# fixstars/cuda-bundle-adjustment

Measured on NVIDIA H100. Metric: LM edges/sec (10 iters), higher is better.
Workload: dtype f64

## Files before the change

### cuda-bundle-adjustment_b200/binding.py

```python
import ctypes as C
import os

import numpy as np

HERE = os.path.dirname(os.path.abspath(__file__))
ROBUST_NONE, ROBUST_HUBER, ROBUST_TUKEY = 0, 1, 2
EDGE_MONOCULAR, EDGE_STEREO = 0, 1
PROFILE_ITEMS = ("0: Initialize Optimizer", "1: Build Structure", "2: Compute Error", "3: Build System",
                 "4: Schur Complement", "5: Symbolic Decomposition", "6: Numerical Decomposition", "7: Update Solution")


PCG_INFO_LEN = 16
PCG_INFO_FIELDS = ("kernel", "two_level", "aggs_per_cta", "G", "gs", "A", "maxRows", "capBlocks", "zhInSmem", "coarse_kernel",
                   "cinfo", "status", "iters", "coarse_rebuilds", "bj_retries", "bad_rebuilds")
PCG_KERNELS = ("none", "k_pcg", "k_pcg2", "k_pcg3", "k_pcg4", "k_pcg5", "k_pcg5_big", "k_pcg5t")
COARSE_KERNELS = ("none", "k_coarse_invert", "cluster2<8>", "cluster2<16>", "k_coarse_dense", "k_coarse_chol_cluster")


class CubaError(RuntimeError):
    pass


def library_path():
    return os.path.join(HERE, "libcuba_b200.so")


class _Config(C.Structure):
    _fields_ = [("device", C.c_int), ("use_fp32", C.c_int), ("pcg_max_iters", C.c_int), ("pcg_tol", C.c_double),
                ("deterministic", C.c_int), ("reserved", C.c_int * 7)]


class _Problem(C.Structure):
    _fields_ = [("Pall", C.c_int32), ("numP", C.c_int32), ("Lall", C.c_int32), ("numL", C.c_int32),
                ("q", C.c_void_p), ("t", C.c_void_p), ("cam", C.c_void_p), ("Xw", C.c_void_p),
                ("E2", C.c_int32), ("idx2", C.c_void_p), ("meas2", C.c_void_p), ("omega2", C.c_void_p),
                ("E3", C.c_int32), ("idx3", C.c_void_p), ("meas3", C.c_void_p), ("omega3", C.c_void_p)]


class _IterStat(C.Structure):
    _fields_ = [("iteration", C.c_int32), ("trials", C.c_int32), ("chi2", C.c_double), ("lambda_", C.c_double),
                ("pcg_iters", C.c_int32), ("pcg_failed", C.c_int32)]


class _Sizes(C.Structure):
    _fields_ = [(n, C.c_int32) for n in ("Pall", "numP", "Lall", "numL", "E2", "E3", "nhpl", "nblk", "nmul", "nblk_full")]


_lib = None

_SYMBOLS = [
    "cuba_last_error", "cuba_version", "cuba_engine_create", "cuba_engine_destroy", "cuba_engine_set_robust_kernel",
    "cuba_comm_unique_id", "cuba_engine_set_comm", "cuba_engine_set_problem", "cuba_engine_set_structure_reuse", "cuba_engine_get_structure_reuses", "cuba_engine_set_state", "cuba_engine_get_sizes", "cuba_engine_reset_state", "cuba_engine_get_stream", "cuba_engine_flush_l2",
    "cuba_engine_optimize", "cuba_engine_get_state", "cuba_engine_get_chi2", "cuba_engine_get_profile",
    "cuba_engine_get_launch_count", "cuba_get_transfer_bytes", "cuba_stage_linearize", "cuba_stage_max_diagonal", "cuba_stage_solve", "cuba_stage_update",
    "cuba_stage_commit", "cuba_stage_chi2", "cuba_debug_get_hpl_structure", "cuba_debug_get_hsc_structure",
    "cuba_debug_get_system", "cuba_debug_get_schur", "cuba_debug_get_delta", "cuba_debug_get_pcg_info", "cuba_debug_get_coarse", "cuba_debug_build_structure_host", "cuba_debug_pcg_partition", "cuba_debug_pcg5_plan", "cuba_debug_pcg5_plan_apc", "cuba_debug_dropin_problem", "cuba_bench_stage",
]


def exported_symbols():
    return list(_SYMBOLS)


def load_library():
    global _lib
    if _lib is not None:
        return _lib
    path = library_path()
    if not os.path.exists(path):
        raise CubaError("%s not built: run `python -c 'import __graft_entry__ as g; g.build()'` (no CPU fallback exists)" % path)
    L = C.CDLL(path)
    L.cuba_last_error.restype = C.c_char_p
    vp, i, d = C.c_void_p, C.c_int, C.c_double
    sig = {
        "cuba_engine_create": [C.POINTER(_Config), C.POINTER(vp)],
        "cuba_engine_destroy": [vp],
        "cuba_engine_set_robust_kernel": [vp, i, i, d],
        "cuba_comm_unique_id": [vp],
        "cuba_engine_set_comm": [vp, i, i, vp],
        "cuba_engine_set_problem": [vp, C.POINTER(_Problem)],
        "cuba_engine_set_structure_reuse": [vp, i],
        "cuba_engine_get_structure_reuses": [vp, C.POINTER(C.c_longlong)],
        "cuba_engine_set_state": [vp, vp, vp, vp],
        "cuba_engine_get_sizes": [vp, C.POINTER(_Sizes)],
        "cuba_engine_reset_state": [vp],
        "cuba_engine_get_stream": [vp, C.POINTER(vp)],
        "cuba_engine_flush_l2": [vp],
        "cuba_engine_optimize": [vp, i, vp, C.POINTER(i)],
        "cuba_engine_get_state": [vp, vp, vp, vp],
        "cuba_engine_get_chi2": [vp, vp],
        "cuba_engine_get_profile": [vp, vp],
        "cuba_engine_get_launch_count": [vp, C.POINTER(C.c_longlong)],
        "cuba_get_transfer_bytes": [C.POINTER(C.c_longlong), C.POINTER(C.c_longlong)],
        "cuba_stage_linearize": [vp, C.POINTER(d)],
        "cuba_stage_max_diagonal": [vp, C.POINTER(d)],
        "cuba_stage_solve": [vp, d, C.POINTER(i), C.POINTER(i)],
        "cuba_stage_update": [vp, d, C.POINTER(d), C.POINTER(d)],
        "cuba_stage_commit": [vp, i],
        "cuba_stage_chi2": [vp, C.POINTER(d)],
        "cuba_debug_get_hpl_structure": [vp, vp, vp, vp],
        "cuba_debug_get_hsc_structure": [vp, vp, vp],
        "cuba_debug_get_system": [vp, vp, vp, vp, vp, vp],
        "cuba_debug_get_schur": [vp, vp, vp, vp],
        "cuba_debug_get_delta": [vp, vp, vp],
        "cuba_debug_get_pcg_info": [vp, vp, C.POINTER(d)],
        "cuba_debug_get_coarse": [vp, vp, vp, vp],
        "cuba_debug_build_structure_host": [C.POINTER(_Problem), i, i, C.POINTER(_Sizes), vp, vp, vp, vp, vp, vp, vp, vp],
        "cuba_debug_pcg_partition": [C.POINTER(_Problem), i, i, vp],
        "cuba_debug_pcg5_plan": [C.POINTER(_Problem), i, i, i, vp],
        "cuba_debug_pcg5_plan_apc": [C.POINTER(_Problem), i, i, i, i, vp, C.POINTER(C.c_uint64)],
        "cuba_debug_dropin_problem": [vp, C.POINTER(_Problem)],
        "cuba_bench_stage": [vp, i, i, i, d, C.POINTER(d)],
    }
    for name, args in sig.items():
        fn = getattr(L, name)
        fn.argtypes = args
        fn.restype = C.c_int
    _lib = L
    return L


def _check(rc):
    if rc != 0:
        raise CubaError("cuba error %d: %s" % (rc, load_library().cuba_last_error().decode()))


def _p(a):
    return None if a is None else a.ctypes.data_as(C.c_void_p)


def _problem_struct(prob):
    keep = [np.ascontiguousarray(prob.q, dtype=np.float64), np.ascontiguousarray(prob.t, dtype=np.float64),
            np.ascontiguousarray(prob.cam, dtype=np.float64), np.ascontiguousarray(prob.Xw, dtype=np.float64),
            np.ascontiguousarray(prob.idx2, dtype=np.int32), np.ascontiguousarray(prob.meas2, dtype=np.float64),
            np.ascontiguousarray(prob.omega2, dtype=np.float64), np.ascontiguousarray(prob.idx3, dtype=np.int32),
            np.ascontiguousarray(prob.meas3, dtype=np.float64), np.ascontiguousarray(prob.omega3, dtype=np.float64)]
    P = _Problem(prob.Pall, prob.numP, prob.Lall, prob.numL, _p(keep[0]), _p(keep[1]), _p(keep[2]), _p(keep[3]),
                 prob.E2, _p(keep[4]), _p(keep[5]), _p(keep[6]), prob.E3, _p(keep[7]), _p(keep[8]), _p(keep[9]))
    return P, keep


def transfer_bytes():
    a, b = C.c_longlong(0), C.c_longlong(0)
    _check(load_library().cuba_get_transfer_bytes(C.byref(a), C.byref(b)))
    return a.value, b.value


def build_structure_host(prob, rank=0, world=1):
    L = load_library()
    P, keep = _problem_struct(prob)
    sz = _Sizes()
    _check(L.cuba_debug_build_structure_host(C.byref(P), rank, world, C.byref(sz), None, None, None, None, None, None, None, None))
    out = {n: getattr(sz, n) for n, _ in _Sizes._fields_}
    arrs = {"hplColPtr": np.zeros(sz.numL + 1, np.int32), "hplRowInd": np.zeros(sz.nhpl, np.int32),
            "edge2Hpl": np.zeros(sz.E2 + sz.E3, np.int32), "hscRowPtr": np.zeros(sz.numP + 1, np.int32),
            "hscColInd": np.zeros(sz.nblk, np.int32), "fullRowPtr": np.zeros(sz.numP + 1, np.int32),
            "fullColInd": np.zeros(sz.nblk_full, np.int32), "shard": np.zeros(4, np.int32)}
    _check(L.cuba_debug_build_structure_host(C.byref(P), rank, world, C.byref(sz), *[_p(arrs[k]) for k in
           ("hplColPtr", "hplRowInd", "edge2Hpl", "hscRowPtr", "hscColInd", "fullRowPtr", "fullColInd", "shard")]))
    out.update(arrs)
    return out


def pcg_partition_host(prob, n_ctas=148, max_aggregates=74):
    L = load_library()
    P, keep = _problem_struct(prob)
    info = np.zeros(8, np.int32)
    _check(L.cuba_debug_pcg_partition(C.byref(P), int(n_ctas), int(max_aggregates), _p(info)))
    return dict(zip(("G", "gs", "A", "needMax", "maxRows", "blkMax", "maxNeedAgg", "coarse_list_size"), (int(v) for v in info)))


def pcg5_plan_host(prob, world=1, num_sms=148, max_aggregates=74):
    L = load_library()
    P, keep = _problem_struct(prob)
    info = np.zeros(8, np.int32)
    _check(L.cuba_debug_pcg5_plan(C.byref(P), int(world), int(num_sms), int(max_aggregates), _p(info)))
    return dict(zip(("ok", "G", "gs", "A", "needMax", "maxRows", "maxNeedAgg", "halo_rows"), (int(v) for v in info)))


def pcg5_plan_apc_host(prob, aggs_per_cta, world=1, num_sms=132, max_aggregates=148):
    L = load_library()
    P, keep = _problem_struct(prob)
    info = np.zeros(8, np.int32)
    h = C.c_uint64(0)
    _check(L.cuba_debug_pcg5_plan_apc(C.byref(P), int(world), int(num_sms), int(max_aggregates), int(aggs_per_cta), _p(info), C.byref(h)))
    out = dict(zip(("ok", "G", "gs", "A", "needMax", "maxRows", "maxNeedAgg", "halo_rows"), (int(v) for v in info)))
    out["hash"] = int(h.value)
    return out


class Engine:

    def __init__(self, device=-1, use_fp32=False, pcg_max_iters=0, pcg_tol=0.0, pcg_variant=0, structure_on_host=False, jh_variant=0, schur_variant=0,
                 coarse_refresh=0, two_level_switch=0, max_aggregates=0):
        self.L = load_library()
        res = (C.c_int * 7)()
        res[0] = int(pcg_variant)
        res[1] = int(bool(structure_on_host))
        res[2] = int(jh_variant)
        res[3] = int(schur_variant)
        res[4] = int(coarse_refresh)
        res[5] = int(two_level_switch)
        res[6] = int(max_aggregates)
        cfg = _Config(device, 2 if use_fp32 == "mixed" else int(use_fp32), int(pcg_max_iters), float(pcg_tol), 1, res)
        h = C.c_void_p()
        _check(self.L.cuba_engine_create(C.byref(cfg), C.byref(h)))
        self.h = h
        self.sizes = None
        self._stats = []

    def close(self):
        if getattr(self, "h", None):
            self.L.cuba_engine_destroy(self.h)
            self.h = None

    def __del__(self):
        try:
            self.close()
        except Exception:
            pass

    def set_robust_kernels(self, kernel_type, delta, edge_type):
        _check(self.L.cuba_engine_set_robust_kernel(self.h, int(edge_type), int(kernel_type), float(delta)))

    def set_comm(self, rank, world, unique_id=None):
        buf = None if unique_id is None else (C.c_char * 128).from_buffer_copy(bytes(unique_id))
        _check(self.L.cuba_engine_set_comm(self.h, rank, world, buf))

    @staticmethod
    def comm_unique_id():
        buf = (C.c_char * 128)()
        _check(load_library().cuba_comm_unique_id(buf))
        return bytes(buf)

    def initialize(self, prob):
        P, keep = _problem_struct(prob)
        _check(self.L.cuba_engine_set_problem(self.h, C.byref(P)))
        sz = _Sizes()
        _check(self.L.cuba_engine_get_sizes(self.h, C.byref(sz)))
        self.sizes = {n: getattr(sz, n) for n, _ in _Sizes._fields_}
        self._stats = []
        return self.sizes

    def set_structure_reuse(self, enable):
        _check(self.L.cuba_engine_set_structure_reuse(self.h, int(bool(enable))))

    def structure_reuses(self):
        n = C.c_longlong(0)
        _check(self.L.cuba_engine_get_structure_reuses(self.h, C.byref(n)))
        return n.value

    def set_state(self, q, t, Xw):
        q, t, Xw = (np.ascontiguousarray(a, dtype=np.float64) for a in (q, t, Xw))
        _check(self.L.cuba_engine_set_state(self.h, _p(q), _p(t), _p(Xw)))

    def reset_state(self):
        _check(self.L.cuba_engine_reset_state(self.h))

    def stream_ptr(self):
        s = C.c_void_p()
        _check(self.L.cuba_engine_get_stream(self.h, C.byref(s)))
        return s.value or 0

    def flush_l2(self):
        _check(self.L.cuba_engine_flush_l2(self.h))

    def optimize(self, niterations):
        stats = (_IterStat * max(niterations, 1))()
        n = C.c_int(0)
        _check(self.L.cuba_engine_optimize(self.h, niterations, stats, C.byref(n)))
        self._stats = [dict(iteration=s.iteration, trials=s.trials, chi2=s.chi2, lambda_=s.lambda_, pcg_iters=s.pcg_iters,
                            pcg_failed=s.pcg_failed) for s in stats[:n.value]]
        return self._stats

    def batch_statistics(self):
        return [(s["iteration"], s["chi2"]) for s in self._stats]

    def time_profile(self):
        sec = np.zeros(len(PROFILE_ITEMS))
        _check(self.L.cuba_engine_get_profile(self.h, _p(sec)))
        return dict(zip(PROFILE_ITEMS, sec.tolist()))

    def state(self):
        s = self.sizes
        q = np.zeros((s["Pall"], 4)); t = np.zeros((s["Pall"], 3)); Xw = np.zeros((s["Lall"], 3))
        _check(self.L.cuba_engine_get_state(self.h, _p(q), _p(t), _p(Xw)))
        return q, t, Xw

    def chi_squared(self):
        out = np.zeros(self.sizes["E2"] + self.sizes["E3"])
        _check(self.L.cuba_engine_get_chi2(self.h, _p(out)))
        return out

    def launch_count(self):
        n = C.c_longlong(0)
        _check(self.L.cuba_engine_get_launch_count(self.h, C.byref(n)))
        return n.value

    def linearize(self):
        v = C.c_double(0)
        _check(self.L.cuba_stage_linearize(self.h, C.byref(v)))
        return v.value

    def max_diagonal(self):
        v = C.c_double(0)
        _check(self.L.cuba_stage_max_diagonal(self.h, C.byref(v)))
        return v.value

    def solve(self, lam):
        it, ok = C.c_int(0), C.c_int(0)
        _check(self.L.cuba_stage_solve(self.h, float(lam), C.byref(it), C.byref(ok)))
        return it.value, bool(ok.value)

    def update(self, lam):
        chi, sc = C.c_double(0), C.c_double(0)
        _check(self.L.cuba_stage_update(self.h, float(lam), C.byref(chi), C.byref(sc)))
        return chi.value, sc.value

    def commit(self, accept):
        _check(self.L.cuba_stage_commit(self.h, int(bool(accept))))

    def chi2(self):
        v = C.c_double(0)
        _check(self.L.cuba_stage_chi2(self.h, C.byref(v)))
        return v.value

    def hpl_structure(self):
        s = self.sizes
        colPtr = np.zeros(s["numL"] + 1, np.int32); rowInd = np.zeros(s["nhpl"], np.int32); e2h = np.zeros(s["E2"] + s["E3"], np.int32)
        _check(self.L.cuba_debug_get_hpl_structure(self.h, _p(colPtr), _p(rowInd), _p(e2h)))
        return colPtr, rowInd, e2h

    def hsc_structure(self):
        s = self.sizes
        rowPtr = np.zeros(s["numP"] + 1, np.int32); colInd = np.zeros(s["nblk"], np.int32)
        _check(self.L.cuba_debug_get_hsc_structure(self.h, _p(rowPtr), _p(colInd)))
        return rowPtr, colInd

    def system(self):
        s = self.sizes
        Hpp = np.zeros((s["numP"], 36)); bp = np.zeros((s["numP"], 6)); Hll = np.zeros((s["numL"], 9)); bl = np.zeros((s["numL"], 3))
        Hpl = np.zeros((s["nhpl"], 18))
        _check(self.L.cuba_debug_get_system(self.h, _p(Hpp), _p(bp), _p(Hll), _p(bl), _p(Hpl)))
        return Hpp, bp, Hll, bl, Hpl

    def schur(self):
        s = self.sizes
        Hsc = np.zeros((s["nblk"], 36)); bsc = np.zeros((s["numP"], 6)); inv = np.zeros((s["numL"], 9))
        _check(self.L.cuba_debug_get_schur(self.h, _p(Hsc), _p(bsc), _p(inv)))
        return Hsc, bsc, inv

    def delta(self):
        s = self.sizes
        xp = np.zeros((s["numP"], 6)); xl = np.zeros((s["numL"], 3))
        _check(self.L.cuba_debug_get_delta(self.h, _p(xp), _p(xl)))
        return xp, xl

    def pcg_info(self):
        info = np.zeros(PCG_INFO_LEN, np.int32)
        lam = C.c_double(0)
        _check(self.L.cuba_debug_get_pcg_info(self.h, _p(info), C.byref(lam)))
        out = dict(zip(PCG_INFO_FIELDS, (int(v) for v in info)))
        out["kernel"] = PCG_KERNELS[out["kernel"]]
        out["coarse_kernel"] = COARSE_KERNELS[out["coarse_kernel"]]
        out["two_level"] = bool(out["two_level"])
        out["coarse_lambda"] = lam.value
        return out

    def coarse(self):
        A = self.pcg_info()["A"]
        agg = np.zeros(self.sizes["numP"], np.int32); AcP = np.zeros((A * (A + 1) // 2, 36)); AcInv = np.zeros((6 * A, 6 * A), np.float32)
        _check(self.L.cuba_debug_get_coarse(self.h, _p(agg), _p(AcP), _p(AcInv)))
        return agg, AcP, AcInv

    def bench_stage(self, stage, reps=10, flush_l2=True, lam=1.0):
        ms = C.c_double(0)
        _check(self.L.cuba_bench_stage(self.h, int(stage), int(reps), int(bool(flush_l2)), float(lam), C.byref(ms)))
        return ms.value
```

### cuda-bundle-adjustment_b200/csrc/cuba_coarse_dense.cuh

```cuda
#pragma once

#include "cuba_pcg4.cuh"

namespace cuba_b200 {
namespace cdense {

constexpr int NB = 16;
constexpr int WARPS = 8;
constexpr int TS = NB + 1;

struct Args {
	const double* AcP;
	int A;
	double* M;
	double* Lm;
	double* Dinv;
	double* W;
	float* AcInv;
	int* info;
	GridBar* bar;
};

__device__ __forceinline__ double ldcg(const double* p) { return __ldcg(p); }

__device__ __forceinline__ bool chol16(double* sD, double* sLi, int lane)
{
	bool ok = true;
	double rdiag = 0.0;
	for (int j = 0; j < NB; j++) {
		const double d = sD[j * TS + j];
		if (!(d > 0)) { ok = false; break; }
		const double sq = sqrt(d), rs = 1.0 / sq;
		__syncwarp();
		if (lane == j) { sD[j * TS + j] = sq; rdiag = rs; }
		else if (lane > j && lane < NB) sD[lane * TS + j] = sD[lane * TS + j] * rs;
		__syncwarp();
		if (lane > j && lane < NB) {
			const double lrj = sD[lane * TS + j];
			for (int c = j + 1; c <= lane; c++) sD[lane * TS + c] -= lrj * sD[c * TS + j];
		}
		__syncwarp();
	}
	if (!ok) return false;
	double col[NB];
#pragma unroll
	for (int i = 0; i < NB; i++) col[i] = 0.0;
	const int q = lane;
#pragma unroll
	for (int i = 0; i < NB; i++) {
		const double ri = __shfl_sync(0xffffffffu, rdiag, i);
		if (q < NB && i >= q) {
			if (i == q) col[i] = ri;
			else {
				double s = 0;
#pragma unroll
				for (int k = 0; k < NB; k++) if (k >= q && k < i) s += sD[i * TS + k] * col[k];
				col[i] = -s * ri;
			}
		}
	}
	if (q < NB) {
#pragma unroll
		for (int i = 0; i < NB; i++) sLi[i * TS + q] = i >= q ? col[i] : 0.0;
	}
	__syncwarp();
	return true;
}

__global__ void __launch_bounds__(WARPS * 32, 1) k_coarse_dense(const Args a)
{
	__shared__ double sD[NB * TS], sLi[NB * TS];
	__shared__ double sP[WARPS][2][NB * TS];
	__shared__ int s_fail;
	__shared__ unsigned int s_gen;
	const int tid = threadIdx.x, lane = tid & 31, wid = tid >> 5;
	const int G = gridDim.x, cta = blockIdx.x;
	const int n = 6 * a.A, nt = (n + NB - 1) / NB, np = nt * NB;
	const int nwarps = G * WARPS, gw = cta * WARPS + wid;
	if (tid == 0) { s_gen = ld_acquire_u32(&a.bar->gen); s_fail = 0; }
	__syncthreads();
	unsigned int gen = s_gen;
	const int r = lane >> 1, c0 = (lane & 1) * 8;

	{
		const int nblkP = a.A * (a.A + 1) / 2;
		for (long long e = (long long)cta * blockDim.x + tid; e < (long long)nblkP * 36; e += (long long)G * blockDim.x) {
			const int b = (int)(e / 36), rc = (int)(e - 36LL * b), c = rc / 6, rr = rc - 6 * c;
			int ib = (int)((sqrt(8.0 * b + 1.0) - 1.0) * 0.5);
			while ((ib + 1) * (ib + 2) / 2 <= b) ib++;
			while (ib * (ib + 1) / 2 > b) ib--;
			const int jb = b - ib * (ib + 1) / 2;
			const int row = 6 * ib + rr, col = 6 * jb + c;
			if (row >= col) __stcg(a.M + (size_t)col * np + row, a.AcP[e]);
		}
		for (int i = n + cta * blockDim.x + tid; i < np; i += G * blockDim.x) __stcg(a.M + (size_t)i * np + i, 1.0);
	}
	grid_barrier(a.bar, G, gen);

	for (int k = 0; k < nt; k++) {
		if (wid == 0) {
			for (int e = lane; e < NB * NB; e += 32) { const int rr = e % NB, cc = e / NB; sD[rr * TS + cc] = rr >= cc ? ldcg(a.M + (size_t)(k * NB + cc) * np + k * NB + rr) : 0.0; }
			__syncwarp();
			const bool ok = chol16(sD, sLi, lane);
			if (!ok && lane == 0) s_fail = 1;
			if (ok && cta == 0) {
				for (int e = lane; e < NB * NB; e += 32) {
					const int rr = e % NB, cc = e / NB;
					__stcg(a.Lm + (size_t)(k * NB + cc) * np + k * NB + rr, rr >= cc ? sD[rr * TS + cc] : 0.0);
					__stcg(a.Dinv + (size_t)k * NB * NB + rr * NB + cc, sLi[rr * TS + cc]);
				}
			}
		}
		__syncthreads();
		if (s_fail) break;
		const int m = nt - k - 1;
		const int ntile = m * (m + 1) / 2;
		double* Pi = sP[wid][0];
		double* Pj = sP[wid][1];
		for (int t = gw; t < ntile; t += nwarps) {
			int li = (int)((sqrt(8.0 * t + 1.0) - 1.0) * 0.5);
			while ((li + 1) * (li + 2) / 2 <= t) li++;
			while (li * (li + 1) / 2 > t) li--;
			const int lj = t - li * (li + 1) / 2;
			const int i = k + 1 + li, j = k + 1 + lj;
			{
				double arow[NB];
#pragma unroll
				for (int mm = 0; mm < NB; mm++) arow[mm] = ldcg(a.M + (size_t)(k * NB + mm) * np + i * NB + r);
#pragma unroll
				for (int c = 0; c < 8; c++) {
					const int cc = c0 + c;
					double s = 0;
#pragma unroll
					for (int mm = 0; mm < NB; mm++) if (mm <= cc) s += arow[mm] * sLi[cc * TS + mm];
					Pi[r * TS + cc] = s;
				}
				if (j != i) {
#pragma unroll
					for (int mm = 0; mm < NB; mm++) arow[mm] = ldcg(a.M + (size_t)(k * NB + mm) * np + j * NB + r);
#pragma unroll
					for (int c = 0; c < 8; c++) {
						const int cc = c0 + c;
						double s = 0;
#pragma unroll
						for (int mm = 0; mm < NB; mm++) if (mm <= cc) s += arow[mm] * sLi[cc * TS + mm];
						Pj[r * TS + cc] = s;
					}
				}
			}
			__syncwarp();
			const double* Q = j != i ? Pj : Pi;
#pragma unroll
			for (int c = 0; c < 8; c++) {
				const int cc = c0 + c;
				double s = 0;
#pragma unroll
				for (int mm = 0; mm < NB; mm++) s += Pi[r * TS + mm] * Q[cc * TS + mm];
				double* dst = a.M + (size_t)(j * NB + cc) * np + i * NB + r;
				__stcg(dst, ldcg(dst) - s);
				if (j == i) __stcg(a.Lm + (size_t)(k * NB + cc) * np + i * NB + r, Pi[r * TS + cc]);
			}
			__syncwarp();
		}
		grid_barrier(a.bar, G, gen);
	}
	if (s_fail) {
		for (long long e = (long long)cta * blockDim.x + tid; e < (long long)n * n; e += (long long)G * blockDim.x) a.AcInv[e] = 0.f;
		if (cta == 0 && tid == 0) *a.info = 1;
		return;
	}

	for (int jt = cta; jt < nt; jt += G) {
		for (int e = tid; e < NB * NB; e += blockDim.x) { const int rr = e / NB, cc = e % NB; __stcg(a.W + (size_t)(jt * NB + cc) * np + jt * NB + rr, ldcg(a.Dinv + (size_t)jt * NB * NB + e)); }
		__syncthreads();
		for (int i = jt + 1; i < nt; i++) {
			double acc[8];
#pragma unroll
			for (int c = 0; c < 8; c++) acc[c] = 0.0;
			for (int k = jt + wid; k < i; k += WARPS) {
				double lrow[NB];
#pragma unroll
				for (int mm = 0; mm < NB; mm++) lrow[mm] = ldcg(a.Lm + (size_t)(k * NB + mm) * np + i * NB + r);
#pragma unroll
				for (int c = 0; c < 8; c++) {
					const double* wc = a.W + (size_t)(jt * NB + c0 + c) * np + k * NB;
					double s = 0;
#pragma unroll
					for (int mm = 0; mm < NB; mm++) s += lrow[mm] * ldcg(wc + mm);
					acc[c] += s;
				}
			}
#pragma unroll
			for (int c = 0; c < 8; c++) sP[wid][1][r * NB + c0 + c] = acc[c];
			__syncthreads();
			if (wid == 0) {
				double* S = sP[0][0];
#pragma unroll
				for (int c = 0; c < 8; c++) {
					double s = 0;
#pragma unroll
					for (int w = 0; w < WARPS; w++) s += sP[w][1][r * NB + c0 + c];
					S[r * TS + c0 + c] = s;
				}
				__syncwarp();
				double lrow[NB];
#pragma unroll
				for (int mm = 0; mm < NB; mm++) lrow[mm] = ldcg(a.Dinv + (size_t)i * NB * NB + r * NB + mm);
#pragma unroll
				for (int c = 0; c < 8; c++) {
					double s = 0;
#pragma unroll
					for (int mm = 0; mm < NB; mm++) if (mm <= r) s += lrow[mm] * S[mm * TS + c0 + c];
					__stcg(a.W + (size_t)(jt * NB + c0 + c) * np + i * NB + r, -s);
				}
			}
			__syncthreads();
		}
	}
	grid_barrier(a.bar, G, gen);

	{
		const int ntile = nt * (nt + 1) / 2;
		double* Wi = sP[wid][0];
		double* Wj = sP[wid][1];
		for (int t = gw; t < ntile; t += nwarps) {
			int i = (int)((sqrt(8.0 * t + 1.0) - 1.0) * 0.5);
			while ((i + 1) * (i + 2) / 2 <= t) i++;
			while (i * (i + 1) / 2 > t) i--;
			const int j = t - i * (i + 1) / 2;
			double acc[8];
#pragma unroll
			for (int c = 0; c < 8; c++) acc[c] = 0.0;
			for (int k = i; k < nt; k++) {
#pragma unroll
				for (int c = 0; c < 8; c++) {
					Wi[r * TS + c0 + c] = ldcg(a.W + (size_t)(i * NB + c0 + c) * np + k * NB + r);
					Wj[r * TS + c0 + c] = ldcg(a.W + (size_t)(j * NB + c0 + c) * np + k * NB + r);
				}
				__syncwarp();
#pragma unroll
				for (int c = 0; c < 8; c++) {
					double s = 0;
#pragma unroll
					for (int mm = 0; mm < NB; mm++) s += Wi[mm * TS + r] * Wj[mm * TS + c0 + c];
					acc[c] += s;
				}
				__syncwarp();
			}
#pragma unroll
			for (int c = 0; c < 8; c++) {
				const int row = i * NB + r, col = j * NB + c0 + c;
				if (row < n && col < n) {
					const float v = (float)acc[c];
					a.AcInv[(size_t)row * n + col] = v;
					a.AcInv[(size_t)col * n + row] = v;
				}
			}
		}
	}
	if (cta == 0 && tid == 0) *a.info = 0;
}

}
}
```

### cuda-bundle-adjustment_b200/csrc/cuba_engine.cu

```cuda
#include <cuda_runtime.h>
#include <dlfcn.h>

#include <algorithm>
#include <chrono>
#include <cmath>
#include <cstdio>
#include <cstring>
#include <memory>
#include <string>
#include <vector>

#include "../../include/cuba_b200.h"
#include "cuba_kernels.cuh"
#include "cuba_pcg2.cuh"
#include "cuba_pcg3.cuh"
#include "cuba_pcg4.cuh"
#include "cuba_pcg5.cuh"
#include "cuba_pcg5t.cuh"
#include "cuba_coarse_dense.cuh"
#include "cuba_peer_reduce.cuh"
#include "cuba_schur2.cuh"
#include "cuba_jh4.cuh"
#include "cuba_schur3.cuh"
#include "cuba_schur5.cuh"
#include "cuba_structure.h"
#include "cuba_structure_gpu.cuh"

namespace cuba_b200 {

static thread_local std::string g_err;
static int fail(int code, const std::string& msg) { g_err = msg; return code; }

#define CUDA_TRY(expr)                                                                                      \
	do {                                                                                                    \
		cudaError_t _e = (expr);                                                                            \
		if (_e != cudaSuccess) {                                                                            \
			char _b[512];                                                                                   \
			snprintf(_b, sizeof(_b), "%s:%d: %s -> %s", __FILE__, __LINE__, #expr, cudaGetErrorString(_e)); \
			return fail(CUBA_ERR_CUDA, _b);                                                                 \
		}                                                                                                   \
	} while (0)

#define KLAUNCH(kernel, n, ...)                                                             \
	do {                                                                                     \
		if ((n) > 0) {                                                                       \
			kernel<<<sgpu::grid_for(n), sgpu::BLK, 0, stream>>>(__VA_ARGS__);                 \
			launches++;                                                                      \
			CUDA_TRY(cudaGetLastError());                                                    \
		}                                                                                    \
	} while (0)

static thread_local long long g_h2dBytes = 0, g_d2hBytes = 0;

struct PinnedArena {
	char* p = nullptr; size_t cap = 0, off = 0;
	~PinnedArena() { if (p) cudaFreeHost(p); }
	void reset() { off = 0; }
	void* put(const void* src, size_t bytes)
	{
		const size_t o = (off + 255) & ~(size_t)255;
		if (o + bytes > cap) {
			if (off != 0) return nullptr;
			if (p) cudaFreeHost(p);
			cap = std::max<size_t>(2 * (o + bytes), (size_t)1 << 20);
			if (cudaMallocHost((void**)&p, cap) != cudaSuccess) { p = nullptr; cap = 0; return nullptr; }
		}
		memcpy(p + o, src, bytes);
		off = o + bytes;
		return p + o;
	}
};

template <typename U>
struct DBuf {
	U* p = nullptr; size_t n = 0, cap = 0;
	bool view = false;
	DBuf() {}
	DBuf(const DBuf&) = delete;
	DBuf& operator=(const DBuf&) = delete;
	~DBuf() { release(); }
	void release() { if (p && !view) cudaFree(p); p = nullptr; n = 0; cap = 0; view = false; }
	void alias(U* q, size_t count) { release(); p = q; n = count; cap = count; view = true; }
	cudaError_t alloc(size_t count)
	{
		if (p && count <= cap && !view) { n = count; return cudaSuccess; }
		release();
		n = count; cap = count ? count : 1;
		return cudaMalloc((void**)&p, sizeof(U) * cap);
	}
	cudaError_t upload(const U* h, size_t count, cudaStream_t s)
	{
		cudaError_t e = alloc(count);
		if (e != cudaSuccess || !count) return e;
		g_h2dBytes += (long long)(sizeof(U) * count);
		return cudaMemcpyAsync(p, h, sizeof(U) * count, cudaMemcpyHostToDevice, s);
	}
	cudaError_t upload(const std::vector<U>& h, cudaStream_t s) { return upload(h.data(), h.size(), s); }
	cudaError_t upload(const std::vector<U>& h, cudaStream_t s, PinnedArena& arena)
	{
		const void* src = h.empty() ? nullptr : arena.put(h.data(), sizeof(U) * h.size());
		return upload(src ? (const U*)src : h.data(), h.size(), s);
	}
	operator U*() const { return p; }
};

struct Nccl {
	void* lib = nullptr;
	typedef struct { char internal[128]; } UniqueId;
	int (*GetUniqueId)(UniqueId*) = nullptr;
	int (*CommInitRank)(void**, int, UniqueId, int) = nullptr;
	int (*CommDestroy)(void*) = nullptr;
	int (*AllReduce)(const void*, void*, size_t, int, int, void*, cudaStream_t) = nullptr;
	int (*AllGather)(const void*, void*, size_t, int, void*, cudaStream_t) = nullptr;
	int (*Broadcast)(const void*, void*, size_t, int, int, void*, cudaStream_t) = nullptr;
	int (*GroupStart)() = nullptr;
	int (*GroupEnd)() = nullptr;
	const char* (*GetErrorString)(int) = nullptr;
	bool load(std::string& why)
	{
		if (lib) return true;
		const char* names[] = { "libnccl.so.2", "libnccl.so" };
		for (const char* nme : names) { lib = dlopen(nme, RTLD_NOW | RTLD_GLOBAL); if (lib) break; }
		if (!lib) { why = std::string("dlopen libnccl.so.2 failed: ") + dlerror(); return false; }
		GetUniqueId = (int (*)(UniqueId*))dlsym(lib, "ncclGetUniqueId");
		CommInitRank = (int (*)(void**, int, UniqueId, int))dlsym(lib, "ncclCommInitRank");
		CommDestroy = (int (*)(void*))dlsym(lib, "ncclCommDestroy");
		AllReduce = (int (*)(const void*, void*, size_t, int, int, void*, cudaStream_t))dlsym(lib, "ncclAllReduce");
		AllGather = (int (*)(const void*, void*, size_t, int, void*, cudaStream_t))dlsym(lib, "ncclAllGather");
		Broadcast = (int (*)(const void*, void*, size_t, int, int, void*, cudaStream_t))dlsym(lib, "ncclBroadcast");
		GroupStart = (int (*)())dlsym(lib, "ncclGroupStart");
		GroupEnd = (int (*)())dlsym(lib, "ncclGroupEnd");
		GetErrorString = (const char* (*)(int))dlsym(lib, "ncclGetErrorString");
		if (!GetUniqueId || !CommInitRank || !CommDestroy || !AllReduce || !AllGather || !Broadcast || !GroupStart || !GroupEnd) { why = "libnccl lacks expected symbols"; return false; }
		return true;
	}
};
static Nccl g_nccl;
enum { NCCL_INT8 = 0, NCCL_FLOAT32 = 7, NCCL_FLOAT64 = 8, NCCL_SUM = 0, NCCL_MAX = 2 };

struct Scalars { double v[8]; unsigned long long maxdiag; PcgStatus pcg; };

struct DevGuard {
	int prev = -1, dev;
	explicit DevGuard(int d) : dev(d) { if (cudaGetDevice(&prev) != cudaSuccess) prev = -1; if (prev != dev) cudaSetDevice(dev); }
	~DevGuard() { if (prev >= 0 && prev != dev) cudaSetDevice(prev); }
};

struct EngineBase {
	virtual ~EngineBase() {}
	cuba_config cfg{};
	int rk_type[2] = { 0, 0 };
	double rk_delta[2] = { 0, 0 };
	int rank = 0, world = 1;
	bool structureReuse = true;
	long long structureReuses = 0;
	int devOrdinal = 0;
	void* comm = nullptr;
	bool haveProblem = false;
	long long launches = 0;
	double prof[CUBA_PROF_NUM] = { 0 };

	virtual int set_problem(const cuba_problem* p) = 0;
	virtual int set_state(const double* q, const double* t, const double* Xw) = 0;
	virtual int get_sizes(cuba_sizes* out) const = 0;
	virtual int reset_state() = 0;
	virtual int get_stream(void** s) = 0;
	virtual int flush_l2() = 0;
	virtual int optimize(int niter, cuba_iter_stat* stats, int* nstats) = 0;
	virtual int get_state(double* q, double* t, double* Xw) = 0;
	virtual int get_chi2(double* out) = 0;
	virtual int get_profile(double* sec) = 0;
	virtual int stage_linearize(double* chi) = 0;
	virtual int stage_max_diagonal(double* md) = 0;
	virtual int stage_solve(double lambda, int* iters, int* ok) = 0;
	virtual int stage_update(double lambda, double* chi, double* scale) = 0;
	virtual int stage_commit(int accept) = 0;
	virtual int stage_chi2(double* chi) = 0;
	virtual int dbg_hpl_structure(int32_t* colPtr, int32_t* rowInd, int32_t* e2h) = 0;
	virtual int dbg_hsc_structure(int32_t* rowPtr, int32_t* colInd) = 0;
	virtual int dbg_system(double* Hpp, double* bp, double* Hll, double* bl, double* Hpl) = 0;
	virtual int dbg_schur(double* Hsc, double* bsc, double* invHll) = 0;
	virtual int dbg_delta(double* xp, double* xl) = 0;
	virtual int bench_stage(int stage, int reps, int flush, double lambda, double* ms) = 0;
	virtual int dbg_pcg_timing(long long* out, int maxCtas) = 0;
	virtual int dbg_pcg_info(int32_t* info, double* coarseLambda) = 0;
	virtual int dbg_coarse(int32_t* rowAgg, double* AcP, float* AcInv) = 0;
};

template <typename T>
struct Engine : EngineBase {
	Structure S;
	cudaStream_t stream = nullptr;
	int numSMs = 0;
	int ntiles = 0, nPoseBlocks = 0, nChiBlocks = 0;
	int tileSize = TILE;
	int jhMinBlocks = 2;
	bool jhV2 = true;
	bool jhV3 = true;
	int jh3Grid = 0, nChiLin = 0;
	bool jhV4 = true;
	int ntW = 0, jh4Grid = 0, jh4HasBig = 0, jh4MinB = 4, jh4Nst = 2;
	const void* jh4AttrSet = nullptr;
	int* jh4Host = nullptr;
	bool jh4Pending = false;
	DBuf<int> w_levels, w_start, w_pieces, w_base, w_tilePose, w_tilePieces, w_pieceCount, w_flag;
	DBuf<jh4::WTile> w_tile;
	DBuf<jh4::Rec> w_rec;
	DBuf<double> w_bigPartial;
	DBuf<TileInfo> tileInfo;
	bool useSchur2 = true;
	bool useSchur5 = false;
	int s5Ntiles = 0;
	DBuf<int> s5TileLm;
	DBuf<TileInfo> s5TileInfo;
	DBuf<int4> s5SegRec;
	DBuf<unsigned int> s5Off;
	int s2Nseg = 0, s2Nvalid = 0;
	DBuf<unsigned long long> s2_key, s2_keyS, s2_key3, s2_key3S;
	DBuf<int> s2_val, s2_valS, s2_head, s2_segId, s2_segStart, s2_segTile, s2_segDest, s2_val3, s2_val3S, s2_segRank, s2_rankDest, s2_tileSegPtr, s2_destSegPtr, s2_p2i, s2_p2j;
	DBuf<schur2::Counts> s2_counts;
	DBuf<T> s2_partial;
	DBuf<int> tilePose0, tilePoseN;
	int cur = 0;
	bool trialValid = false;
	DBuf<T> pose[2], Xw[2], cam, pose0, Xw0;
	DBuf<T> e_mx, e_my, e_mz, e_om, p_mx, p_my, p_mz, p_om;
	DBuf<int> tilePtr;
	DBuf<int> e_ip, e_il, e_hpl, e_user, lmPtr, tileLm, hplLm, posePtr, p_il;
	DBuf<T> Hpp, bp, Hll, bl, Hpl, invHll, fVal, bsc, xp, xl;
	DBuf<T> uVal;
	DBuf<float> HplF;
	bool mixed = false;
	bool upperReduce = false;
	DBuf<int> prodPtr, prodI, prodJ, prodL, blkRow, blkCol, u2f, u2fT, fRowPtr, fColInd;
	bool useSchur3 = true;
	DBuf<T> pr, pz, pq, pp0, pp1, Minv;
	DBuf<double> pcgPartial;
	int pcgGrid = 0;
	DBuf<T> fHat, Linv, vR0, vR1, vS0, vS1, vW0, vW1, vP, vY;
	DBuf<int> fLocal, ctaRow, needPtr, needCol;
	DBuf<double> pcg2Partial;
	DBuf<GridBar> gridBar;
	DBuf<long long> pcgTiming;
	DBuf<unsigned long long> llFlags;
	int pcg2Grid = 0, pcg2Cap = 0, pcg2NeedMax = 0, pcg2MaxRows = 0;
	DBuf<T> cZx, cZhat;
	DBuf<float> cAcInv;
	DBuf<double> cAcP, cPart, cU, cLp, cLd, cWp;
	DBuf<int> cAggRow, cNaPtr, cNaList, cNeedAgg, cInfo, cRowOf, cCbPtr, cCbList;
	int pcg4A = 0, pcg4Gs = 1, pcg4MaxNeedAgg = 0, pcg4Cap = 0, pcg4SliceInSmem = 0, pcg4ZhInSmem = 0;
	size_t pcg4Smem = 0, pcg4InvSmem = 0;
	bool pcg4Ok = false, tlActive = false, pcg4Cluster = false;
	PinnedArena arena;
	bool coarseValid = false;
	int coarseAge = 0;
	double coarseLambda = 0, curLambda = 0;
	bool pcg3Ok = false;
	size_t pcg2Smem = 0;
	DBuf<double> chiPartial, scalePartialL, scalePartialP, chiSq;
	DBuf<Scalars> dScal;
	Scalars* hScal = nullptr;
	DBuf<double> flushBuf;
	std::vector<std::pair<int, std::pair<cudaEvent_t, cudaEvent_t>>> profEvents;
	std::vector<cudaEvent_t> eventPool;

	~Engine() override
	{
		DevGuard guard(devOrdinal);
		if (stream) cudaStreamSynchronize(stream);
		p5CloseMappings(); uCloseMappings();
		for (auto& pe : profEvents) { cudaEventDestroy(pe.second.first); cudaEventDestroy(pe.second.second); }
		for (auto ev : eventPool) cudaEventDestroy(ev);
		if (hScal) cudaFreeHost(hScal);
		if (hMeta) cudaFreeHost(hMeta);
		if (jh4Host) cudaFreeHost(jh4Host);
		if (stream) cudaStreamDestroy(stream);
		if (comm && g_nccl.CommDestroy) g_nccl.CommDestroy(comm);
	}

	int init()
	{
		int ndev = 0;
		cudaError_t e = cudaGetDeviceCount(&ndev);
		if (e != cudaSuccess || ndev <= 0)
			return fail(CUBA_ERR_CUDA, std::string("no CUDA device available (") + cudaGetErrorString(e) + "); this library has no CPU fallback");
		if (cfg.device >= 0) CUDA_TRY(cudaSetDevice(cfg.device));
		int dev = 0;
		CUDA_TRY(cudaGetDevice(&dev));
		devOrdinal = dev;
		CUDA_TRY(cudaDeviceGetAttribute(&numSMs, cudaDevAttrMultiProcessorCount, dev));
		CUDA_TRY(cudaStreamCreateWithFlags(&stream, cudaStreamNonBlocking));
		CUDA_TRY(cudaMallocHost((void**)&hScal, sizeof(Scalars)));
		memset(hScal, 0, sizeof(Scalars));
		CUDA_TRY(dScal.alloc(1));
		CUDA_TRY(cudaMemsetAsync(dScal.p, 0, sizeof(Scalars), stream));
		return CUBA_OK;
	}

	cudaEvent_t newEvent()
	{
		cudaEvent_t ev;
		if (!eventPool.empty()) { ev = eventPool.back(); eventPool.pop_back(); return ev; }
		cudaEventCreate(&ev);
		return ev;
	}
	struct ProfScope {
		Engine* e; int item; cudaEvent_t a, b;
		ProfScope(Engine* e_, int item_) : e(e_), item(item_) { a = e->newEvent(); b = e->newEvent(); cudaEventRecord(a, e->stream); }
		~ProfScope() { cudaEventRecord(b, e->stream); e->profEvents.push_back({ item, { a, b } }); }
	};
	void resolveProfile()
	{
		cudaStreamSynchronize(stream);
		for (auto& pe : profEvents) {
			float ms = 0;
			if (cudaEventElapsedTime(&ms, pe.second.first, pe.second.second) == cudaSuccess) prof[pe.first] += 1e-3 * ms;
			eventPool.push_back(pe.second.first); eventPool.push_back(pe.second.second);
		}
		profEvents.clear();
	}

	RobustParams rkParams() const
	{
		RobustParams r;
		for (int i = 0; i < 2; i++) { r.type[i] = rk_type[i]; r.delta[i] = rk_delta[i]; }
		return r;
	}

	int allreduce(void* buf, size_t count, bool isT)
	{
		if (world <= 1 || !comm) return CUBA_OK;
		const int dt = isT ? (sizeof(T) == 8 ? NCCL_FLOAT64 : NCCL_FLOAT32) : NCCL_FLOAT64;
		const int rc = g_nccl.AllReduce(buf, buf, count, dt, NCCL_SUM, comm, stream);
		if (rc != 0) return fail(CUBA_ERR_COMM, std::string("ncclAllReduce failed: ") + (g_nccl.GetErrorString ? g_nccl.GetErrorString(rc) : "?"));
		return CUBA_OK;
	}

	DBuf<double> rawQ, rawT, rawC, rawX;
	int upload_state(const double* q, const double* t, const double* c, const double* X)
	{
		const int Pall = S.Pall, Lall = S.Lall;
		CUDA_TRY(rawQ.upload(q, 4 * (size_t)Pall, stream)); CUDA_TRY(rawT.upload(t, 3 * (size_t)Pall, stream));
		CUDA_TRY(rawX.upload(X, 3 * (size_t)Lall, stream));
		if (c) CUDA_TRY(rawC.upload(c, 5 * (size_t)Pall, stream));
		CUDA_TRY(pose0.alloc(8 * (size_t)Pall)); CUDA_TRY(Xw0.alloc(4 * (size_t)Lall));
		for (int b = 0; b < 2; b++) { CUDA_TRY(pose[b].alloc(8 * (size_t)Pall)); CUDA_TRY(Xw[b].alloc(4 * (size_t)Lall)); }
		if (c) CUDA_TRY(cam.alloc(8 * (size_t)Pall));
		const int n = std::max(Pall, Lall);
		if (n > 0) {
			k_pack_state<T><<<(n + 255) / 256, 256, 0, stream>>>(rawQ.p, rawT.p, c ? rawC.p : nullptr, rawX.p, Pall, Lall,
				pose0.p, pose[0].p, pose[1].p, c ? cam.p : nullptr, Xw0.p, Xw[0].p, Xw[1].p);
			launches++;
			CUDA_TRY(cudaGetLastError());
		}
		return CUBA_OK;
	}

	std::vector<std::pair<const char*, std::chrono::steady_clock::time_point>> marks;
	void tmark(const char* name) { if (markOn) marks.push_back({ name, std::chrono::steady_clock::now() }); }
	bool markOn = false;
	int set_problem(const cuba_problem* p) override
	{
		markOn = getenv("CUBA_SETUP_TIMING") != nullptr; marks.clear(); tmark("start");
		if (!p) return fail(CUBA_ERR_INVALID, "set_problem: null problem");
		if (p->Pall < 0 || p->Lall < 0 || p->numP < 0 || p->numL < 0 || p->numP > p->Pall || p->numL > p->Lall || p->E2 < 0 || p->E3 < 0)
			return fail(CUBA_ERR_INVALID, "set_problem: invalid sizes");
		if ((p->Pall > 0 && (!p->q || !p->t || !p->cam)) || (p->Lall > 0 && !p->Xw) || (p->E2 > 0 && (!p->idx2 || !p->meas2 || !p->omega2)) ||
			(p->E3 > 0 && (!p->idx3 || !p->meas3 || !p->omega3)))
			return fail(CUBA_ERR_INVALID, "set_problem: null array with a non-zero count");
		const auto t0 = std::chrono::steady_clock::now();
		lastPcgKernel = CUBA_PCG_KERNEL_NONE; p5Rebuilds = 0; bjRetries = 0;
		if (structureReuse && reusable && haveProblem && cfg.reserved[1] != 1 && same_topology(p)) {
			int rc = refresh_values(p); if (rc) return rc;
			structureReuses++;
			prof[CUBA_PROF_BUILD_STRUCTURE] += std::chrono::duration<double>(std::chrono::steady_clock::now() - t0).count();
			return CUBA_OK;
		}
		haveProblem = false;
		reusable = false;
		hostStructureValid = false;
		shardBoundValid = false;
		switch (cfg.reserved[2]) {
		case 2: tileSize = 256; jhMinBlocks = 3; break;
		case 3: tileSize = 128; jhMinBlocks = 4; break;
		case 4: tileSize = 128; jhMinBlocks = 6; break;
		case 1: tileSize = 256; jhMinBlocks = 2; break;
		default: tileSize = JH2_TL; jhMinBlocks = 4; break;
		}
		jhV4 = (cfg.reserved[2] == 0 || (cfg.reserved[2] >= 7 && cfg.reserved[2] <= 9)) && sizeof(T) == 8;
		jh4Nst = cfg.reserved[2] == 7 ? 3 : 2;
		jh4MinB = cfg.reserved[2] == 8 ? 5 : (cfg.reserved[2] == 9 ? 6 : 4);
		jhV3 = cfg.reserved[2] == 6 && sizeof(T) == 8;
		jhV2 = cfg.reserved[2] == 5 && sizeof(T) == 8;
		if (cfg.reserved[2] == 5) { tileSize = JH2_TL; jhMinBlocks = 4; }
		if (cfg.reserved[2] == 0 && sizeof(T) != 8) { tileSize = 128; jhMinBlocks = 6; }
		int rc = (cfg.reserved[1] == 1) ? build_on_host(p) : build_on_gpu(p);
		if (rc) return rc;
		tmark("structure built");
		rc = upload_state(p->q, p->t, p->cam, p->Xw); if (rc) return rc;
		tmark("state uploaded");
		rc = alloc_system(); if (rc) return rc;
		CUDA_TRY(cudaStreamSynchronize(stream));
		tmark("alloc_system done");
		if (markOn) {
			for (size_t i = 1; i < marks.size(); i++)
				fprintf(stderr, "setup %-28s %8.3f ms\n", marks[i].first, 1e3 * std::chrono::duration<double>(marks[i].second - marks[i - 1].second).count());
			fprintf(stderr, "setup total %8.3f ms\n", 1e3 * std::chrono::duration<double>(marks.back().second - marks.front().second).count());
		}
		cur = 0; trialValid = false;
		tlActive = false; coarseValid = false; coarseAge = 0; p5CoarseValid = false; p5CoarseAge = 0;
		resolveProfile();
		for (int i = 0; i < CUBA_PROF_NUM; i++) prof[i] = 0;
		const auto t1 = std::chrono::steady_clock::now();
		prof[CUBA_PROF_BUILD_STRUCTURE] += std::chrono::duration<double>(t1 - t0).count();
		haveProblem = true;
		if (cfg.reserved[1] != 1 && structureReuse) {
			lastIdx2.assign(p->idx2, p->idx2 + 2 * (size_t)p->E2); lastIdx3.assign(p->idx3, p->idx3 + 2 * (size_t)p->E3);
			const int sz[6] = { p->Pall, p->numP, p->Lall, p->numL, p->E2, p->E3 };
			memcpy(lastSizes, sz, sizeof(sz));
			reusable = true;
		}
		return CUBA_OK;
	}

	bool same_topology(const cuba_problem* p) const
	{
		const int sz[6] = { p->Pall, p->numP, p->Lall, p->numL, p->E2, p->E3 };
		if (memcmp(sz, lastSizes, sizeof(sz)) != 0) return false;
		if (p->E2 > 0 && memcmp(p->idx2, lastIdx2.data(), sizeof(int32_t) * 2 * (size_t)p->E2) != 0) return false;
		if (p->E3 > 0 && memcmp(p->idx3, lastIdx3.data(), sizeof(int32_t) * 2 * (size_t)p->E3) != 0) return false;
		return true;
	}

	int refresh_values(const cuba_problem* p)
	{
		using namespace sgpu;
		const int E2 = p->E2, E3 = p->E3, eL = S.eLocal;
		CUDA_TRY(g_meas2.upload(p->meas2, 2 * (size_t)E2, stream)); CUDA_TRY(g_meas3.upload(p->meas3, 3 * (size_t)E3, stream));
		CUDA_TRY(g_om2.upload(p->omega2, (size_t)E2, stream)); CUDA_TRY(g_om3.upload(p->omega3, (size_t)E3, stream));
		int rc = upload_state(p->q, p->t, p->cam, p->Xw); if (rc) return rc;
		KLAUNCH(k_edge_stream<T>, eL, g_keyS.p, g_valS.p, g_ff.p, g_hplG.p, savedKBeg, eL, S.hplBase, E2, g_meas2.p, g_om2.p, g_meas3.p, g_om3.p,
			e_user.p, e_ip.p, e_il.p, e_hpl.p, e_mx.p, e_my.p, e_mz.p, e_om.p);
		KLAUNCH(k_pose_stream<T>, eL, g_psrc.p, posePtr.p, S.numP, eL, e_ip.p, e_il.p, e_mx.p, e_my.p, e_mz.p, e_om.p, p_il.p, p_mx.p, p_my.p, p_mz.p, p_om.p);
		if constexpr (sizeof(T) == 8) {
			if (jhV4 && ntW > 0) {
				const int lb = S.lmBeg, N = S.lmEnd - S.lmBeg;
				KLAUNCH(jh4::k_emit, (long long)N * 32, w_start.p, w_pieces.p, w_base.p, N, lmPtr.p, lb, w_levels.p,
					e_mx.p, e_my.p, e_mz.p, e_om.p, e_ip.p, e_il.p, e_hpl.p, w_tile.p, w_rec.p, w_tilePose.p, w_tilePieces.p);
			}
		}
		CUDA_TRY(cudaStreamSynchronize(stream));
		cur = 0; trialValid = false;
		tlActive = false; coarseValid = false; coarseAge = 0; p5CoarseValid = false; p5CoarseAge = 0;
		resolveProfile();
		for (int i = 0; i < CUBA_PROF_NUM; i++) prof[i] = 0;
		return CUBA_OK;
	}

	int build_on_host(const cuba_problem* p)
	{
		const char* err = "";
		if (!build_structure(p->Pall, p->numP, p->Lall, p->numL, p->E2, p->idx2, p->E3, p->idx3, rank, world, tileSize, S, &err))
			return fail(CUBA_ERR_INVALID, err);
		hostStructureValid = true;
		const int eL = S.eLocal;
		std::vector<T> mx(eL), my(eL), mz(eL), om(eL);
		for (int e = 0; e < eL; e++) {
			const int u = S.order[e];
			if (u < S.E2) { mx[e] = (T)p->meas2[2 * (size_t)u]; my[e] = (T)p->meas2[2 * (size_t)u + 1]; mz[e] = T(0); om[e] = (T)p->omega2[u]; }
			else { const size_t k = (size_t)(u - S.E2); mx[e] = (T)p->meas3[3 * k]; my[e] = (T)p->meas3[3 * k + 1]; mz[e] = (T)p->meas3[3 * k + 2]; om[e] = (T)p->omega3[k]; }
		}
		CUDA_TRY(e_mx.upload(mx, stream)); CUDA_TRY(e_my.upload(my, stream)); CUDA_TRY(e_mz.upload(mz, stream)); CUDA_TRY(e_om.upload(om, stream));
		CUDA_TRY(e_ip.upload(S.e_ip, stream)); CUDA_TRY(e_il.upload(S.e_il, stream)); CUDA_TRY(e_hpl.upload(S.e_hpl, stream));
		CUDA_TRY(e_user.upload(S.order, stream));
		CUDA_TRY(lmPtr.upload(S.lmPtr, stream)); CUDA_TRY(tilePtr.upload(S.lmPtr, stream));
		CUDA_TRY(tileLm.upload(S.tileLm, stream)); CUDA_TRY(hplLm.upload(S.hplLm, stream));
		const size_t nPe = S.p_src.size();
		std::vector<T> qx(nPe), qy(nPe), qz(nPe), qo(nPe);
		for (size_t k = 0; k < nPe; k++) { const int e = S.p_src[k]; qx[k] = mx[e]; qy[k] = my[e]; qz[k] = mz[e]; qo[k] = om[e]; }
		CUDA_TRY(p_mx.upload(qx, stream)); CUDA_TRY(p_my.upload(qy, stream)); CUDA_TRY(p_mz.upload(qz, stream)); CUDA_TRY(p_om.upload(qo, stream));
		CUDA_TRY(p_il.upload(S.p_il, stream)); CUDA_TRY(posePtr.upload(S.posePtr, stream));
		CUDA_TRY(prodPtr.upload(S.prodPtr, stream)); CUDA_TRY(prodI.upload(S.prodI, stream)); CUDA_TRY(prodJ.upload(S.prodJ, stream));
		CUDA_TRY(blkRow.upload(S.blkRow, stream)); CUDA_TRY(blkCol.upload(S.blkCol, stream));
		CUDA_TRY(u2f.upload(S.u2f, stream)); CUDA_TRY(u2fT.upload(S.u2fT, stream));
		CUDA_TRY(fRowPtr.upload(S.fRowPtr, stream)); CUDA_TRY(fColInd.upload(S.fColInd, stream));
		CUDA_TRY(cudaStreamSynchronize(stream));
		ntiles = (int)S.tileLm.size() - 1;
		return CUBA_OK;
	}
// ... 570 lines not shown
					schur3::k_schur3<double, float><<<(S.nblk + schur3::WARPS - 1) / schur3::WARPS, schur3::WARPS * 32, 0, stream>>>(m);
				}
			}
			else if (cfg.reserved[3] != 4) schur3::k_schur3<T><<<(S.nblk + schur3::WARPS - 1) / schur3::WARPS, schur3::WARPS * 32, 0, stream>>>(a);
			else schur3::k_schur4<T><<<(S.nblk + schur3::WARPS - 1) / schur3::WARPS, schur3::WARPS * 32, 0, stream>>>(a);
			launches++;
			CUDA_TRY(cudaGetLastError());
			if (upperReduce) {
				static const bool timing = getenv("CUBA_SCHUR_TIMING") != nullptr;
				cudaEvent_t ev[3];
				if (timing) { for (auto& e : ev) cudaEventCreate(&e); cudaEventRecord(ev[0], stream); }
				int rc = uPeerOk ? launch_peer_allreduce() : allreduce(uVal.p, 36 * (size_t)S.nblk + 6 * (size_t)S.numP, true); if (rc) return rc;
				if (timing) cudaEventRecord(ev[1], stream);
				KLAUNCH(schur3::k_expand_upper<T>, 36LL * S.nblk, uVal.p, u2f.p, u2fT.p, blkRow.p, blkCol.p, S.nblk, fVal.p);
				if (timing) {
					cudaEventRecord(ev[2], stream); cudaEventSynchronize(ev[2]);
					float a1 = 0, a2 = 0; cudaEventElapsedTime(&a1, ev[0], ev[1]); cudaEventElapsedTime(&a2, ev[1], ev[2]);
					static int count = 0;
					if (rank == 0 && (count++ % 16) == 8) fprintf(stderr, "schur split: all-reduce (%s) %.3f ms, expand %.3f ms, %zu elements\n", uPeerOk ? "peer" : "nccl", a1, a2, uCount);
					for (auto& e : ev) cudaEventDestroy(e);
				}
			}
			else if (world > 1) {
				int rc = allreduce(fVal.p, 36 * (size_t)S.nfull + 6 * (size_t)S.numP, true); if (rc) return rc;
			}
		}
		else if (S.numP > 0 && S.numL > 0) {
			SchurArgs<T> a;
			a.Hpl = Hpl; a.invHll = invHll; a.bl = bl; a.Hpp = Hpp; a.bp = bp;
			a.prodPtr = prodPtr; a.prodI = prodI; a.prodJ = prodJ; a.hplLm = hplLm;
			a.blkRow = blkRow; a.blkCol = blkCol; a.u2f = u2f; a.u2fT = u2fT; a.nblk = S.nblk;
			a.lambda = lambda; a.addDiag = rank == 0 ? 1 : 0; a.fVal = fVal; a.bsc = bsc;
			const int wpb = SCHUR_BLOCK / 32;
			k_schur<T><<<(S.nblk + wpb - 1) / wpb, SCHUR_BLOCK, 0, stream>>>(a);
			launches++;
			CUDA_TRY(cudaGetLastError());
			if (world > 1) {
				int rc = allreduce(fVal.p, 36 * (size_t)S.nfull + 6 * (size_t)S.numP, true); if (rc) return rc;
			}
		}
		return CUBA_OK;
	}

	int setup_jh4()
	{
		ntW = 0; jh4Grid = 0; jh4HasBig = 0;
		if constexpr (sizeof(T) == 8) {
			using namespace jh4;
			const int lb = S.lmBeg, N = S.lmEnd - S.lmBeg;
			if (N <= 0 || S.eLocal <= 0) return CUBA_OK;
			int K = 1;
			while ((1LL << K) <= (long long)N) K++;
			CUDA_TRY(w_levels.alloc((size_t)K * ((size_t)N + 1)));
			CUDA_TRY(w_start.alloc((size_t)N + 1)); CUDA_TRY(w_pieces.alloc((size_t)N + 1)); CUDA_TRY(w_base.alloc((size_t)N + 1));
			CUDA_TRY(w_flag.alloc(1));
			CUDA_TRY(cudaMemsetAsync(w_flag.p, 0, sizeof(int), stream));
			KLAUNCH(jh4::k_next, N + 1, lmPtr.p, lb, N, w_levels.p);
			for (int k = 1; k < K; k++)
				KLAUNCH(jh4::k_lift, N + 1, w_levels.p + (size_t)(k - 1) * ((size_t)N + 1), N, w_levels.p + (size_t)k * ((size_t)N + 1));
			KLAUNCH(jh4::k_starts, N + 1, w_levels.p, K, N, lmPtr.p, lb, w_start.p, w_pieces.p, w_flag.p);
			int rc = exclusiveSum(w_pieces.p, w_base.p, N + 1); if (rc) return rc;
			if (!jh4Host) CUDA_TRY(cudaMallocHost((void**)&jh4Host, 2 * sizeof(int)));
			CUDA_TRY(cudaMemcpyAsync(&jh4Host[0], w_base.p + N, sizeof(int), cudaMemcpyDeviceToHost, stream));
			CUDA_TRY(cudaMemcpyAsync(&jh4Host[1], w_flag.p, sizeof(int), cudaMemcpyDeviceToHost, stream));
			jh4Pending = true;
		}
		return CUBA_OK;
	}
	int setup_jh4_finish()
	{
		if (!jh4Pending) return CUBA_OK;
		jh4Pending = false;
		if constexpr (sizeof(T) == 8) {
			using namespace jh4;
			const int lb = S.lmBeg, N = S.lmEnd - S.lmBeg;
			CUDA_TRY(cudaStreamSynchronize(stream));
			const int big = jh4Host[1];
			ntW = jh4Host[0]; jh4HasBig = big;
			if (ntW <= 0) return CUBA_OK;
			CUDA_TRY(w_tile.alloc(ntW)); CUDA_TRY(w_rec.alloc(ntW)); CUDA_TRY(w_tilePose.alloc(32 * (size_t)ntW)); CUDA_TRY(w_tilePieces.alloc(ntW)); CUDA_TRY(w_pieceCount.alloc(ntW));
			CUDA_TRY(cudaMemsetAsync(w_pieceCount.p, 0, sizeof(int) * (size_t)ntW, stream));
			CUDA_TRY(w_bigPartial.alloc(std::max<size_t>(big ? 12 * (size_t)ntW : 12, 11 * (size_t)numSMs * 6 * jh4::WARPS)));
			KLAUNCH(jh4::k_emit, (long long)N * 32, w_start.p, w_pieces.p, w_base.p, N, lmPtr.p, lb, w_levels.p,
				e_mx.p, e_my.p, e_mz.p, e_om.p, e_ip.p, e_il.p, e_hpl.p, w_tile.p, w_rec.p, w_tilePose.p, w_tilePieces.p);
			jh4Grid = std::max(1, std::min((ntW + WARPS - 1) / WARPS, numSMs * jh4MinB));
		}
		return CUBA_OK;
	}

	int setup_schur2(const TileInfo* tinfo, int nt)
	{
		using namespace schur2;
		const int N = (int)S.nmulLocal, nblk = S.nblk;
		if (N <= 0) { useSchur2 = false; useSchur5 = false; return CUBA_OK; }
		CUDA_TRY(s2_key.alloc(N)); CUDA_TRY(s2_keyS.alloc(N)); CUDA_TRY(s2_val.alloc(N)); CUDA_TRY(s2_valS.alloc(N));
		CUDA_TRY(s2_head.alloc(N)); CUDA_TRY(s2_segId.alloc(N)); CUDA_TRY(s2_counts.alloc(1));
		KLAUNCH(schur2::k_keys, N, prodPtr.p, nblk, prodI.p, N, tinfo, nt, s2_key.p, s2_val.p);
		int rc = sortPairs(s2_key.p, s2_keyS.p, s2_val.p, s2_valS.p, N, 64); if (rc) return rc;
		KLAUNCH(schur2::k_heads, N, s2_keyS.p, N, s2_head.p);
		rc = exclusiveSum(s2_head.p, s2_segId.p, N); if (rc) return rc;
		schur2::k_counts<<<1, 32, 0, stream>>>(s2_keyS.p, s2_head.p, s2_segId.p, N, s2_counts.p);
		launches++;
		schur2::Counts hc;
		CUDA_TRY(cudaMemcpyAsync(&hc, s2_counts.p, sizeof(hc), cudaMemcpyDeviceToHost, stream));
		CUDA_TRY(cudaStreamSynchronize(stream));
		const int nseg = hc.nseg;
		s2Nseg = nseg; s2Nvalid = hc.nvalid;
		CUDA_TRY(s2_segStart.alloc((size_t)nseg + 1)); CUDA_TRY(s2_segTile.alloc(nseg)); CUDA_TRY(s2_segDest.alloc(nseg));
		CUDA_TRY(s2_key3.alloc(nseg)); CUDA_TRY(s2_key3S.alloc(nseg)); CUDA_TRY(s2_val3.alloc(nseg)); CUDA_TRY(s2_val3S.alloc(nseg));
		CUDA_TRY(s2_segRank.alloc(nseg)); CUDA_TRY(s2_rankDest.alloc(nseg));
		CUDA_TRY(s2_tileSegPtr.alloc((size_t)nt + 1)); CUDA_TRY(s2_destSegPtr.alloc((size_t)nblk + 1));
		CUDA_TRY(s2_p2i.alloc(N)); CUDA_TRY(s2_p2j.alloc(N));
		KLAUNCH(schur2::k_segments, N + 1, s2_keyS.p, s2_valS.p, s2_head.p, s2_segId.p, prodI.p, prodJ.p, N, nseg, hc.nvalid,
			s2_segStart.p, s2_segTile.p, s2_segDest.p, s2_p2i.p, s2_p2j.p, s2_key3.p, s2_val3.p);
		KLAUNCH(schur2::k_ptr_from_field, nt + 1, s2_segTile.p, nseg, nt, s2_tileSegPtr.p);
		rc = sortPairs(s2_key3.p, s2_key3S.p, s2_val3.p, s2_val3S.p, nseg, 32 + sgpu::bits_for((unsigned long long)std::max(nblk, 1))); if (rc) return rc;
		KLAUNCH(schur2::k_rank, nseg, s2_key3S.p, s2_val3S.p, nseg, s2_segRank.p, s2_rankDest.p);
		KLAUNCH(schur2::k_ptr_from_field, nblk + 1, s2_rankDest.p, nseg, nblk, s2_destSegPtr.p);
		CUDA_TRY(s2_partial.alloc((size_t)schur2::PW * std::max(nseg, 1)));
		return CUBA_OK;
	}

	int setup_pcg2()
	{
		const int numP = S.numP;
		int smemMax = 0;
		CUDA_TRY(cudaDeviceGetAttribute(&smemMax, cudaDevAttrMaxSharedMemoryPerBlockOptin, devOrdinal));
		const size_t budget = (size_t)smemMax > 8192 ? (size_t)smemMax - 6144 : 0;
		const size_t matBytes = (size_t)S.nfull * (36 * sizeof(T) + 4);
		int G = std::max((numP + 7) / 8, (int)((matBytes + budget - 1) / std::max<size_t>(budget, 1)));
		G = std::max(1, std::min(G, std::min(numSMs, numP)));
		PcgPartition& PP = hostPP;
		build_pcg_partition(numP, S.nfull, S.fRowPtr, S.fColInd, G, PP);
		const std::vector<int>& rows = PP.rows; const std::vector<int>& nptr = PP.nptr; const std::vector<int>& ncol = PP.ncol; const std::vector<int>& local = PP.local;
		const int needMax = PP.needMax, blkMax = PP.blkMax, maxRows = PP.maxRows;
		const size_t needBytes = (size_t)needMax * (12 * sizeof(T) + 8) + (size_t)maxRows * (12 * sizeof(T) + 4) + ((size_t)maxRows + 1) * 4
			+ (size_t)PCG3_CHUNK * 6 * sizeof(T);
		pcg3Ok = maxRows * 6 <= PCG3_BLOCK && 2 * G <= 2 * PCG3_BLOCK;
		size_t cap = budget > needBytes ? (budget - needBytes) / (36 * sizeof(T) + 4) : 0;
		cap = std::min<size_t>(cap, (size_t)blkMax);
		pcg2Grid = G; pcg2Cap = (int)cap; pcg2NeedMax = needMax; pcg2MaxRows = maxRows;
		pcg2Smem = (size_t)cap * 36 * sizeof(T) + needBytes + (size_t)cap * 4 + 16;
		CUDA_TRY(cudaFuncSetAttribute(k_pcg2<T>, cudaFuncAttributeMaxDynamicSharedMemorySize, (int)pcg2Smem));
		CUDA_TRY(cudaFuncSetAttribute(k_pcg3<T>, cudaFuncAttributeMaxDynamicSharedMemorySize, (int)pcg2Smem));
		CUDA_TRY(llFlags.alloc(2 * (2 * 6 * (size_t)numP) + 2 * (2 * PCG3_REPL * 2 * (size_t)G) + 2));
		int perSM = 0;
		CUDA_TRY(cudaOccupancyMaxActiveBlocksPerMultiprocessor(&perSM, k_pcg2<T>, PCG2_BLOCK, pcg2Smem));
		if (perSM < 1) return fail(CUBA_ERR_CUDA, "k_pcg2 cannot be resident with the requested shared memory");
		arena.reset();
		CUDA_TRY(ctaRow.upload(rows, stream, arena)); CUDA_TRY(needPtr.upload(nptr, stream, arena)); CUDA_TRY(needCol.upload(ncol, stream, arena));
		CUDA_TRY(fLocal.upload(local, stream, arena));
		const size_t n6 = 6 * (size_t)numP;
		CUDA_TRY(fHat.alloc(36 * (size_t)S.nfull)); CUDA_TRY(Linv.alloc(36 * (size_t)numP));
		CUDA_TRY(vR0.alloc(n6)); CUDA_TRY(vR1.alloc(n6)); CUDA_TRY(vS0.alloc(n6)); CUDA_TRY(vS1.alloc(n6));
		CUDA_TRY(vW0.alloc(n6)); CUDA_TRY(vW1.alloc(n6)); CUDA_TRY(vP.alloc(n6)); CUDA_TRY(vY.alloc(n6));
		CUDA_TRY(pcg2Partial.alloc(4 * (size_t)G));
		CUDA_TRY(gridBar.alloc(1));
		CUDA_TRY(cudaMemsetAsync(gridBar.p, 0, sizeof(GridBar), stream));
		tmark("  pcg2 partition + uploads");
		pcg4Ok = false;
		if (cfg.reserved[0] == 3 || sizeof(T) != 8 || numP > 80 * numSMs * (world > 1 && numP >= 2048 ? world : 1)) {
			const int maxAgg = (cfg.reserved[6] > 0 && cfg.reserved[6] < PCG4_MAXAGG) ? cfg.reserved[6] : PCG4_MAXAGG;
			CoarsePartition CP;
			build_coarse_partition(numP, PP, maxAgg, CP);
			const int gs = CP.gs, A = CP.A, nc = 6 * A;
			pcg4Cluster = A > PCG4_MAXAGG1;
			pcg4A = A; pcg4Gs = gs; pcg4MaxNeedAgg = CP.maxNeedAgg;
			size_t fixed4 = (size_t)needMax * (12 * sizeof(T) + 8) + (size_t)maxRows * (6 * sizeof(T) + 8) + 8 + 2 * (size_t)nc * sizeof(T)
				+ (size_t)pcg4MaxNeedAgg * (6 * sizeof(T) + 4) + 64;
			const size_t matAll = (size_t)blkMax * (36 * sizeof(T) + 4);
			const size_t zhBytes = (size_t)needMax * 36 * sizeof(T);
			const size_t sliceBytes = (((size_t)pcg4MaxNeedAgg * 6 * nc + 1) & ~(size_t)1) * sizeof(float);
			pcg4ZhInSmem = budget >= fixed4 + matAll + zhBytes ? 1 : 0;
			if (pcg4ZhInSmem) fixed4 += zhBytes;
			pcg4SliceInSmem = budget >= fixed4 + matAll + sliceBytes ? 1 : 0;
			if (pcg4SliceInSmem) fixed4 += sliceBytes;
			size_t cap4 = budget > fixed4 ? (budget - fixed4) / (36 * sizeof(T) + 4) : 0;
			cap4 = std::min<size_t>(cap4, (size_t)blkMax);
			pcg4Cap = (int)cap4;
			pcg4Smem = (size_t)cap4 * (36 * sizeof(T) + 4) + fixed4;
			if (getenv("CUBA_PCG_VERBOSE")) fprintf(stderr, "pcg4: G %d A %d gs %d needMax %d maxRows %d blkMax %d maxNeedAgg %d zhInSmem %d sliceInSmem %d cap %d smem %zu\n",
				G, A, gs, needMax, maxRows, blkMax, pcg4MaxNeedAgg, pcg4ZhInSmem, pcg4SliceInSmem, pcg4Cap, pcg4Smem);
			const size_t nblkPz = (size_t)A * (A + 1) / 2;
			pcg4InvSmem = pcg4Cluster ? (((nblkPz + PCG4_CL - 1) / PCG4_CL + 2 * (size_t)A) * 36 * sizeof(double) + 2 * nblkPz + 16)
			                          : ((nblkPz + 2 * (size_t)A) * 36 * sizeof(double));
			pcg4Ok = budget > fixed4 && nc + 64 <= PCG4_BLOCK && pcg4InvSmem + 1024 <= (size_t)smemMax && numP >= 2 * A;
			if (pcg4Ok) {
				CUDA_TRY(cudaFuncSetAttribute(k_pcg4<T>, cudaFuncAttributeMaxDynamicSharedMemorySize, (int)pcg4Smem));
				if (pcg4Cluster) CUDA_TRY(cudaFuncSetAttribute(k_coarse_chol_cluster, cudaFuncAttributeMaxDynamicSharedMemorySize, (int)pcg4InvSmem));
				else CUDA_TRY(cudaFuncSetAttribute(k_coarse_invert<T>, cudaFuncAttributeMaxDynamicSharedMemorySize, (int)pcg4InvSmem));
				int perSM4 = 0;
				CUDA_TRY(cudaOccupancyMaxActiveBlocksPerMultiprocessor(&perSM4, k_pcg4<T>, PCG4_BLOCK, pcg4Smem));
				if (perSM4 < 1) pcg4Ok = false;
			}
			if (pcg4Ok) {
				CUDA_TRY(cAggRow.upload(CP.aggRow, stream, arena)); CUDA_TRY(cNaPtr.upload(CP.naPtr, stream, arena)); CUDA_TRY(cNaList.upload(CP.naList, stream, arena));
				CUDA_TRY(cNeedAgg.upload(CP.needAgg, stream, arena));
				build_coarse_lists(numP, S.nfull, S.fRowPtr, S.fColInd, CP);
				CUDA_TRY(cRowOf.upload(CP.rowOf, stream, arena)); CUDA_TRY(cCbPtr.upload(CP.cbPtr, stream, arena)); CUDA_TRY(cCbList.upload(CP.cbList, stream, arena));
				CUDA_TRY(cZx.alloc(36 * (size_t)numP)); CUDA_TRY(cZhat.alloc(36 * (size_t)numP)); CUDA_TRY(cU.alloc(36 * (size_t)S.nfull));
				CUDA_TRY(cAcP.alloc((size_t)A * (A + 1) / 2 * 36)); CUDA_TRY(cAcInv.alloc((size_t)nc * nc));
				CUDA_TRY(cLp.alloc((size_t)A * (A + 1) / 2 * 36)); CUDA_TRY(cWp.alloc((size_t)A * (A + 1) / 2 * 36)); CUDA_TRY(cLd.alloc((size_t)A * 36));
				CUDA_TRY(cPart.alloc(2 * (size_t)G * PCG4_PSTRIDE)); CUDA_TRY(cInfo.alloc(1));
				CUDA_TRY(cudaMemsetAsync(cPart.p, 0, sizeof(double) * cPart.n, stream));
			}
			tlActive = false; coarseValid = false; coarseAge = 0;
		}
		return CUBA_OK;
	}

	int launch_pcg4()
	{
		ProfScope ps(this, CUBA_PROF_DECOMP_NUMERICAL);
		const int numP = S.numP, A = pcg4A, nblkP = A * (A + 1) / 2;
		KLAUNCH(k_coarse_basis<T>, numP, pose[cur].p, numP, cZx.p);
		const int refreshEvery = cfg.reserved[4] > 0 ? cfg.reserved[4] : 8;
		const double lamRatio = (coarseValid && coarseLambda > 0 && curLambda > 0) ? std::max(curLambda / coarseLambda, coarseLambda / curLambda) : 1.0;
		if (!coarseValid || coarseAge >= refreshEvery || lamRatio > 300.0) {
			KLAUNCH(k_coarse_project<T>, 36LL * S.nfull, fVal.p, cRowOf.p, fColInd.p, S.nfull, cZx.p, cU.p);
			KLAUNCH(k_coarse_assemble, (long long)nblkP * 36, cCbPtr.p, cCbList.p, cU.p, nblkP, cAcP.p);
			if (pcg4Cluster) {
				k_coarse_chol_cluster<<<PCG4_CL, 1024, pcg4InvSmem, stream>>>(cAcP.p, A, cLp.p, cLd.p, cAcInv.p, cInfo.p);
				k_coarse_trinv<<<A, 256, (size_t)A * 36 * sizeof(double), stream>>>(cLp.p, cLd.p, A, cWp.p, cInfo.p);
				k_coarse_wtw<<<(nblkP * 36 + 255) / 256, 256, 0, stream>>>(cWp.p, A, cAcInv.p, cInfo.p);
				launches += 2;
			}
			else k_coarse_invert<T><<<1, 1024, pcg4InvSmem, stream>>>(cAcP.p, A, cAcInv.p, cInfo.p);
			launches++;
			CUDA_TRY(cudaGetLastError());
			coarseValid = true; coarseAge = 0; coarseLambda = curLambda;
		}
		coarseAge++;
		Pcg4Args<T> b;
		Pcg2Args<T>& a = b.base;
		a.fRowPtr = fRowPtr; a.fColInd = fColInd; a.fLocal = fLocal; a.fVal = fVal; a.fHat = fHat;
		a.ctaRow = ctaRow; a.needPtr = needPtr; a.needCol = needCol; a.b = bsc; a.numP = S.numP; a.Linv = Linv;
		a.R0 = vR0; a.R1 = vR1; a.S0 = vS0; a.S1 = vS1; a.W0 = vW0; a.W1 = vW1; a.P = vP; a.Y = vY; a.x = xp;
		a.partial = pcg2Partial; a.bar = gridBar; a.capBlocks = pcg4Cap; a.needMax = pcg2NeedMax; a.maxRows = pcg2MaxRows;
		a.maxIters = cfg.pcg_max_iters > 0 ? cfg.pcg_max_iters : std::max(200, 40 * S.numP);
		const double tol = cfg.pcg_tol > 0 ? cfg.pcg_tol : (sizeof(T) == 8 ? 1e-11 : 1e-6);
		a.tol2 = tol * tol;
		a.status = &dScal.p->pcg;
		b.Zx = cZx; b.Zhat = cZhat; b.AcInv = cAcInv; b.aggRow = cAggRow; b.naPtr = cNaPtr; b.naList = cNaList; b.needAgg = cNeedAgg;
		b.A = A; b.gs = pcg4Gs; b.maxNeedAgg = pcg4MaxNeedAgg; b.sliceInSmem = pcg4SliceInSmem; b.zhInSmem = pcg4ZhInSmem; b.cpart = cPart;
		b.timing = nullptr;
#ifdef CUBA_PCG_TIMING
		CUDA_TRY(pcgTiming.alloc(8 * (size_t)pcg2Grid));
		b.timing = pcgTiming.p;
#endif
		void* args[] = { (void*)&b };
		CUDA_TRY(cudaLaunchCooperativeKernel((void*)k_pcg4<T>, dim3(pcg2Grid), dim3(PCG4_BLOCK), args, pcg4Smem, stream));
		launches++;
		lastPcgTwoLevel = true;
		lastPcgKernel = CUBA_PCG_KERNEL_PCG4;
		return CUBA_OK;
	}
	bool lastPcgTwoLevel = false;
	bool forceBlockJacobi = false;
	void note_pcg_iters(int iters) { if (!lastPcgTwoLevel && iters > (cfg.reserved[5] > 0 ? cfg.reserved[5] : 100)) tlActive = true; }

	int launch_pcg2(bool flagged)
	{
		ProfScope ps(this, CUBA_PROF_DECOMP_NUMERICAL);
		Pcg2Args<T> a;
		a.fRowPtr = fRowPtr; a.fColInd = fColInd; a.fLocal = fLocal; a.fVal = fVal; a.fHat = fHat;
		a.ctaRow = ctaRow; a.needPtr = needPtr; a.needCol = needCol; a.b = bsc; a.numP = S.numP; a.Linv = Linv;
		a.R0 = vR0; a.R1 = vR1; a.S0 = vS0; a.S1 = vS1; a.W0 = vW0; a.W1 = vW1; a.P = vP; a.Y = vY; a.x = xp;
		a.partial = pcg2Partial; a.bar = gridBar; a.capBlocks = pcg2Cap; a.needMax = pcg2NeedMax; a.maxRows = pcg2MaxRows;
		a.maxIters = cfg.pcg_max_iters > 0 ? cfg.pcg_max_iters : std::max(200, 40 * S.numP);
		const double tol = cfg.pcg_tol > 0 ? cfg.pcg_tol : (sizeof(T) == 8 ? 1e-11 : 1e-6);
		a.tol2 = tol * tol;
		a.status = &dScal.p->pcg;
		if (flagged) {
			Pcg3Args<T> b;
			b.base = a;
			b.wFlag = llFlags.p;
			b.pFlag = llFlags.p + 2 * (2 * 6 * (size_t)S.numP);
			b.abortFlag = (int*)(b.pFlag + 2 * (2 * PCG3_REPL * 2 * (size_t)pcg2Grid));
			b.timing = nullptr;
#ifdef CUBA_PCG_TIMING
			CUDA_TRY(pcgTiming.alloc(8 * (size_t)pcg2Grid));
			b.timing = pcgTiming.p;
#endif
			CUDA_TRY(cudaMemsetAsync(llFlags.p, 0, sizeof(unsigned long long) * llFlags.n, stream));
			void* args3[] = { (void*)&b };
			CUDA_TRY(cudaLaunchCooperativeKernel((void*)k_pcg3<T>, dim3(pcg2Grid), dim3(PCG3_BLOCK), args3, pcg2Smem, stream));
			launches++;
			lastPcgKernel = CUBA_PCG_KERNEL_PCG3;
			return CUBA_OK;
		}
		void* args[] = { (void*)&a };
		CUDA_TRY(cudaLaunchCooperativeKernel((void*)k_pcg2<T>, dim3(pcg2Grid), dim3(PCG2_BLOCK), args, pcg2Smem, stream));
		launches++;
		lastPcgKernel = CUBA_PCG_KERNEL_PCG2;
		return CUBA_OK;
	}


	DBuf<int> p5CtaRow, p5NeedPtr, p5NeedCol, p5Local, p5AggRow, p5NaPtr, p5NaList, p5NeedAgg, p5CbPtr, p5CbList;
	DBuf<unsigned char> p5RowPeers;
	DBuf<T> p5Linv, p5R0, p5Zhat, p5RcRow, p5Rc0;
	DBuf<float> p5AcInv;
	DBuf<double> p5AcP, p5Lp, p5Wp, p5Ld;
	DBuf<double> cdM, cdL, cdW, cdDinv;
	bool p5Dense = false;
	DBuf<unsigned long long> p5Boards;
	void* p5PeerBase[PCG5_MAXWORLD] = { nullptr };
	void* p5MappedFor = nullptr;
	size_t p5WWords = 0, p5PWords = 0, p5RWords = 0, p5CWords = 0;
	PcgPartition hostPP;
	Pcg5Dims p5Dims{}, p5DimsBJ{};
	size_t p5Smem = 0;
	int p5G = 0, p5W = 1, p5A = 0, p5Gs = 1;
	bool p5Ok = false, p5Dist = false, p5Big = false, p5Tuned = false;
	p5t::Pcg5Dims p5tDims{}, p5tDimsBJ{};
	const void* p5Fn = nullptr;
	int p5Block = PCG5_BLOCK;
	int p5Cluster = 0;
	bool p5CoarseValid = false; int p5CoarseAge = 0; double p5CoarseLambda = 0;
	size_t p5InvSmem = 0;
	int p5Apc = 1;
	static constexpr int P5_INFO_LOG = 256;
	int lastPcgKernel = CUBA_PCG_KERNEL_NONE;
	long long p5Rebuilds = 0, bjRetries = 0;
	int* p5InfoSlot() const { return cInfo.p + 1 + (int)(p5Rebuilds % P5_INFO_LOG); }
	long long p5TagBound = 0;

	Pcg5Ctl* p5Ctl(void* base) const { return (Pcg5Ctl*)((unsigned long long*)base + 2 * (p5WWords + p5PWords + p5RWords + p5CWords)); }

	void p5CloseMappings()
	{
		for (int r = 0; r < PCG5_MAXWORLD; r++) {
			if (p5PeerBase[r] && r != rank) cudaIpcCloseMemHandle(p5PeerBase[r]);
			p5PeerBase[r] = nullptr;
		}
		p5MappedFor = nullptr;
	}

	int ipcExchange(void* localBase, void** peerBase, void*& mappedFor, bool& ok)
	{
		ok = false;
		if (mappedFor == localBase) { ok = true; return CUBA_OK; }
		for (int r = 0; r < PCG5_MAXWORLD; r++) { if (peerBase[r] && r != rank) cudaIpcCloseMemHandle(peerBase[r]); peerBase[r] = nullptr; }
		mappedFor = nullptr;
		cudaIpcMemHandle_t mine;
		int good = cudaIpcGetMemHandle(&mine, localBase) == cudaSuccess ? 1 : 0;
		if (!good) cudaGetLastError();
		DBuf<char> dh;
		CUDA_TRY(dh.alloc(sizeof(cudaIpcMemHandle_t) * (size_t)world));
		CUDA_TRY(cudaMemcpyAsync(dh.p + sizeof(cudaIpcMemHandle_t) * (size_t)rank, &mine, sizeof(mine), cudaMemcpyHostToDevice, stream));
		int rc = g_nccl.AllGather(dh.p + sizeof(cudaIpcMemHandle_t) * (size_t)rank, dh.p, sizeof(cudaIpcMemHandle_t), NCCL_INT8, comm, stream);
		if (rc != 0) return fail(CUBA_ERR_COMM, "ncclAllGather (memory handles) failed");
		std::vector<cudaIpcMemHandle_t> all(world);
		CUDA_TRY(cudaMemcpyAsync(all.data(), dh.p, sizeof(cudaIpcMemHandle_t) * (size_t)world, cudaMemcpyDeviceToHost, stream));
		CUDA_TRY(cudaStreamSynchronize(stream));
		for (int r = 0; r < world && good; r++) {
			if (r == rank) { peerBase[r] = localBase; continue; }
			if (cudaIpcOpenMemHandle(&peerBase[r], all[r], cudaIpcMemLazyEnablePeerAccess) != cudaSuccess) { cudaGetLastError(); peerBase[r] = nullptr; good = 0; }
		}
		DBuf<double> flag;
		CUDA_TRY(flag.alloc(1));
		const double mineOk = good;
		CUDA_TRY(cudaMemcpyAsync(flag.p, &mineOk, sizeof(double), cudaMemcpyHostToDevice, stream));
		rc = allreduce(flag.p, 1, false); if (rc) return rc;
		double tot = 0;
		CUDA_TRY(cudaMemcpyAsync(&tot, flag.p, sizeof(double), cudaMemcpyDeviceToHost, stream));
		CUDA_TRY(cudaStreamSynchronize(stream));
		if ((int)(tot + 0.5) != world) {
			for (int r = 0; r < PCG5_MAXWORLD; r++) { if (peerBase[r] && r != rank) cudaIpcCloseMemHandle(peerBase[r]); peerBase[r] = nullptr; }
			return CUBA_OK;
		}
		mappedFor = localBase;
		ok = true;
		return CUBA_OK;
	}
	int p5Exchange(bool& ok) { return ipcExchange((void*)p5Boards.p, p5PeerBase, p5MappedFor, ok); }

	void* uPeerBase[PCG5_MAXWORLD] = { nullptr };
	void* uMappedFor = nullptr;
	bool uPeerOk = false;
	unsigned int uEpoch = 0;
	size_t uCount = 0;
	void uCloseMappings()
	{
		for (int r = 0; r < PCG5_MAXWORLD; r++) { if (uPeerBase[r] && r != rank) cudaIpcCloseMemHandle(uPeerBase[r]); uPeerBase[r] = nullptr; }
		uMappedFor = nullptr; uPeerOk = false;
	}
	int launch_peer_allreduce()
	{
		peer::Args<T> pa;
		pa.local = uVal.p; pa.n = uCount; pa.rank = rank; pa.world = world; pa.epoch = ++uEpoch; pa.bar = gridBar;
		const size_t sigOff = (uCount + 1) & ~(size_t)1;
		for (int r = 0; r < peer::MAXW; r++) { pa.peers[r] = nullptr; pa.sigPeer[r] = nullptr; }
		for (int r = 0; r < world; r++) { pa.peers[r] = (T*)uPeerBase[r]; pa.sigPeer[r] = (unsigned int*)((T*)uPeerBase[r] + sigOff); }
		pa.sigLocal = (unsigned int*)(uVal.p + sigOff);
		void* args[] = { (void*)&pa };
		CUDA_TRY(cudaLaunchCooperativeKernel((void*)peer::k_peer_allreduce<T>, dim3(numSMs), dim3(peer::BLOCK), args, 0, stream));
		launches++;
		return CUBA_OK;
	}

	int setup_pcg5()
	{
		p5Ok = false; p5Dist = false; p5CoarseValid = false; p5CoarseAge = 0;
		const int numP = S.numP;
		if (numP < 1) return CUBA_OK;
		const int mode = cfg.reserved[0];
		if (mode == 1 || mode == 2 || mode == 3 || mode == 4) return CUBA_OK;
		const bool wantDist = world > 1 && comm && mode != 7 && (mode == 8 || numP >= 2048);
		const int W = wantDist ? world : 1;
		int smemMax = 0;
		CUDA_TRY(cudaDeviceGetAttribute(&smemMax, cudaDevAttrMaxSharedMemoryPerBlockOptin, devOrdinal));
		const size_t budget = (size_t)smemMax > 4096 ? (size_t)smemMax - 2048 : 0;
		const int maxAgg = (cfg.reserved[6] > 0 && cfg.reserved[6] < PCG5_MAXAGG) ? cfg.reserved[6] : PCG5_MAXAGG;
		const bool tryTuned = W == 1 && !getenv("CUBA_PCG5_LEGACY");
		int apcTop = p5t::DEFAULT_APC;
		if (const char* e = getenv("CUBA_PCG5_AGGS_PER_CTA")) apcTop = std::min(3, std::max(1, atoi(e)));
		p5Tuned = false;
		Pcg5Plan plan;
		Pcg5Dims d{};
		int NR = 0;
		const size_t per = 36 * sizeof(T) + 4;
		size_t wantCache = 0;
		for (int apc = tryTuned ? apcTop : 1; apc >= 1 && !p5Tuned; apc--) {
			build_pcg5_plan(numP, S.nfull, S.fRowPtr, S.fColInd, W, numSMs, maxAgg, 2 * PCG5_BLOCK / 6, plan, &hostPP, apc);
			if (!plan.ok) continue;
			const int G = plan.G, nc = 6 * plan.A;
			const PcgPartition& PP = plan.P; const CoarsePartition& CP = plan.C;
			NR = 3 + 6 * (G / plan.gs);
			d = Pcg5Dims{};
			d.needMax = PP.needMax; d.maxRows = PP.maxRows; d.nc = nc; d.maxNeedAgg = CP.maxNeedAgg;
			d.npv = std::max(std::max(G * p5t::pcg5t_np(apc), W * NR), 6 * CP.maxNeedAgg); d.nls = NR;
			d.sliceRows = (nc + G - 1) / G;
			wantCache = PP.blkMax > PCG5_REGBLK ? (size_t)(PP.blkMax - PCG5_REGBLK) : 0;
			if (!tryTuned) break;
			using TS = p5t::Pcg5Shape;
			p5t::Pcg5Dims t{};
			t.needMax = PP.needMax; t.maxRows = PP.maxRows; t.nc = nc; t.maxNeedAgg = CP.maxNeedAgg;
			t.npv = d.npv; t.nls = NR; t.sliceRows = d.sliceRows;
			t.ccCap = PP.blkMax >= TS::CHUNK ? TS::CHUNK : std::max((std::max(PP.blkMax, PP.needMax) + 31) / 32 * 32, 32);
			t.sqWords = p5t::pcg5t_np(apc) * (TS::BLOCK / 32);
			t.capBlocks = 0; t.zhInSmem = 0;
			const size_t base = p5t::Pcg5Layout<T>(t).total + 64;
			const size_t zhBytes = (size_t)t.needMax * 36 * sizeof(T);
			size_t used = base + wantCache * per, cap = wantCache;
			if (used + zhBytes <= budget) { t.zhInSmem = 1; used += zhBytes; }
			if (apc > 1 && used > budget && base <= budget) { cap = std::min(wantCache, (budget - base) / per); used = base + cap * per; }
			if (PP.maxRows * 6 <= TS::BLOCK && used <= budget) {
				t.capBlocks = (int)cap;
				p5tDims = t;
				p5tDimsBJ = t; p5tDimsBJ.nc = 0; p5tDimsBJ.maxNeedAgg = 0; p5tDimsBJ.zhInSmem = 0; p5tDimsBJ.sliceRows = 0; p5tDimsBJ.nls = 3; p5tDimsBJ.npv = std::max(G * 3, W * 3);
				const size_t smemT = std::max(p5t::Pcg5Layout<T>(p5tDims).total, p5t::Pcg5Layout<T>(p5tDimsBJ).total);
				const void* fn = apc == 3 ? (const void*)p5t::k_pcg5t<T, 3> : apc == 2 ? (const void*)p5t::k_pcg5t<T, 2> : (const void*)p5t::k_pcg5t<T, 1>;
				int perSM = 0;
				if (smemT <= (size_t)smemMax - 1024 && cudaFuncSetAttribute(fn, cudaFuncAttributeMaxDynamicSharedMemorySize, (int)smemT) == cudaSuccess &&
					cudaOccupancyMaxActiveBlocksPerMultiprocessor(&perSM, fn, TS::BLOCK, smemT) == cudaSuccess && perSM >= 1) {
					p5Tuned = true; p5Big = false; p5Fn = fn; p5Block = TS::BLOCK; p5Smem = smemT;
					p5Dims = Pcg5Dims{}; p5Dims.capBlocks = t.capBlocks;
					d.capBlocks = t.capBlocks; d.zhInSmem = t.zhInSmem;
				} else cudaGetLastError();
			}
			if (!p5Tuned && apc == 1) break;
		}
		if (!plan.ok) return CUBA_OK;
		const int G = plan.G, gs = plan.gs, A = plan.A;
		const PcgPartition& PP = plan.P; const CoarsePartition& CP = plan.C;
		const std::vector<unsigned char>& peers = plan.rowPeers;
		const int nc = 6 * A;
		if (!p5Tuned) {
		bool big = PP.maxRows * 6 > PCG5_BLOCK;
		{
			d.capBlocks = 0; d.zhInSmem = 0;
			const size_t base = Pcg5Layout<T>(d).total + 64;
			if (base > budget) return CUBA_OK;
			const size_t zhBytes = (size_t)d.needMax * 36 * sizeof(T);
			size_t used = base + wantCache * per;
			if (used + zhBytes <= budget) { d.zhInSmem = 1; used += zhBytes; }
			const size_t fixed = used - wantCache * per;
			d.capBlocks = (int)std::min(wantCache, (budget - fixed) / per);
			if ((size_t)d.capBlocks < wantCache) big = true;
			if (big) d.capBlocks = (int)std::min((size_t)PP.blkMax, (budget - fixed) / per);
		}
		p5Dims = d;
		p5DimsBJ = d; p5DimsBJ.nc = 0; p5DimsBJ.maxNeedAgg = 0; p5DimsBJ.zhInSmem = 0; p5DimsBJ.sliceRows = 0; p5DimsBJ.nls = 3; p5DimsBJ.npv = std::max(G * 3, W * 3);
		p5Smem = std::max(Pcg5Layout<T>(p5Dims).total, Pcg5Layout<T>(p5DimsBJ).total);
		if (p5Smem > (size_t)smemMax - 1024) return CUBA_OK;
		p5Big = big;
		p5Fn = p5Big ? (const void*)k_pcg5<T, true> : (const void*)k_pcg5<T, false>;
		p5Block = PCG5_BLOCK;
		CUDA_TRY(cudaFuncSetAttribute(p5Fn, cudaFuncAttributeMaxDynamicSharedMemorySize, (int)p5Smem));
		int perSM = 0;
		if (p5Big) CUDA_TRY(cudaOccupancyMaxActiveBlocksPerMultiprocessor(&perSM, k_pcg5<T, true>, PCG5_BLOCK, p5Smem));
		else CUDA_TRY(cudaOccupancyMaxActiveBlocksPerMultiprocessor(&perSM, k_pcg5<T, false>, PCG5_BLOCK, p5Smem));
		if (perSM < 1) return CUBA_OK;
		}
		if (getenv("CUBA_PCG_VERBOSE")) fprintf(stderr, "pcg5: world %d G %d gs %d A %d aggsPerCta %d needMax %d maxRows %d blkMax %d maxNeedAgg %d zhInSmem %d sliceRows %d cap %d smem %zu\n",
			W, G, gs, A, plan.apc, d.needMax, d.maxRows, PP.blkMax, d.maxNeedAgg, d.zhInSmem, d.sliceRows, d.capBlocks, p5Smem);
		if (getenv("CUBA_PCG_VERBOSE")) fprintf(stderr, "pcg5: shape %s, %d threads\n", p5Big ? "big" : p5Tuned ? "tuned" : "legacy", p5Block);
		p5Dense = A > PCG4_MAXAGG1 && (A > PCG5_MAXAGG || !getenv("CUBA_COARSE_CLUSTER"));
		p5Cluster = A > PCG5_MAXAGG ? 0 : A > PCG4_MAXAGG1 ? (A > PCG4_MAXAGG ? 16 : 8) : 0;
		const size_t nblkPz = (size_t)A * (A + 1) / 2;
		if (A > PCG5_MAXAGG) p5InvSmem = 0;
		else if (p5Cluster) {
			const size_t nloc = (nblkPz + p5Cluster - 1) / p5Cluster;
			p5InvSmem = nloc * 36 * sizeof(double) + 2 * nloc + 16;
		} else p5InvSmem = (nblkPz + 2 * (size_t)A) * 36 * sizeof(double);
		if (p5InvSmem + 1024 > (size_t)smemMax) return CUBA_OK;
		if (p5Cluster == 16) {
			CUDA_TRY(cudaFuncSetAttribute(k_coarse_chol_cluster2<16>, cudaFuncAttributeMaxDynamicSharedMemorySize, (int)p5InvSmem));
			CUDA_TRY(cudaFuncSetAttribute(k_coarse_chol_cluster2<16>, cudaFuncAttributeNonPortableClusterSizeAllowed, 1));
		} else if (p5Cluster == 8) CUDA_TRY(cudaFuncSetAttribute(k_coarse_chol_cluster2<8>, cudaFuncAttributeMaxDynamicSharedMemorySize, (int)p5InvSmem));
		else if (!p5Dense) CUDA_TRY(cudaFuncSetAttribute(k_coarse_invert<T>, cudaFuncAttributeMaxDynamicSharedMemorySize, (int)std::max(p5InvSmem, (!pcg4Cluster && pcg4Ok) ? pcg4InvSmem : 0)));
		if (p5Cluster && (size_t)A * 36 * sizeof(double) > 48 * 1024) CUDA_TRY(cudaFuncSetAttribute(k_coarse_trinv, cudaFuncAttributeMaxDynamicSharedMemorySize, (int)((size_t)A * 36 * sizeof(double))));
		CUDA_TRY(p5CtaRow.upload(PP.rows, stream, arena)); CUDA_TRY(p5NeedPtr.upload(PP.nptr, stream, arena)); CUDA_TRY(p5NeedCol.upload(PP.ncol, stream, arena));
		CUDA_TRY(p5Local.upload(PP.local, stream, arena)); CUDA_TRY(p5RowPeers.upload(peers, stream, arena));
		CUDA_TRY(p5AggRow.upload(CP.aggRow, stream, arena)); CUDA_TRY(p5NaPtr.upload(CP.naPtr, stream, arena)); CUDA_TRY(p5NaList.upload(CP.naList, stream, arena));
		CUDA_TRY(p5NeedAgg.upload(CP.needAgg, stream, arena)); CUDA_TRY(p5CbPtr.upload(CP.cbPtr, stream, arena)); CUDA_TRY(p5CbList.upload(CP.cbList, stream, arena));
		CUDA_TRY(cRowOf.upload(CP.rowOf, stream, arena));
		const size_t nP = (size_t)numP;
		CUDA_TRY(p5Linv.alloc(36 * nP)); CUDA_TRY(p5R0.alloc(6 * nP)); CUDA_TRY(p5Zhat.alloc(36 * nP)); CUDA_TRY(p5RcRow.alloc(6 * nP)); CUDA_TRY(p5Rc0.alloc(std::max(nc, 1)));
		CUDA_TRY(cZx.alloc(36 * nP)); CUDA_TRY(cU.alloc(36 * (size_t)S.nfull)); CUDA_TRY(cInfo.alloc(1 + P5_INFO_LOG));
		CUDA_TRY(cudaMemsetAsync(cInfo.p, 0, sizeof(int) * cInfo.n, stream));
		CUDA_TRY(fHat.alloc(36 * (size_t)S.nfull));
		CUDA_TRY(p5AcP.alloc(nblkPz * 36)); CUDA_TRY(p5AcInv.alloc((size_t)nc * nc)); CUDA_TRY(p5Lp.alloc(nblkPz * 36)); CUDA_TRY(p5Wp.alloc(nblkPz * 36)); CUDA_TRY(p5Ld.alloc((size_t)A * 36));
		if (p5Dense) {
			const size_t ntd = ((size_t)nc + cdense::NB - 1) / cdense::NB, npd = ntd * cdense::NB;
			CUDA_TRY(cdM.alloc(npd * npd)); CUDA_TRY(cdL.alloc(npd * npd)); CUDA_TRY(cdW.alloc(npd * npd)); CUDA_TRY(cdDinv.alloc(ntd * cdense::NB * cdense::NB));
			CUDA_TRY(gridBar.alloc(1));
		}
		const size_t wW = 4 * 6 * nP, pW = 4 * (size_t)PCG5_REPL * G * p5t::pcg5t_np(plan.apc), rW = 4 * (size_t)PCG5_REPL * W * NR, cW = 4 * (size_t)PCG5_REPL * nc;
		const size_t words2 = 2 * (wW + pW + rW + cW) + (sizeof(Pcg5Ctl) + 7) / 8 + 2;
		const bool fresh = !p5Boards.p || words2 > p5Boards.cap || wW != p5WWords || pW != p5PWords || rW != p5RWords || cW != p5CWords;
		if (fresh) {
			if (p5MappedFor) { CUDA_TRY(cudaStreamSynchronize(stream)); p5CloseMappings(); }
			CUDA_TRY(p5Boards.alloc(std::max(words2, (size_t)(1u << 18))));
			CUDA_TRY(cudaMemsetAsync(p5Boards.p, 0, sizeof(unsigned long long) * p5Boards.cap, stream));
			p5WWords = wW; p5PWords = pW; p5RWords = rW; p5CWords = cW;
			p5TagBound = 0;
		}
		p5G = G; p5W = W; p5A = A; p5Gs = gs; p5Apc = plan.apc;
		if (W > 1) {
			bool ok = false;
			int rc = p5Exchange(ok); if (rc) return rc;
			if (!ok) {
				if (rank == 0) fprintf(stderr, "cuba_b200: cudaIpc mapping of the peers' PCG boards failed; keeping the replicated PCG\n");
				return CUBA_OK;
			}
			p5Dist = true;
		} else p5PeerBase[rank] = (void*)p5Boards.p;
		p5Ok = true;
		return CUBA_OK;
	}

	int launch_coarse_setup(int A, int cluster, size_t invSmem, const int* cbPtr, const int* cbList, double* AcP, float* AcInv, double* Lp, double* Ld, double* Wp, bool dense = false)
	{
		const int nblkP = A * (A + 1) / 2;
		int* infoP = p5InfoSlot();
		KLAUNCH(k_coarse_project<T>, 36LL * S.nfull, fVal.p, cRowOf.p, fColInd.p, S.nfull, cZx.p, cU.p);
		KLAUNCH(k_coarse_assemble, (long long)nblkP * 36, cbPtr, cbList, cU.p, nblkP, AcP);
		if (dense) {
			CUDA_TRY(cudaMemsetAsync(cdM.p, 0, sizeof(double) * cdM.n, stream));
			cdense::Args da;
			da.AcP = AcP; da.A = A; da.M = cdM; da.Lm = cdL; da.Dinv = cdDinv; da.W = cdW; da.AcInv = AcInv; da.info = infoP; da.bar = gridBar;
			void* dargs[] = { (void*)&da };
			CUDA_TRY(cudaLaunchCooperativeKernel((void*)cdense::k_coarse_dense, dim3(numSMs), dim3(cdense::WARPS * 32), dargs, 0, stream));
			launches++;
			return CUBA_OK;
		}
		if (cluster) {
			cudaLaunchConfig_t lc = {};
			lc.gridDim = dim3(cluster); lc.blockDim = dim3(1024); lc.dynamicSmemBytes = invSmem; lc.stream = stream;
			cudaLaunchAttribute at[1];
			at[0].id = cudaLaunchAttributeClusterDimension; at[0].val.clusterDim.x = cluster; at[0].val.clusterDim.y = 1; at[0].val.clusterDim.z = 1;
			lc.attrs = at; lc.numAttrs = 1;
			if (cluster == 16) CUDA_TRY(cudaLaunchKernelEx(&lc, k_coarse_chol_cluster2<16>, (const double*)AcP, A, Lp, Ld, AcInv, infoP));
			else CUDA_TRY(cudaLaunchKernelEx(&lc, k_coarse_chol_cluster2<8>, (const double*)AcP, A, Lp, Ld, AcInv, infoP));
			k_coarse_trinv<<<A, 256, (size_t)A * 36 * sizeof(double), stream>>>(Lp, Ld, A, Wp, infoP);
			k_coarse_wtw<<<(nblkP * 36 + 255) / 256, 256, 0, stream>>>(Wp, A, AcInv, infoP);
			launches += 2;
		}
		else k_coarse_invert<T><<<1, 1024, invSmem, stream>>>(AcP, A, AcInv, infoP);
		launches++;
		CUDA_TRY(cudaGetLastError());
		return CUBA_OK;
	}

	int launch_pcg5(bool twoLevel)
	{
		ProfScope ps(this, CUBA_PROF_DECOMP_NUMERICAL);
		const int numP = S.numP, A = twoLevel ? p5A : 0;
		const int maxIters = cfg.pcg_max_iters > 0 ? cfg.pcg_max_iters : std::max(200, 40 * numP);
		p5TagBound += (long long)maxIters + 8;
		if (p5TagBound > (1LL << 31)) {
			if (p5Dist) { int rc0 = allreduce(&dScal.p->v[7], 1, false); if (rc0) return rc0; }
			CUDA_TRY(cudaMemsetAsync(p5Boards.p, 0, sizeof(unsigned long long) * p5Boards.cap, stream));
			if (p5Dist) { int rc0 = allreduce(&dScal.p->v[7], 1, false); if (rc0) return rc0; }
			p5TagBound = (long long)maxIters + 8;
		}
		if (twoLevel) KLAUNCH(k_coarse_basis<T>, numP, pose[cur].p, numP, cZx.p);
		Pcg5PrepArgs<T> pa;
		pa.fRowPtr = fRowPtr; pa.fColInd = fColInd; pa.fVal = fVal; pa.b = bsc; pa.Zx = cZx; pa.numP = numP; pa.A = A; pa.aggRow = p5AggRow;
		pa.Linv = p5Linv; pa.R0 = p5R0; pa.Zhat = p5Zhat; pa.rcRow = p5RcRow; pa.rc0 = p5Rc0; pa.ctl = p5Ctl(p5Boards.p);
		k_pcg5_prep_rows<T><<<(numP + 127) / 128, 128, 0, stream>>>(pa);
		launches++;
		if (twoLevel) {
			k_pcg5_prep_rc<T><<<(6 * A + 127) / 128, 128, 0, stream>>>(pa);
			launches++;
			const int refreshEvery = cfg.reserved[4] > 0 ? cfg.reserved[4] : 8;
			const double lamRatio = (p5CoarseValid && p5CoarseLambda > 0 && curLambda > 0) ? std::max(curLambda / p5CoarseLambda, p5CoarseLambda / curLambda) : 1.0;
			if (!p5CoarseValid || p5CoarseAge >= refreshEvery || lamRatio > 300.0) {
				int rc = launch_coarse_setup(A, p5Cluster, p5InvSmem, p5CbPtr, p5CbList, p5AcP, p5AcInv, p5Lp, p5Ld, p5Wp, p5Dense); if (rc) return rc;
				p5CoarseValid = true; p5CoarseAge = 0; p5CoarseLambda = curLambda; p5Rebuilds++;
			}
			p5CoarseAge++;
		}
		CUDA_TRY(cudaGetLastError());
		auto fill = [&](auto& a) {
			using CtlPtr = decltype(a.ctl);
			a.fRowPtr = fRowPtr; a.fColInd = fColInd; a.fLocal = p5Local; a.fVal = fVal; a.fHat = fHat;
			a.ctaRow = p5CtaRow; a.needPtr = p5NeedPtr; a.needCol = p5NeedCol;
			a.numP = numP; a.G = p5G; a.rank = p5Dist ? rank : 0; a.world = p5W;
			a.Linv = p5Linv; a.R0 = p5R0; a.Zhat = p5Zhat; a.rc0 = p5Rc0; a.x = xp;
			a.maxIters = maxIters;
			const double tol = cfg.pcg_tol > 0 ? cfg.pcg_tol : (sizeof(T) == 8 ? 1e-11 : 1e-6);
			a.tol2 = tol * tol;
			a.status = &dScal.p->pcg;
			a.AcInv = p5AcInv; a.naPtr = p5NaPtr; a.naList = p5NaList; a.needAgg = p5NeedAgg; a.A = A; a.gs = p5Gs;
			for (int r = 0; r < PCG5_MAXWORLD; r++) { a.peerW[r] = nullptr; a.peerR[r] = nullptr; a.peerCtl[r] = nullptr; }
			for (int r = 0; r < p5W; r++) {
				unsigned long long* base = (unsigned long long*)p5PeerBase[p5Dist ? r : rank];
				a.peerW[r] = base; a.peerR[r] = base + 2 * (p5WWords + p5PWords); a.peerCtl[r] = reinterpret_cast<CtlPtr>(p5Ctl(base));
			}
			a.wBoard = p5Boards.p; a.pBoard = p5Boards.p + 2 * p5WWords; a.rBoard = p5Boards.p + 2 * (p5WWords + p5PWords);
			a.cBoard = p5Boards.p + 2 * (p5WWords + p5PWords + p5RWords);
			a.rowPeers = p5RowPeers; a.ctl = reinterpret_cast<CtlPtr>(p5Ctl(p5Boards.p));
			a.timing = nullptr;
		};
#ifdef CUBA_PCG_TIMING
		CUDA_TRY(pcgTiming.alloc(8 * (size_t)p5G));
#endif
		if (p5Dist) CUDA_TRY(cudaMemsetAsync(xp.p, 0, sizeof(T) * 6 * (size_t)numP, stream));
		Pcg5Args<T> a;
		p5t::Pcg5Args<T> at;
		void* args[1];
		if (p5Tuned) {
			fill(at);
			at.aggRow = p5AggRow;
			at.dims = twoLevel ? p5tDims : p5tDimsBJ;
			at.dims.capBlocks = p5tDims.capBlocks;
#ifdef CUBA_PCG_TIMING
			at.timing = pcgTiming.p;
#endif
			args[0] = (void*)&at;
		} else {
			fill(a);
			a.dims = twoLevel ? p5Dims : p5DimsBJ;
			a.dims.capBlocks = p5Dims.capBlocks;
#ifdef CUBA_PCG_TIMING
			a.timing = pcgTiming.p;
#endif
			args[0] = (void*)&a;
		}
		CUDA_TRY(cudaLaunchCooperativeKernel(p5Fn, dim3(p5G), dim3(p5Block), args, p5Smem, stream));
		k_pcg5_commit<<<1, 1, 0, stream>>>(p5Ctl(p5Boards.p));
		launches += 2;
		CUDA_TRY(cudaGetLastError());
		if (p5Dist) { int rc = allreduce(xp.p, 6 * (size_t)numP, true); if (rc) return rc; }
		lastPcgTwoLevel = twoLevel;
		lastPcgKernel = p5Tuned ? CUBA_PCG_KERNEL_PCG5T : p5Big ? CUBA_PCG_KERNEL_PCG5_BIG : CUBA_PCG_KERNEL_PCG5;
		return CUBA_OK;
	}

	int launch_pcg()
	{
		lastPcgTwoLevel = false;
		{
			const int m = cfg.reserved[0];
			const bool two = tlActive && !forceBlockJacobi;
			if (p5Ok && (m == 5 || m == 6)) return launch_pcg5(m == 5 && !forceBlockJacobi);
			if (p5Ok && (m == 0 || m == 7 || m == 8) && (p5Dist || two)) return launch_pcg5(two);
			if ((m == 0 || m == 7 || m == 8) && !(pcg4Ok && two)) return launch_pcg2(pcg3Ok);
			if ((m == 0 || m == 7 || m == 8) && pcg4Ok && two) return launch_pcg4();
		}
		if (pcg4Ok && cfg.reserved[0] == 3 && !forceBlockJacobi) return launch_pcg4();
		if (cfg.reserved[0] == 0 || cfg.reserved[0] == 3 || cfg.reserved[0] == 4) return launch_pcg2(pcg3Ok);
		if (cfg.reserved[0] == 2) return launch_pcg2(false);
		ProfScope ps(this, CUBA_PROF_DECOMP_NUMERICAL);
		PcgArgs<T> a;
		a.fRowPtr = fRowPtr; a.fColInd = fColInd; a.fVal = fVal; a.b = bsc; a.numP = S.numP;
		a.x = xp; a.r = pr; a.z = pz; a.q = pq; a.p0 = pp0; a.p1 = pp1; a.Minv = Minv; a.partial = pcgPartial;
		a.maxIters = cfg.pcg_max_iters > 0 ? cfg.pcg_max_iters : std::max(200, 40 * S.numP);
		const double tol = cfg.pcg_tol > 0 ? cfg.pcg_tol : (sizeof(T) == 8 ? 1e-11 : 1e-6);
		a.tol2 = tol * tol;
		a.status = &dScal.p->pcg;
		void* args[] = { (void*)&a };
		CUDA_TRY(cudaLaunchCooperativeKernel((void*)k_pcg<T>, dim3(pcgGrid), dim3(PCG_BLOCK), args, 0, stream));
		launches++;
		lastPcgKernel = CUBA_PCG_KERNEL_PCG;
		return CUBA_OK;
	}

	int launch_backsub(T lambda)
	{
		ProfScope ps(this, CUBA_PROF_SCHUR_COMPLEMENT);
		if (ntiles > 0 && S.numL > 0) {
			BacksubArgs<T> a;
			a.Hpl = Hpl; a.invHll = invHll; a.bl = bl; a.xp = xp; a.ip = e_ip; a.hpl = e_hpl; a.lmPtr = tilePtr; a.tileLm = tileLm;
			a.numL = S.numL; a.lambda = lambda; a.XwCur = Xw[cur]; a.XwTrial = Xw[cur ^ 1]; a.xl = xl; a.scalePartial = scalePartialL;
			if (mixed) {
				if constexpr (sizeof(T) == 8) {
					BacksubArgs<double, float> m;
					m.Hpl = HplF; m.invHll = invHll; m.bl = bl; m.xp = xp; m.ip = e_ip; m.hpl = e_hpl; m.lmPtr = tilePtr; m.tileLm = tileLm;
					m.numL = S.numL; m.lambda = lambda; m.XwCur = Xw[cur]; m.XwTrial = Xw[cur ^ 1]; m.xl = xl; m.scalePartial = scalePartialL;
					if (tileSize == 128) k_backsub<double, 128, float><<<ntiles, 128, 0, stream>>>(m);
					else k_backsub<double, 256, float><<<ntiles, 256, 0, stream>>>(m);
				}
			}
			else if (tileSize == 128) k_backsub<T, 128><<<ntiles, 128, 0, stream>>>(a);
			else k_backsub<T, 256><<<ntiles, 256, 0, stream>>>(a);
			launches++;
			CUDA_TRY(cudaGetLastError());
		}
		return CUBA_OK;
	}

	int stage_solve(double lambda, int* iters, int* ok) override
	{
		if (!haveProblem) return fail(CUBA_ERR_STATE, "solve before set_problem");
		const T lam = (T)lambda;
		curLambda = lambda;
		int rc = launch_schur(lam); if (rc) return rc;
		int nScaleL = 0;
		if (S.numP > 0 && S.numL > 0) {
			rc = launch_pcg(); if (rc) return rc;
			rc = launch_backsub(lam); if (rc) return rc;
			nScaleL = ntiles;
		} else if (S.numP > 0) {
			k_solve_poses_only<T><<<(S.numP + 127) / 128, 128, 0, stream>>>(Hpp, bp, S.numP, lam, xp);
			launches++;
			CUDA_TRY(cudaGetLastError());
			hScal->pcg.iters = 0; hScal->pcg.status = 0;
			lastPcgKernel = CUBA_PCG_KERNEL_NONE;
		} else if (S.numL > 0) {
			nScaleL = (S.numL + RED_BLOCK - 1) / RED_BLOCK;
			k_solve_landmarks_only<T><<<nScaleL, RED_BLOCK, 0, stream>>>(invHll, bl, S.numL, lam, Xw[cur], Xw[cur ^ 1], xl, scalePartialL);
			launches++;
			CUDA_TRY(cudaGetLastError());
		}
		nScaleLandmark = nScaleL;
		solvedLambda = lambda;
		if (iters || ok) {
			rc = fetchScalars(); if (rc) return rc;
			const bool usedPcg = S.numP > 0 && S.numL > 0;
			if (usedPcg) note_pcg_iters(hScal->pcg.iters);
			if (iters) *iters = usedPcg ? hScal->pcg.iters : 0;
			if (ok) *ok = usedPcg ? (hScal->pcg.status == 0) : 1;
		}
		return CUBA_OK;
	}
	int nScaleLandmark = 0;
	double solvedLambda = 0;

	int stage_update(double lambda, double* chi, double* scale) override
	{
		if (!haveProblem) return fail(CUBA_ERR_STATE, "update before set_problem");
		const T lam = (T)lambda;
		{
			ProfScope ps(this, CUBA_PROF_UPDATE);
			if (S.numP > 0) {
				k_update_poses<T><<<nPoseBlocks, RED_BLOCK, 0, stream>>>(xp, bp, S.numP, lam, pose[cur], pose[cur ^ 1], scalePartialP);
				launches++;
				CUDA_TRY(cudaGetLastError());
			}
		}
		int rc = launch_chi2(cur ^ 1, 1, false); if (rc) return rc;
		rc = launch_sum(scalePartialL, nScaleLandmark, scalePartialP, S.numP > 0 ? nPoseBlocks : 0, nullptr, 0, 2); if (rc) return rc;
		if (world > 1) { rc = allreduce(&dScal.p->v[1], 2, false); if (rc) return rc; }
		rc = fetchScalars(); if (rc) return rc;
		trialValid = true;
		if (chi) *chi = hScal->v[1];
		if (scale) *scale = hScal->v[2] + hScal->v[3];
		return CUBA_OK;
	}

	int stage_commit(int accept) override
	{
		if (!trialValid) return fail(CUBA_ERR_STATE, "commit without a trial state");
		if (accept) cur ^= 1;
		trialValid = false;
		return CUBA_OK;
	}

	int optimize(int niter, cuba_iter_stat* stats, int* nstats) override
	{
		if (!haveProblem) return fail(CUBA_ERR_STATE, "optimize before set_problem");
		const int maxq = 10;
		const double tau = 1e-5;
		double nu = 2, lambda = 0, F = 0;
		int n = 0;
		tlActive = false; coarseValid = false; coarseAge = 0;
		p5CoarseValid = false; p5CoarseAge = 0; forceBlockJacobi = false;
		bool haveF = false;
		for (int it = 0; it < niter; it++) {
			double chi0 = 0;
			int rc = stage_linearize(&chi0); if (rc) return rc;
			if (!haveF) F = chi0;
			F = chi0; haveF = true;
			if (it == 0) {
				double md = 0;
				rc = stage_max_diagonal(&md); if (rc) return rc;
				lambda = tau * md;
			}
			int q = 0, trials = 0, pcgIters = 0, pcgFailed = 0;
			double rho = -1;
			for (; q < maxq && rho < 0; q++) {
				trials++;
				int iters = 0, ok = 1;
				double Fhat = 0, scale = 0;
				for (int attempt = 0; attempt < 2; attempt++) {
					rc = stage_solve(lambda, nullptr, nullptr); if (rc) return rc;
					rc = stage_update(lambda, &Fhat, &scale); if (rc) return rc;
					if (!(S.numP > 0 && S.numL > 0)) break;
					const PcgStatus& ps = hScal->pcg;
					iters += ps.iters;
					if (ps.status == 3) return fail(CUBA_ERR_COMM, "PCG: a CTA or a peer GPU stopped answering (flag exchange timed out)");
					const double loose = sizeof(T) == 8 ? 1e-6 : 1e-3;
					ok = ps.status == 0 || (ps.status == 1 && ps.rz0 > 0 && ps.rz <= loose * loose * ps.rz0);
					if (ps.status == 2 && lastPcgTwoLevel && attempt == 0) {
						forceBlockJacobi = true; coarseValid = false; p5CoarseValid = false; bjRetries++;
						rc = stage_commit(0); if (rc) return rc;
						continue;
					}
					break;
				}
				forceBlockJacobi = false;
				if (S.numP > 0 && S.numL > 0) note_pcg_iters(hScal->pcg.iters);
				pcgIters += iters; if (!ok) pcgFailed++;
				scale += 1e-3;
				rho = ok ? (F - Fhat) / scale : -1;
				if (!(rho == rho)) rho = -1;
				if (rho > 0) {
					const double a = 2 * rho - 1;
					lambda *= std::max(1. / 3, std::min(1 - a * a * a, 2. / 3));
					nu = 2; F = Fhat;
					rc = stage_commit(1); if (rc) return rc;
					break;
				} else {
					lambda *= nu; nu *= 2;
					rc = stage_commit(0); if (rc) return rc;
				}
			}
			if (stats) {
				stats[n].iteration = it; stats[n].trials = trials; stats[n].chi2 = F; stats[n].lambda = lambda;
				stats[n].pcg_iters = pcgIters; stats[n].pcg_failed = pcgFailed;
			}
			n++;
			if (q == maxq || rho <= 0 || !std::isfinite(lambda)) break;
		}
		if (nstats) *nstats = n;
		resolveProfile();
		return CUBA_OK;
	}

	int get_state(double* q, double* t, double* X) override
	{
		if (!haveProblem) return fail(CUBA_ERR_STATE, "get_state before set_problem");
		std::vector<T> hp((size_t)S.Pall * 8), hx((size_t)S.Lall * 4);
		g_d2hBytes += (long long)(sizeof(T) * (hp.size() + hx.size()));
		CUDA_TRY(cudaMemcpyAsync(hp.data(), pose[cur].p, sizeof(T) * hp.size(), cudaMemcpyDeviceToHost, stream));
		if (world > 1 && comm && S.numL > 0) {
			T* tmp = Xw[cur ^ 1].p;
			trialValid = false;
			CUDA_TRY(cudaMemcpyAsync(tmp, Xw[cur].p, sizeof(T) * 4 * (size_t)S.Lall, cudaMemcpyDeviceToDevice, stream));
			if (shardBoundValid) {
				const int dt = sizeof(T) == 8 ? NCCL_FLOAT64 : NCCL_FLOAT32;
				g_nccl.GroupStart();
				int rcn = 0;
				for (int r = 0; r < world; r++) {
					const int b0 = std::min(shardBound[r], S.numL), b1 = std::min(shardBound[r + 1], S.numL);
					if (b1 > b0) rcn |= g_nccl.Broadcast(tmp + 4 * (size_t)b0, tmp + 4 * (size_t)b0, 4 * (size_t)(b1 - b0), dt, r, comm, stream);
				}
				rcn |= g_nccl.GroupEnd();
				if (rcn != 0) return fail(CUBA_ERR_COMM, "ncclBroadcast (landmark gather) failed");
			} else {
				CUDA_TRY(cudaMemsetAsync(tmp, 0, sizeof(T) * 4 * (size_t)S.Lall, stream));
				if (S.lmEnd > S.lmBeg)
					CUDA_TRY(cudaMemcpyAsync(tmp + 4 * (size_t)S.lmBeg, Xw[cur].p + 4 * (size_t)S.lmBeg, sizeof(T) * 4 * (size_t)(S.lmEnd - S.lmBeg), cudaMemcpyDeviceToDevice, stream));
				int rc = allreduce(tmp, 4 * (size_t)S.Lall, true); if (rc) return rc;
			}
			CUDA_TRY(cudaMemcpyAsync(hx.data(), tmp, sizeof(T) * hx.size(), cudaMemcpyDeviceToHost, stream));
			CUDA_TRY(cudaStreamSynchronize(stream));
		} else {
			CUDA_TRY(cudaMemcpyAsync(hx.data(), Xw[cur].p, sizeof(T) * hx.size(), cudaMemcpyDeviceToHost, stream));
			CUDA_TRY(cudaStreamSynchronize(stream));
		}
		for (int i = 0; i < S.Pall; i++) {
			if (q) for (int k = 0; k < 4; k++) q[4 * (size_t)i + k] = (double)hp[8 * (size_t)i + k];
			if (t) for (int k = 0; k < 3; k++) t[3 * (size_t)i + k] = (double)hp[8 * (size_t)i + 4 + k];
		}
		if (X) for (int i = 0; i < S.Lall; i++) for (int k = 0; k < 3; k++) X[3 * (size_t)i + k] = (double)hx[4 * (size_t)i + k];
		return CUBA_OK;
	}

	int get_chi2(double* out) override
	{
		if (!haveProblem) return fail(CUBA_ERR_STATE, "get_chi2 before set_problem");
		CUDA_TRY(cudaMemsetAsync(chiSq.p, 0, sizeof(double) * (size_t)std::max(S.E, 1), stream));
		if (S.eLocal > 0) {
			k_chi_sqs<T><<<(S.eLocal + 255) / 256, 256, 0, stream>>>(chiArgs(cur), e_user, chiSq);
			launches++;
			CUDA_TRY(cudaGetLastError());
		}
		if (world > 1) { int rc = allreduce(chiSq.p, (size_t)S.E, false); if (rc) return rc; }
		g_d2hBytes += (long long)(sizeof(double) * (size_t)S.E);
		CUDA_TRY(cudaMemcpyAsync(out, chiSq.p, sizeof(double) * (size_t)S.E, cudaMemcpyDeviceToHost, stream));
		CUDA_TRY(cudaStreamSynchronize(stream));
		return CUBA_OK;
	}

	int get_profile(double* sec) override
	{
		resolveProfile();
		for (int i = 0; i < CUBA_PROF_NUM; i++) sec[i] = prof[i];
		return CUBA_OK;
	}

	int dbg_hpl_structure(int32_t* colPtr, int32_t* rowInd, int32_t* e2h) override
	{
		if (!haveProblem) return fail(CUBA_ERR_STATE, "no problem");
		{ const int rc0 = ensureHostStructure(); if (rc0) return rc0; }
		if (colPtr) memcpy(colPtr, S.hplColPtr.data(), sizeof(int) * S.hplColPtr.size());
		if (rowInd) memcpy(rowInd, S.hplRowInd.data(), sizeof(int) * S.hplRowInd.size());
		if (e2h) memcpy(e2h, S.edge2Hpl.data(), sizeof(int) * S.edge2Hpl.size());
		return CUBA_OK;
	}
	int dbg_hsc_structure(int32_t* rowPtr, int32_t* colInd) override
	{
		if (!haveProblem) return fail(CUBA_ERR_STATE, "no problem");
		{ const int rc0 = ensureHostStructure(); if (rc0) return rc0; }
		if (rowPtr) memcpy(rowPtr, S.hscRowPtr.data(), sizeof(int) * S.hscRowPtr.size());
		if (colInd) memcpy(colInd, S.hscColInd.data(), sizeof(int) * S.hscColInd.size());
		return CUBA_OK;
	}
	int download(const T* d, size_t n, double* out)
	{
		std::vector<T> h(n);
		CUDA_TRY(cudaMemcpyAsync(h.data(), d, sizeof(T) * n, cudaMemcpyDeviceToHost, stream));
		CUDA_TRY(cudaStreamSynchronize(stream));
		for (size_t i = 0; i < n; i++) out[i] = (double)h[i];
		return CUBA_OK;
	}
	int dbg_system(double* oHpp, double* obp, double* oHll, double* obl, double* oHpl) override
	{
		if (!haveProblem) return fail(CUBA_ERR_STATE, "no problem");
		int rc;
		if (oHpp && (rc = download(Hpp, 36 * (size_t)S.numP, oHpp))) return rc;
		if (obp && (rc = download(bp, 6 * (size_t)S.numP, obp))) return rc;
		if (oHll && (rc = download(Hll, 9 * (size_t)S.numL, oHll))) return rc;
		if (obl && (rc = download(bl, 3 * (size_t)S.numL, obl))) return rc;
		if (oHpl) {
			memset(oHpl, 0, sizeof(double) * 18 * (size_t)S.nhpl);
			if (mixed) {
				std::vector<float> hf(20 * (size_t)S.nhplLocal);
				CUDA_TRY(cudaMemcpyAsync(hf.data(), HplF.p, sizeof(float) * hf.size(), cudaMemcpyDeviceToHost, stream));
				CUDA_TRY(cudaStreamSynchronize(stream));
				for (size_t b = 0; b < (size_t)S.nhplLocal; b++) for (int e = 0; e < 18; e++) oHpl[18 * ((size_t)S.hplBase + b) + e] = (double)hf[20 * b + e];
			}
			else if ((rc = download(Hpl, 18 * (size_t)S.nhplLocal, oHpl + 18 * (size_t)S.hplBase))) return rc;
		}
		return CUBA_OK;
	}
	int dbg_schur(double* oHsc, double* obsc, double* oinv) override
	{
		if (!haveProblem) return fail(CUBA_ERR_STATE, "no problem");
		int rc;
		if ((rc = ensureHostStructure())) return rc;
		if (oHsc) {
			std::vector<double> full(36 * (size_t)S.nfull);
			if ((rc = download(fVal, full.size(), full.data()))) return rc;
			for (int k = 0; k < S.nblk; k++) memcpy(oHsc + 36 * (size_t)k, full.data() + 36 * (size_t)S.u2f[k], sizeof(double) * 36);
		}
		if (obsc && (rc = download(bsc, 6 * (size_t)S.numP, obsc))) return rc;
		if (oinv && (rc = download(invHll, 9 * (size_t)S.numL, oinv))) return rc;
		return CUBA_OK;
	}
	int dbg_delta(double* oxp, double* oxl) override
	{
		if (!haveProblem) return fail(CUBA_ERR_STATE, "no problem");
		int rc;
		if (oxp && (rc = download(xp, 6 * (size_t)S.numP, oxp))) return rc;
		if (oxl && (rc = download(xl, 3 * (size_t)S.numL, oxl))) return rc;
		return CUBA_OK;
	}

	int dbg_pcg_timing(long long* out, int maxCtas) override
	{
		const int n = std::min(maxCtas, pcg2Grid);
		if (!pcgTiming.p || n <= 0) return 0;
		cudaMemcpyAsync(out, pcgTiming.p, sizeof(long long) * 8 * (size_t)n, cudaMemcpyDeviceToHost, stream);
		cudaStreamSynchronize(stream);
		return n;
	}

	int dbg_pcg_info(int32_t* info, double* coarseLambda) override
	{
		if (!haveProblem) return fail(CUBA_ERR_STATE, "no problem");
		CUDA_TRY(cudaStreamSynchronize(stream));
		PcgStatus ps{};
		CUDA_TRY(cudaMemcpy(&ps, &dScal.p->pcg, sizeof(ps), cudaMemcpyDeviceToHost));
		int last = -1, bad = 0;
		if (p5Ok && p5A > 0 && p5Rebuilds > 0) {
			const int nlog = (int)std::min<long long>(p5Rebuilds, P5_INFO_LOG);
			std::vector<int> log(nlog);
			CUDA_TRY(cudaMemcpy(log.data(), cInfo.p + 1, sizeof(int) * nlog, cudaMemcpyDeviceToHost));
			for (int v : log) if (v != 0) bad++;
			last = log[(int)((p5Rebuilds - 1) % P5_INFO_LOG)];
		}
		int coarseKernel = CUBA_COARSE_KERNEL_NONE;
		if (lastPcgTwoLevel && lastPcgKernel == CUBA_PCG_KERNEL_PCG4) coarseKernel = pcg4Cluster ? CUBA_COARSE_KERNEL_PCG4_CLUSTER : CUBA_COARSE_KERNEL_INVERT;
		else if (lastPcgTwoLevel && p5Ok)
			coarseKernel = p5Dense ? CUBA_COARSE_KERNEL_DENSE : p5Cluster == 16 ? CUBA_COARSE_KERNEL_CLUSTER16 : p5Cluster == 8 ? CUBA_COARSE_KERNEL_CLUSTER8 : CUBA_COARSE_KERNEL_INVERT;
		const bool tuned = p5Ok && p5Tuned;
		const int32_t v[CUBA_PCG_INFO_LEN] = {
			lastPcgKernel, lastPcgKernel != CUBA_PCG_KERNEL_NONE && lastPcgTwoLevel ? 1 : 0,
			p5Ok ? p5Apc : 0, p5Ok ? p5G : 0, p5Ok ? p5Gs : 0, p5Ok ? p5A : 0,
			p5Ok ? (tuned ? p5tDims.maxRows : p5Dims.maxRows) : 0, p5Ok ? (tuned ? p5tDims.capBlocks : p5Dims.capBlocks) : 0,
			p5Ok ? (tuned ? p5tDims.zhInSmem : p5Dims.zhInSmem) : 0,
			coarseKernel, last, ps.status, ps.iters, (int32_t)p5Rebuilds, (int32_t)bjRetries, bad };
		if (info) memcpy(info, v, sizeof(v));
		if (coarseLambda) *coarseLambda = p5CoarseValid ? p5CoarseLambda : 0.0;
		return CUBA_OK;
	}
	int dbg_coarse(int32_t* rowAgg, double* oAcP, float* oAcInv) override
	{
		if (!haveProblem) return fail(CUBA_ERR_STATE, "no problem");
		if (!p5Ok || p5A < 1 || !p5CoarseValid) return fail(CUBA_ERR_STATE, "debug_get_coarse: no coarse level of k_pcg5 has been built");
		const int A = p5A, nc = 6 * A;
		CUDA_TRY(cudaStreamSynchronize(stream));
		if (rowAgg) {
			std::vector<int> ptr(A + 1);
			CUDA_TRY(cudaMemcpy(ptr.data(), p5AggRow.p, sizeof(int) * (A + 1), cudaMemcpyDeviceToHost));
			for (int i = 0; i < S.numP; i++) rowAgg[i] = -1;
			for (int ag = 0; ag < A; ag++) for (int i = ptr[ag]; i < ptr[ag + 1] && i < S.numP; i++) rowAgg[i] = ag;
		}
		if (oAcP) CUDA_TRY(cudaMemcpy(oAcP, p5AcP.p, sizeof(double) * 36 * ((size_t)A * (A + 1) / 2), cudaMemcpyDeviceToHost));
		if (oAcInv) CUDA_TRY(cudaMemcpy(oAcInv, p5AcInv.p, sizeof(float) * (size_t)nc * nc, cudaMemcpyDeviceToHost));
		return CUBA_OK;
	}

	int bench_stage(int stage, int reps, int flush, double lambda, double* ms) override
	{
		if (!haveProblem) return fail(CUBA_ERR_STATE, "bench before set_problem");
		if (reps < 1) reps = 1;
		const size_t flushN = (size_t)40 << 20;
		if (flush) CUDA_TRY(flushBuf.alloc(flushN));
		cudaEvent_t a, b;
		CUDA_TRY(cudaEventCreate(&a)); CUDA_TRY(cudaEventCreate(&b));
		double total = 0;
		const T lam = (T)lambda;
		for (int r = 0; r < reps; r++) {
			if (flush) { k_fill<<<numSMs * 8, 256, 0, stream>>>(flushBuf.p, flushN, (double)r); launches++; }
			CUDA_TRY(cudaEventRecord(a, stream));
			int rc = CUBA_OK;
			switch (stage) {
			case 0: rc = launch_linearize_landmark(); if (!rc) rc = launch_linearize_pose(); break;
			case 1: rc = launch_linearize_landmark(); break;
			case 2: rc = launch_linearize_pose(); break;
			case 3: rc = launch_schur(lam); break;
			case 4: curLambda = lambda; rc = launch_pcg(); break;
			case 5: rc = launch_backsub(lam); if (!rc) rc = stage_update_nofetch(lam); break;
			case 6: rc = launch_chi2(cur, 0); break;
			case 7:
				if (!p5Ok || p5A < 1) rc = fail(CUBA_ERR_STATE, "bench_stage: no two-level k_pcg5 plan");
				else rc = launch_coarse_setup(p5A, p5Cluster, p5InvSmem, p5CbPtr, p5CbList, p5AcP, p5AcInv, p5Lp, p5Ld, p5Wp, p5Dense);
				break;
			default: rc = fail(CUBA_ERR_INVALID, "bench_stage: unknown stage");
			}
			if (rc) return rc;
			CUDA_TRY(cudaEventRecord(b, stream));
			CUDA_TRY(cudaEventSynchronize(b));
			float t = 0;
			CUDA_TRY(cudaEventElapsedTime(&t, a, b));
			total += t;
		}
		cudaEventDestroy(a); cudaEventDestroy(b);
		resolveProfile();
		if (ms) *ms = total / reps;
		return CUBA_OK;
	}
	int stage_update_nofetch(T lam)
	{
		if (S.numP > 0) {
			k_update_poses<T><<<nPoseBlocks, RED_BLOCK, 0, stream>>>(xp, bp, S.numP, lam, pose[cur], pose[cur ^ 1], scalePartialP);
			launches++;
			CUDA_TRY(cudaGetLastError());
		}
		return launch_chi2(cur ^ 1, 1);
	}
};

}

using namespace cuba_b200;

struct cuba_engine { std::unique_ptr<EngineBase> impl; };

extern "C" {

const char* cuba_last_error(void) { return g_err.c_str(); }
int cuba_version(void) { return 100; }

int cuba_engine_create(const cuba_config* cfg, cuba_engine** out)
{
	if (!out) return fail(CUBA_ERR_INVALID, "create: null out");
	cuba_config c;
	memset(&c, 0, sizeof(c));
	c.device = -1; c.deterministic = 1;
	if (cfg) c = *cfg;
	std::unique_ptr<EngineBase> impl;
	int rc;
	if (c.use_fp32 == 1) { auto* e = new Engine<float>(); e->cfg = c; impl.reset(e); rc = e->init(); }
	else { auto* e = new Engine<double>(); e->cfg = c; impl.reset(e); rc = e->init(); }
	if (rc) return rc;
	if (getenv("CUBA_NO_STRUCTURE_REUSE")) impl->structureReuse = false;
	*out = new cuba_engine{ std::move(impl) };
	return CUBA_OK;
}

int cuba_engine_destroy(cuba_engine* e) { delete e; return CUBA_OK; }

#define ENGINE_OR_FAIL(e) if (!(e) || !(e)->impl) return fail(CUBA_ERR_INVALID, "null engine"); DevGuard _devGuard((e)->impl->devOrdinal)

int cuba_engine_set_robust_kernel(cuba_engine* e, int edge_type, int kernel_type, double delta)
{
	ENGINE_OR_FAIL(e);
	if (edge_type < 0 || edge_type > 1 || kernel_type < 0 || kernel_type > 2) return fail(CUBA_ERR_INVALID, "set_robust_kernel: bad type");
	e->impl->rk_type[edge_type] = kernel_type; e->impl->rk_delta[edge_type] = delta;
	return CUBA_OK;
}

int cuba_comm_unique_id(void* out128)
{
	std::string why;
	if (!g_nccl.load(why)) return fail(CUBA_ERR_COMM, why);
	Nccl::UniqueId id;
	const int rc = g_nccl.GetUniqueId(&id);
	if (rc) return fail(CUBA_ERR_COMM, "ncclGetUniqueId failed");
	memcpy(out128, &id, 128);
	return CUBA_OK;
}

int cuba_engine_set_comm(cuba_engine* e, int rank, int world, const void* uid)
{
	ENGINE_OR_FAIL(e);
	if (world < 1 || rank < 0 || rank >= world || world > PCG5_MAXWORLD) return fail(CUBA_ERR_INVALID, "set_comm: bad rank/world (at most 8 ranks)");
	if (e->impl->haveProblem) return fail(CUBA_ERR_STATE, "set_comm must precede set_problem");
	e->impl->rank = rank; e->impl->world = world;
	if (world == 1) return CUBA_OK;
	if (getenv("CUBA_DRY_SHARD")) return CUBA_OK;
	if (!uid) return fail(CUBA_ERR_INVALID, "set_comm: null unique id");
	std::string why;
	if (!g_nccl.load(why)) return fail(CUBA_ERR_COMM, why);
	Nccl::UniqueId id;
	memcpy(&id, uid, 128);
	const int rc = g_nccl.CommInitRank(&e->impl->comm, world, id, rank);
	if (rc) return fail(CUBA_ERR_COMM, std::string("ncclCommInitRank failed: ") + (g_nccl.GetErrorString ? g_nccl.GetErrorString(rc) : "?"));
	return CUBA_OK;
}

int cuba_engine_set_problem(cuba_engine* e, const cuba_problem* p) { ENGINE_OR_FAIL(e); return e->impl->set_problem(p); }
int cuba_engine_set_structure_reuse(cuba_engine* e, int enable) { ENGINE_OR_FAIL(e); e->impl->structureReuse = enable != 0; return CUBA_OK; }
int cuba_engine_get_structure_reuses(cuba_engine* e, long long* count) { ENGINE_OR_FAIL(e); if (count) *count = e->impl->structureReuses; return CUBA_OK; }
int cuba_engine_set_state(cuba_engine* e, const double* q, const double* t, const double* Xw)
{
	ENGINE_OR_FAIL(e);
	if (!q || !t || !Xw) return fail(CUBA_ERR_INVALID, "set_state: null array");
	return e->impl->set_state(q, t, Xw);
}
int cuba_engine_reset_state(cuba_engine* e) { ENGINE_OR_FAIL(e); return e->impl->reset_state(); }
int cuba_engine_get_stream(cuba_engine* e, void** s) { ENGINE_OR_FAIL(e); if (!s) return fail(CUBA_ERR_INVALID, "null out"); return e->impl->get_stream(s); }
int cuba_engine_flush_l2(cuba_engine* e) { ENGINE_OR_FAIL(e); return e->impl->flush_l2(); }
int cuba_engine_get_sizes(const cuba_engine* e, cuba_sizes* out) { ENGINE_OR_FAIL(e); if (!out) return fail(CUBA_ERR_INVALID, "null out"); return e->impl->get_sizes(out); }
int cuba_engine_optimize(cuba_engine* e, int niter, cuba_iter_stat* stats, int* nstats) { ENGINE_OR_FAIL(e); return e->impl->optimize(niter, stats, nstats); }
int cuba_engine_get_state(cuba_engine* e, double* q, double* t, double* Xw) { ENGINE_OR_FAIL(e); return e->impl->get_state(q, t, Xw); }
int cuba_engine_get_chi2(cuba_engine* e, double* per_edge) { ENGINE_OR_FAIL(e); if (!per_edge) return fail(CUBA_ERR_INVALID, "null out"); return e->impl->get_chi2(per_edge); }
int cuba_engine_get_profile(cuba_engine* e, double* sec) { ENGINE_OR_FAIL(e); if (!sec) return fail(CUBA_ERR_INVALID, "null out"); return e->impl->get_profile(sec); }
int cuba_debug_get_pcg_timing(cuba_engine* e, long long* out, int maxCtas)
{
	if (!e || !e->impl) return -1;
	DevGuard guard(e->impl->devOrdinal);
	return e->impl->dbg_pcg_timing(out, maxCtas);
}
int cuba_get_transfer_bytes(long long* h2d, long long* d2h) { if (h2d) *h2d = g_h2dBytes; if (d2h) *d2h = g_d2hBytes; return CUBA_OK; }
int cuba_engine_get_launch_count(cuba_engine* e, long long* count) { ENGINE_OR_FAIL(e); if (count) *count = e->impl->launches; return CUBA_OK; }

int cuba_stage_linearize(cuba_engine* e, double* chi2) { ENGINE_OR_FAIL(e); return e->impl->stage_linearize(chi2); }
int cuba_stage_max_diagonal(cuba_engine* e, double* md) { ENGINE_OR_FAIL(e); return e->impl->stage_max_diagonal(md); }
int cuba_stage_solve(cuba_engine* e, double lambda, int* iters, int* ok)
{
	ENGINE_OR_FAIL(e);
	int it = 0, k = 1;
	const int rc = e->impl->stage_solve(lambda, &it, &k);
	if (iters) *iters = it;
	if (ok) *ok = k;
	return rc;
}
int cuba_stage_update(cuba_engine* e, double lambda, double* chi, double* scale) { ENGINE_OR_FAIL(e); return e->impl->stage_update(lambda, chi, scale); }
int cuba_stage_commit(cuba_engine* e, int accept) { ENGINE_OR_FAIL(e); return e->impl->stage_commit(accept); }
int cuba_stage_chi2(cuba_engine* e, double* chi) { ENGINE_OR_FAIL(e); return e->impl->stage_chi2(chi); }

int cuba_debug_get_hpl_structure(cuba_engine* e, int32_t* colPtr, int32_t* rowInd, int32_t* e2h) { ENGINE_OR_FAIL(e); return e->impl->dbg_hpl_structure(colPtr, rowInd, e2h); }
int cuba_debug_get_hsc_structure(cuba_engine* e, int32_t* rowPtr, int32_t* colInd) { ENGINE_OR_FAIL(e); return e->impl->dbg_hsc_structure(rowPtr, colInd); }
int cuba_debug_get_system(cuba_engine* e, double* Hpp, double* bp, double* Hll, double* bl, double* Hpl) { ENGINE_OR_FAIL(e); return e->impl->dbg_system(Hpp, bp, Hll, bl, Hpl); }
int cuba_debug_get_schur(cuba_engine* e, double* Hsc, double* bsc, double* invHll) { ENGINE_OR_FAIL(e); return e->impl->dbg_schur(Hsc, bsc, invHll); }
int cuba_debug_get_delta(cuba_engine* e, double* xp, double* xl) { ENGINE_OR_FAIL(e); return e->impl->dbg_delta(xp, xl); }
int cuba_debug_get_pcg_info(cuba_engine* e, int32_t* info, double* coarse_lambda) { ENGINE_OR_FAIL(e); return e->impl->dbg_pcg_info(info, coarse_lambda); }
int cuba_debug_get_coarse(cuba_engine* e, int32_t* aggRow, double* AcP, float* AcInv) { ENGINE_OR_FAIL(e); return e->impl->dbg_coarse(aggRow, AcP, AcInv); }
int cuba_debug_build_structure_host(const cuba_problem* p, int rank, int world, cuba_sizes* sizes,
	int32_t* hplColPtr, int32_t* hplRowInd, int32_t* edge2Hpl, int32_t* hscRowPtr, int32_t* hscColInd,
	int32_t* fullRowPtr, int32_t* fullColInd, int32_t* shard)
{
	if (!p) return fail(CUBA_ERR_INVALID, "null problem");
	Structure S;
	const char* err = "";
	if (!build_structure(p->Pall, p->numP, p->Lall, p->numL, p->E2, p->idx2, p->E3, p->idx3, rank, world, TILE, S, &err))
		return fail(CUBA_ERR_INVALID, err);
	if (sizes) {
		sizes->Pall = S.Pall; sizes->numP = S.numP; sizes->Lall = S.Lall; sizes->numL = S.numL; sizes->E2 = S.E2; sizes->E3 = S.E3;
		sizes->nhpl = S.nhpl; sizes->nblk = S.nblk; sizes->nmul = (int32_t)S.nmul; sizes->nblk_full = S.nfull;
	}
	auto cp = [](int32_t* dst, const std::vector<int>& v) { if (dst && !v.empty()) memcpy(dst, v.data(), sizeof(int) * v.size()); };
	cp(hplColPtr, S.hplColPtr); cp(hplRowInd, S.hplRowInd); cp(edge2Hpl, S.edge2Hpl);
	cp(hscRowPtr, S.hscRowPtr); cp(hscColInd, S.hscColInd); cp(fullRowPtr, S.fRowPtr); cp(fullColInd, S.fColInd);
	if (shard) { shard[0] = S.lmBeg; shard[1] = S.lmEnd; shard[2] = S.eLocal; shard[3] = (int32_t)S.nmulLocal; }
	if ((int)S.tileLm.size() < 1 || S.tileLm.front() != S.lmBeg || S.tileLm.back() != S.lmEnd) return fail(CUBA_ERR_INVALID, "structure self-check: tiles");
	for (size_t t = 0; t + 1 < S.tileLm.size(); t++) {
		const int nl = S.tileLm[t + 1] - S.tileLm[t];
		const int ne = S.lmPtr[S.tileLm[t + 1]] - S.lmPtr[S.tileLm[t]];
		if (nl < 1 || nl > TILE || (ne > TILE && nl != 1)) return fail(CUBA_ERR_INVALID, "structure self-check: tile size");
	}
	for (int k = 0; k < S.nblk; k++)
		for (int n = S.prodPtr[k]; n < S.prodPtr[k + 1]; n++) {
			const int i = S.prodI[n] + S.hplBase, j = S.prodJ[n] + S.hplBase;
			if (S.hplRowInd[i] != S.blkRow[k] || S.hplRowInd[j] != S.blkCol[k] || S.hplLm[S.prodI[n]] != S.hplLm[S.prodJ[n]] || i > j)
				return fail(CUBA_ERR_INVALID, "structure self-check: product list");
		}
	return CUBA_OK;
}

int cuba_debug_pcg_partition(const cuba_problem* p, int nCtas, int maxAgg, int32_t* info)
{
	if (!p || nCtas < 1 || maxAgg < 1) return fail(CUBA_ERR_INVALID, "pcg_partition: bad arguments");
	Structure S;
	const char* err = "";
	if (!build_structure(p->Pall, p->numP, p->Lall, p->numL, p->E2, p->idx2, p->E3, p->idx3, 0, 1, TILE, S, &err)) return fail(CUBA_ERR_INVALID, err);
	if (S.numP < 1) return fail(CUBA_ERR_INVALID, "pcg_partition: no free pose");
	const int G = std::max(1, std::min(nCtas, S.numP));
	PcgPartition P; CoarsePartition C;
	build_pcg_partition(S.numP, S.nfull, S.fRowPtr, S.fColInd, G, P);
	build_coarse_partition(S.numP, P, maxAgg, C);
	build_coarse_lists(S.numP, S.nfull, S.fRowPtr, S.fColInd, C);
	const char* bad = check_pcg_partition(S.numP, S.nfull, S.fRowPtr, S.fColInd, P, C);
	if (bad) return fail(CUBA_ERR_INVALID, std::string("pcg_partition self-check: ") + bad);
	if (info) { info[0] = P.G; info[1] = C.gs; info[2] = C.A; info[3] = P.needMax; info[4] = P.maxRows; info[5] = P.blkMax; info[6] = C.maxNeedAgg; info[7] = (int32_t)C.cbList.size(); }
	return CUBA_OK;
}

int cuba_debug_pcg5_plan(const cuba_problem* p, int world, int numSMs, int maxAgg, int32_t* info)
{
	return cuba_debug_pcg5_plan_apc(p, world, numSMs, maxAgg, 1, info, nullptr);
}

int cuba_debug_pcg5_plan_apc(const cuba_problem* p, int world, int numSMs, int maxAgg, int aggsPerCta, int32_t* info, uint64_t* hash)
{
	if (!p || world < 1 || world > 8 || numSMs < 1 || maxAgg < 1 || aggsPerCta < 1 || aggsPerCta > 3) return fail(CUBA_ERR_INVALID, "pcg5_plan: bad arguments");
	Structure S;
	const char* err = "";
	if (!build_structure(p->Pall, p->numP, p->Lall, p->numL, p->E2, p->idx2, p->E3, p->idx3, 0, 1, TILE, S, &err)) return fail(CUBA_ERR_INVALID, err);
	Pcg5Plan plan;
	build_pcg5_plan(S.numP, S.nfull, S.fRowPtr, S.fColInd, world, numSMs, maxAgg, 2 * PCG5_BLOCK / 6, plan, nullptr, aggsPerCta);
	if (info) for (int i = 0; i < 8; i++) info[i] = 0;
	if (hash) *hash = 0;
	if (!plan.ok) return CUBA_OK;
	const char* bad = check_pcg5_plan(S.numP, S.nfull, S.fRowPtr, S.fColInd, plan);
	if (bad) return fail(CUBA_ERR_INVALID, std::string("pcg5_plan self-check: ") + bad);
	if (info) {
		int halo = 0;
		for (unsigned char m : plan.rowPeers) if (m) halo++;
		info[0] = 1; info[1] = plan.G; info[2] = plan.gs; info[3] = plan.A; info[4] = plan.P.needMax; info[5] = plan.P.maxRows; info[6] = plan.C.maxNeedAgg; info[7] = halo;
	}
	if (hash) {
		uint64_t h = 1469598103934665603ull;
		auto mix = [&h](const void* data, size_t bytes) {
			const unsigned char* b = (const unsigned char*)data;
			for (size_t i = 0; i < bytes; i++) { h ^= b[i]; h *= 1099511628211ull; }
		};
		auto vec = [&mix](const std::vector<int>& v) { const uint64_t n = v.size(); mix(&n, sizeof n); mix(v.data(), v.size() * sizeof(int)); };
		const int scal[] = { plan.G, plan.gs, plan.A, plan.P.needMax, plan.P.blkMax, plan.P.maxRows, plan.C.maxNeedAgg };
		mix(scal, sizeof scal);
		for (const std::vector<int>* v : { &plan.P.rows, &plan.P.nptr, &plan.P.ncol, &plan.P.local, &plan.C.aggRow, &plan.C.rowAgg, &plan.C.naPtr,
			&plan.C.naList, &plan.C.needAgg, &plan.C.rowOf, &plan.C.cbPtr, &plan.C.cbList }) vec(*v);
		mix(plan.rowPeers.data(), plan.rowPeers.size());
		*hash = h;
	}
	return CUBA_OK;
}

int cuba_bench_stage(cuba_engine* e, int stage, int reps, int flush, double lambda, double* ms) { ENGINE_OR_FAIL(e); return e->impl->bench_stage(stage, reps, flush, lambda, ms); }

}
```

### cuda-bundle-adjustment_b200/csrc/cuba_math.cuh

```cuda
#pragma once

#include <math.h>

#if defined(__CUDACC__)
#define CUBA_HD __host__ __device__ __forceinline__
#else
#define CUBA_HD inline
#endif

namespace cuba_b200 {

enum { RK_NONE = 0, RK_HUBER = 1, RK_TUKEY = 2 };

template <typename T> CUBA_HD T t_sqrt(T x);
template <> CUBA_HD double t_sqrt<double>(double x) { return sqrt(x); }
template <> CUBA_HD float t_sqrt<float>(float x) { return sqrtf(x); }
template <typename T> CUBA_HD T t_sin(T x);
template <> CUBA_HD double t_sin<double>(double x) { return sin(x); }
template <> CUBA_HD float t_sin<float>(float x) { return sinf(x); }
template <typename T> CUBA_HD T t_cos(T x);
template <> CUBA_HD double t_cos<double>(double x) { return cos(x); }
template <> CUBA_HD float t_cos<float>(float x) { return cosf(x); }

template <typename T>
CUBA_HD void rotate(const T q[4], const T X[3], T Xc[3])
{
	T a0 = q[1] * X[2] - q[2] * X[1];
	T a1 = q[2] * X[0] - q[0] * X[2];
	T a2 = q[0] * X[1] - q[1] * X[0];
	a0 += a0; a1 += a1; a2 += a2;
	const T b0 = q[1] * a2 - q[2] * a1;
	const T b1 = q[2] * a0 - q[0] * a2;
	const T b2 = q[0] * a1 - q[1] * a0;
	Xc[0] = X[0] + q[3] * a0 + b0;
	Xc[1] = X[1] + q[3] * a1 + b1;
	Xc[2] = X[2] + q[3] * a2 + b2;
}

template <typename T>
CUBA_HD void robust(int type, T delta, T e, T& rho, T& drho)
{
	const T d2 = delta * delta;
	if (type == RK_HUBER) {
		if (e <= d2) { rho = e; drho = T(1); }
		else { const T s = t_sqrt(e); rho = 2 * s * delta - d2; drho = delta / s; }
	} else if (type == RK_TUKEY) {
		const T maxv = (T(1) / 3) * d2;
		if (e <= d2) { const T u = 1 - e / d2; rho = maxv * (1 - u * u * u); drho = u * u; }
		else { rho = maxv; drho = T(0); }
	} else { rho = e; drho = T(1); }
}

template <typename T>
CUBA_HD void edge_residual(const T q[4], const T t[3], const T cam[5], const T Xw[3], const T m[3], bool stereo,
	T Xc[3], T r[3])
{
	rotate(q, Xw, Xc);
	Xc[0] += t[0]; Xc[1] += t[1]; Xc[2] += t[2];
	const T invZ = 1 / Xc[2];
	const T u = cam[0] * invZ * Xc[0] + cam[2];
	const T v = cam[1] * invZ * Xc[1] + cam[3];
	r[0] = u - m[0];
	r[1] = v - m[1];
	r[2] = stereo ? ((u - cam[4] * invZ) - m[2]) : T(0);
}

template <typename T>
CUBA_HD void edge_jacobians(const T q[4], const T cam[5], const T Xc[3], bool stereo, T JP[3][6], T JL[3][3])
{
	const T x = q[0], y = q[1], z = q[2], w = q[3];
	const T tx = 2 * x, ty = 2 * y, tz = 2 * z;
	const T twx = tx * w, twy = ty * w, twz = tz * w;
	const T txx = tx * x, txy = ty * x, txz = tz * x;
	const T tyy = ty * y, tyz = tz * y, tzz = tz * z;
	const T R00 = 1 - (tyy + tzz), R01 = txy - twz, R02 = txz + twy;
	const T R10 = txy + twz, R11 = 1 - (txx + tzz), R12 = tyz - twx;
	const T R20 = txz - twy, R21 = tyz + twx, R22 = 1 - (txx + tyy);

	const T invZ = 1 / Xc[2];
	const T xn = invZ * Xc[0], yn = invZ * Xc[1];
	const T fu = cam[0], fv = cam[1];
	const T fuZ = fu * invZ, fvZ = fv * invZ;

	JL[0][0] = -fuZ * (R00 - xn * R20); JL[0][1] = -fuZ * (R01 - xn * R21); JL[0][2] = -fuZ * (R02 - xn * R22);
	JL[1][0] = -fvZ * (R10 - yn * R20); JL[1][1] = -fvZ * (R11 - yn * R21); JL[1][2] = -fvZ * (R12 - yn * R22);

	JP[0][0] = fu * xn * yn;       JP[0][1] = -fu * (1 + xn * xn); JP[0][2] = fu * yn;
	JP[0][3] = -fuZ;               JP[0][4] = T(0);                JP[0][5] = fuZ * xn;
	JP[1][0] = fv * (1 + yn * yn); JP[1][1] = -fv * xn * yn;       JP[1][2] = -fv * xn;
	JP[1][3] = T(0);               JP[1][4] = -fvZ;                JP[1][5] = fvZ * yn;

	if (stereo) {
		const T bZZ = cam[4] * invZ * invZ;
		JL[2][0] = JL[0][0] - bZZ * R20; JL[2][1] = JL[0][1] - bZZ * R21; JL[2][2] = JL[0][2] - bZZ * R22;
		JP[2][0] = JP[0][0] - bZZ * Xc[1]; JP[2][1] = JP[0][1] + bZZ * Xc[0]; JP[2][2] = JP[0][2];
		JP[2][3] = JP[0][3];               JP[2][4] = T(0);                   JP[2][5] = JP[0][5] - bZZ;
	} else {
#pragma unroll
		for (int i = 0; i < 3; i++) JL[2][i] = T(0);
#pragma unroll
		for (int i = 0; i < 6; i++) JP[2][i] = T(0);
	}
}

template <typename T>
CUBA_HD void sym3_inverse(T A00, T A01, T A02, T A11, T A12, T A22, T B[6] )
{
	const T det = A00 * A11 * A22 + A01 * A12 * A02 + A02 * A01 * A12 - A00 * A12 * A12 - A02 * A11 * A02 - A01 * A01 * A22;
	const T id = 1 / det;
	B[0] = id * (A11 * A22 - A12 * A12);
	B[1] = id * (A02 * A12 - A01 * A22);
	B[2] = id * (A01 * A12 - A02 * A11);
	B[3] = id * (A00 * A22 - A02 * A02);
	B[4] = id * (A02 * A01 - A00 * A12);
	B[5] = id * (A00 * A11 - A01 * A01);
}

template <typename T>
CUBA_HD bool spd6_inverse(T A[36])
{
	T L[36];
#pragma unroll
	for (int i = 0; i < 36; i++) L[i] = T(0);
	for (int j = 0; j < 6; j++) {
		T d = A[j * 6 + j];
		for (int k = 0; k < j; k++) d -= L[k * 6 + j] * L[k * 6 + j];
		if (!(d > T(0))) return false;
		d = t_sqrt(d);
		L[j * 6 + j] = d;
		const T id = 1 / d;
		for (int i = j + 1; i < 6; i++) {
			T s = A[j * 6 + i];
			for (int k = 0; k < j; k++) s -= L[k * 6 + i] * L[k * 6 + j];
			L[j * 6 + i] = s * id;
		}
	}
	T Li[36];
#pragma unroll
	for (int i = 0; i < 36; i++) Li[i] = T(0);
	for (int j = 0; j < 6; j++) {
		Li[j * 6 + j] = 1 / L[j * 6 + j];
		for (int i = j + 1; i < 6; i++) {
			T s = T(0);
			for (int k = j; k < i; k++) s -= L[k * 6 + i] * Li[j * 6 + k];
			Li[j * 6 + i] = s / L[i * 6 + i];
		}
	}
	for (int j = 0; j < 6; j++)
		for (int i = 0; i <= j; i++) {
			T s = T(0);
			for (int k = j; k < 6; k++) s += Li[i * 6 + k] * Li[j * 6 + k];
			A[j * 6 + i] = s; A[i * 6 + j] = s;
		}
	return true;
}

template <typename T>
CUBA_HD void se3_update(const T upd[6], T q[4], T t[3])
{
	const T wx = upd[0], wy = upd[1], wz = upd[2];
	const T theta = t_sqrt(wx * wx + wy * wy + wz * wz);
	T a1, a2, a3;
	if (theta < T(0.00001)) { a1 = T(1); a2 = T(0.5); a3 = T(1) / 6; }
	else {
		a1 = t_sin(theta) / theta;
		a2 = (1 - t_cos(theta)) / (theta * theta);
		a3 = (theta - t_sin(theta)) / (theta * theta * theta);
	}
	const T O1[3][3] = { { T(0), -wz, wy }, { wz, T(0), -wx }, { -wy, wx, T(0) } };
	const T xx = wx * wx, yy = wy * wy, zz = wz * wz, xy = wx * wy, yz = wy * wz, zx = wz * wx;
	const T O2[3][3] = { { -yy - zz, xy, zx }, { xy, -zz - xx, yz }, { zx, yz, -xx - yy } };
	T R[3][3], V[3][3];
#pragma unroll
	for (int i = 0; i < 3; i++)
#pragma unroll
		for (int j = 0; j < 3; j++) {
			const T I = (i == j) ? T(1) : T(0);
			R[i][j] = I + a1 * O1[i][j] + a2 * O2[i][j];
			V[i][j] = I + a2 * O1[i][j] + a3 * O2[i][j];
		}
	T eq[4];
	T tr = R[0][0] + R[1][1] + R[2][2];
	if (tr > T(0)) {
		tr = t_sqrt(tr + 1);
		eq[3] = T(0.5) * tr; tr = T(0.5) / tr;
		eq[0] = (R[2][1] - R[1][2]) * tr; eq[1] = (R[0][2] - R[2][0]) * tr; eq[2] = (R[1][0] - R[0][1]) * tr;
	} else {
		int i = 0;
		if (R[1][1] > R[0][0]) i = 1;
		if (R[2][2] > R[i][i]) i = 2;
		const int j = (i + 1) % 3, k = (j + 1) % 3;
		tr = t_sqrt(R[i][i] - R[j][j] - R[k][k] + 1);
		eq[i] = T(0.5) * tr; tr = T(0.5) / tr;
		eq[3] = (R[k][j] - R[j][k]) * tr; eq[j] = (R[j][i] + R[i][j]) * tr; eq[k] = (R[k][i] + R[i][k]) * tr;
	}
	T et[3];
#pragma unroll
	for (int i = 0; i < 3; i++) et[i] = V[i][0] * upd[3] + V[i][1] * upd[4] + V[i][2] * upd[5];
	T u[3];
	rotate(eq, t, u);
#pragma unroll
	for (int i = 0; i < 3; i++) t[i] = et[i] + u[i];
	T r[4];
	r[3] = eq[3] * q[3] - eq[0] * q[0] - eq[1] * q[1] - eq[2] * q[2];
	r[0] = eq[3] * q[0] + eq[0] * q[3] + eq[1] * q[2] - eq[2] * q[1];
	r[1] = eq[3] * q[1] + eq[1] * q[3] + eq[2] * q[0] - eq[0] * q[2];
	r[2] = eq[3] * q[2] + eq[2] * q[3] + eq[0] * q[1] - eq[1] * q[0];
	T invn = 1 / t_sqrt(r[0] * r[0] + r[1] * r[1] + r[2] * r[2] + r[3] * r[3]);
	if (r[3] < T(0)) invn = -invn;
#pragma unroll
	for (int i = 0; i < 4; i++) q[i] = invn * r[i];
}

}
```

### cuda-bundle-adjustment_b200/csrc/cuba_schur5.cuh

```cuda
#pragma once

#include "cuba_schur2.cuh"

namespace cuba_b200 {
namespace schur5 {

constexpr int TL = 512;
constexpr int BS = 21;
constexpr int WINDOW = 448;
constexpr int WARPS = 8;

struct Smem {
	double V[TL * BS];
	double zero[2];
	double L[TL * 6];
	int lm[TL];
};

__device__ __forceinline__ void dmma884(double& c0, double& c1, double a, double b)
{
	asm volatile("mma.sync.aligned.m8n8k4.row.col.f64.f64.f64.f64 {%0, %1}, {%2}, {%3}, {%0, %1};" : "+d"(c0), "+d"(c1) : "d"(a), "d"(b));
}

__device__ __forceinline__ void chol3(const double B[6], double L[6])
{
	L[0] = sqrt(B[0]);
	const double i0 = 1.0 / L[0];
	L[1] = B[1] * i0; L[2] = B[2] * i0;
	L[3] = sqrt(B[3] - L[1] * L[1]);
	L[4] = (B[4] - L[2] * L[1]) / L[3];
	L[5] = sqrt(B[5] - L[2] * L[2] - L[4] * L[4]);
}

__global__ void k_seg_records(const int* __restrict__ segStart, const int* __restrict__ segDest, const int* __restrict__ segRank, const int* __restrict__ segTile,
	const int* __restrict__ blkRow, const int* __restrict__ blkCol, const TileInfo* __restrict__ info, const int* __restrict__ p2i, const int* __restrict__ p2j,
	int nseg, int4* rec)
{
	const int s = blockIdx.x * blockDim.x + threadIdx.x;
	if (s >= nseg) return;
	const int k = segDest[s], h0 = info[segTile[s]].h0;
	int flags = blkRow[k] == blkCol[k] ? 1 : 0;
	for (int n = segStart[s]; n < segStart[s + 1]; n++) if (p2i[n] - h0 >= TL || p2j[n] - h0 >= TL) { flags |= 2; break; }
	rec[s] = make_int4(segStart[s], segStart[s + 1] - segStart[s], segRank[s], flags);
}
__global__ void k_prod_offsets(const int* __restrict__ segStart, const int* __restrict__ segTile, const TileInfo* __restrict__ info,
	const int* __restrict__ p2i, const int* __restrict__ p2j, int nseg, int nprod, unsigned int* off)
{
	const int n = blockIdx.x * blockDim.x + threadIdx.x;
	if (n >= nprod) return;
	int lo = 0, hi = nseg - 1;
	while (lo < hi) { const int mid = (lo + hi + 1) >> 1; if (segStart[mid] <= n) lo = mid; else hi = mid - 1; }
	const int h0 = info[segTile[lo]].h0;
	const int bi = p2i[n] - h0, bj = p2j[n] - h0;
	const unsigned int oi = bi < TL ? (unsigned)(bi * BS) : 0u, oj = bj < TL ? (unsigned)(bj * BS) : 0u;
	off[n] = oi | (oj << 16);
}

struct Args {
	const double* Hpl; const double* Hll; const double* bl;
	const TileInfo* info; const int* hplLm;
	const int* tileSegPtr; const int4* segRec; const unsigned int* off; const int* p2i; const int* p2j;
	int numL; double lambda;
	double* invHll; double* partial;
};

__global__ void __launch_bounds__(WARPS * 32, 2) k_schur_tiles_mma(const Args a)
{
	extern __shared__ __align__(16) unsigned char smem_raw[];
	Smem& sm = *reinterpret_cast<Smem*>(smem_raw);
	const int tid = threadIdx.x, lane = tid & 31, wid = tid >> 5, t = blockIdx.x;
	const TileInfo ti = a.info[t];
	const int nb = ti.h1 - ti.h0;
	int nl = ti.l1 - ti.l0;
	if (ti.l0 + nl > a.numL) nl = a.numL - ti.l0;
	const int nbs = nb < TL ? nb : TL;
	for (int i = tid; i < nbs * 9; i += WARPS * 32) {
		double x, y;
		ld2(a.Hpl + 18 * (size_t)ti.h0 + 2 * i, x, y);
		const int b = i / 9, e = 2 * (i - 9 * b);
		sm.V[BS * b + e] = x; sm.V[BS * b + e + 1] = y;
	}
	for (int i = tid; i < nbs; i += WARPS * 32) sm.lm[i] = a.hplLm[ti.h0 + i] - ti.l0;
	if (tid < 2) sm.zero[tid] = 0.0;
	for (int j = tid; j < nl; j += WARPS * 32) {
		const double* H = a.Hll + 9 * (size_t)(ti.l0 + j);
		double B[6];
		sym3_inverse<double>(H[0] + a.lambda, H[3], H[6], H[4] + a.lambda, H[7], H[8] + a.lambda, B);
		double* o = a.invHll + 9 * (size_t)(ti.l0 + j);
		o[0] = B[0]; o[1] = B[1]; o[2] = B[2]; o[3] = B[1]; o[4] = B[3]; o[5] = B[4]; o[6] = B[2]; o[7] = B[4]; o[8] = B[5];
		if (j < TL) {
			double L[6];
			chol3(B, L);
#pragma unroll
			for (int k = 0; k < 6; k++) sm.L[6 * j + k] = L[k];
		}
	}
	if (nb <= 0) return;
	__syncthreads();
	for (int w = tid; w < nbs * 6; w += WARPS * 32) {
		const int b = w / 6, r = w - 6 * b;
		const int lml = sm.lm[b];
		double L[6];
		if (lml < TL) {
#pragma unroll
			for (int k = 0; k < 6; k++) L[k] = sm.L[6 * lml + k];
		} else {
			const double* iv = a.invHll + 9 * (size_t)(ti.l0 + lml);
			const double B[6] = { iv[0], iv[3], iv[6], iv[4], iv[7], iv[8] };
			chol3(B, L);
		}
		double* Vb = sm.V + BS * b;
		const double a0 = Vb[r], a1 = Vb[6 + r], a2 = Vb[12 + r];
		Vb[r] = a0 * L[0] + a1 * L[1] + a2 * L[2];
		Vb[6 + r] = a1 * L[3] + a2 * L[4];
		Vb[12 + r] = a2 * L[5];
		if (r == 0) {
			const double* bb = a.bl + 3 * (size_t)(ti.l0 + lml);
			const double b0 = bb[0], b1 = bb[1], b2 = bb[2];
			Vb[18] = L[0] * b0 + L[1] * b1 + L[2] * b2;
			Vb[19] = L[3] * b1 + L[4] * b2;
			Vb[20] = L[5] * b2;
		}
	}
	__syncthreads();
	const int g = lane >> 2, q = lane & 3;
	const bool inAB = g < 6 && q < 3;
	const int fo = q * 6 + g;
	const int s0 = a.tileSegPtr[t], s1 = a.tileSegPtr[t + 1];
	const int4 none = make_int4(0, 0, 0, 0);
	int4 rec = s0 + wid < s1 ? __ldg(a.segRec + s0 + wid) : none;
	int4 recN = s0 + wid + WARPS < s1 ? __ldg(a.segRec + s0 + wid + WARPS) : none;
	unsigned int cur = 0;
	if (s0 + wid < s1 && lane < rec.y) cur = __ldg(a.off + rec.x + lane);
	const double* aBase = inAB ? sm.V + fo : sm.zero;
	const int aMul = inAB ? 1 : 0;
	for (int s = s0 + wid; s < s1; s += WARPS) {
		const int4 recNN = s + 2 * WARPS < s1 ? __ldg(a.segRec + s + 2 * WARPS) : none;
		unsigned int nxt = 0;
		if (s + WARPS < s1 && lane < recN.y) nxt = __ldg(a.off + recN.x + lane);
		const bool diag = (rec.w & 1) != 0;
		const bool useU = diag && g == 6 && q < 3;
		const double* bBase = inAB ? sm.V + fo : (useU ? sm.V + 18 + q : sm.zero);
		const int bMul = (inAB || useU) ? 1 : 0;
		double c0 = 0.0, c1 = 0.0, d0 = 0.0, d1 = 0.0, e0 = 0.0, e1 = 0.0, f0 = 0.0, f1 = 0.0;
		const int n0 = rec.x, n1 = rec.x + rec.y;
		if (!(rec.w & 2)) {
			for (int nb0 = n0; nb0 < n1; nb0 += 32) {
				const int nn = n1 - nb0 < 32 ? n1 - nb0 : 32;
				unsigned int my = cur;
				if (nb0 > n0) { my = 0; if (lane < nn) my = __ldg(a.off + nb0 + lane); }
#define CUBA_S5_STEP(U, C0, C1)                                                                   \
				{                                                                                 \
					const unsigned int o = __shfl_sync(0xffffffffu, my, (U));                     \
					dmma884(C0, C1, aBase[(o & 0xffffu) * aMul], bBase[(o >> 16) * bMul]);        \
				}
				int u = 0;
				for (; u + 4 <= nn; u += 4) {
					CUBA_S5_STEP(u, c0, c1) CUBA_S5_STEP(u + 1, d0, d1) CUBA_S5_STEP(u + 2, e0, e1) CUBA_S5_STEP(u + 3, f0, f1)
				}
				for (; u < nn; u++) CUBA_S5_STEP(u, c0, c1)
#undef CUBA_S5_STEP
			}
			c0 = (c0 + d0) + (e0 + f0); c1 = (c1 + d1) + (e1 + f1);
		} else {
			for (int n = n0; n < n1; n++) {
				const int bi = __ldg(a.p2i + n), bj = __ldg(a.p2j + n);
				const int lmg = a.hplLm[bi];
				const double* iv = a.invHll + 9 * (size_t)lmg;
				const double B[6] = { iv[0], iv[3], iv[6], iv[4], iv[7], iv[8] };
				double L[6];
				chol3(B, L);
				const double lq0 = q == 0 ? L[0] : 0.0, lq1 = q == 0 ? L[1] : (q == 1 ? L[3] : 0.0), lq2 = q == 0 ? L[2] : (q == 1 ? L[4] : L[5]);
				double av = 0.0, bv = 0.0;
				if (inAB) {
					const double* gi = a.Hpl + 18 * (size_t)bi;
					const double* gj = a.Hpl + 18 * (size_t)bj;
					av = gi[g] * lq0 + gi[6 + g] * lq1 + gi[12 + g] * lq2;
					bv = gj[g] * lq0 + gj[6 + g] * lq1 + gj[12 + g] * lq2;
				} else if (useU) {
					const double* bb = a.bl + 3 * (size_t)lmg;
					bv = q == 0 ? L[0] * bb[0] + L[1] * bb[1] + L[2] * bb[2] : (q == 1 ? L[3] * bb[1] + L[4] * bb[2] : L[5] * bb[2]);
				}
				dmma884(c0, c1, av, bv);
			}
		}
		double* out = a.partial + (size_t)schur2::PW * rec.z;
		if (g < 6) {
			if (q < 3) { out[(2 * q) * 6 + g] = c0; out[(2 * q + 1) * 6 + g] = c1; }
			else out[36 + g] = c0;
		}
		rec = recN; recN = recNN; cur = nxt;
	}
}

}
}
```

### include/cuba_b200.h

```cpp
#ifndef CUBA_B200_H
#define CUBA_B200_H

#include <stddef.h>
#include <stdint.h>

#ifdef __cplusplus
extern "C" {
#endif

#define CUBA_OK 0
#define CUBA_ERR_INVALID (-1)
#define CUBA_ERR_CUDA (-2)
#define CUBA_ERR_STATE (-3)
#define CUBA_ERR_COMM (-4)

#define CUBA_ROBUST_NONE 0
#define CUBA_ROBUST_HUBER 1
#define CUBA_ROBUST_TUKEY 2

#define CUBA_EDGE_MONOCULAR 0
#define CUBA_EDGE_STEREO 1

#define CUBA_PROF_INITIALIZE 0
#define CUBA_PROF_BUILD_STRUCTURE 1
#define CUBA_PROF_COMPUTE_ERROR 2
#define CUBA_PROF_BUILD_SYSTEM 3
#define CUBA_PROF_SCHUR_COMPLEMENT 4
#define CUBA_PROF_DECOMP_SYMBOLIC 5
#define CUBA_PROF_DECOMP_NUMERICAL 6
#define CUBA_PROF_UPDATE 7
#define CUBA_PROF_NUM 8

typedef struct cuba_config {
	int device;
	int use_fp32;
	int pcg_max_iters;
	double pcg_tol;
	int deterministic;
	int reserved[7];
} cuba_config;

typedef struct cuba_problem {
	int32_t Pall, numP;
	int32_t Lall, numL;
	const double* q;
	const double* t;
	const double* cam;
	const double* Xw;
	int32_t E2;
	const int32_t* idx2;
	const double* meas2;
	const double* omega2;
	int32_t E3;
	const int32_t* idx3;
	const double* meas3;
	const double* omega3;
} cuba_problem;

typedef struct cuba_iter_stat {
	int32_t iteration;
	int32_t trials;
	double chi2;
	double lambda;
	int32_t pcg_iters;
	int32_t pcg_failed;
} cuba_iter_stat;

typedef struct cuba_sizes {
	int32_t Pall, numP, Lall, numL, E2, E3;
	int32_t nhpl;
	int32_t nblk;
	int32_t nmul;
	int32_t nblk_full;
} cuba_sizes;

typedef struct cuba_engine cuba_engine;

const char* cuba_last_error(void);
int cuba_version(void);

int cuba_engine_create(const cuba_config* cfg , cuba_engine** out);
int cuba_engine_destroy(cuba_engine* e);

int cuba_engine_set_robust_kernel(cuba_engine* e, int edge_type, int kernel_type, double delta);

int cuba_comm_unique_id(void* out128);
int cuba_engine_set_comm(cuba_engine* e, int rank, int world, const void* nccl_unique_id);

int cuba_engine_set_problem(cuba_engine* e, const cuba_problem* p);
int cuba_engine_set_structure_reuse(cuba_engine* e, int enable);
int cuba_engine_get_structure_reuses(cuba_engine* e, long long* count);
int cuba_engine_set_state(cuba_engine* e, const double* q, const double* t, const double* Xw);

int cuba_engine_reset_state(cuba_engine* e);

int cuba_engine_get_sizes(const cuba_engine* e, cuba_sizes* out);
int cuba_engine_get_stream(cuba_engine* e, void** stream);
int cuba_engine_flush_l2(cuba_engine* e);

int cuba_engine_optimize(cuba_engine* e, int niterations, cuba_iter_stat* stats, int* nstats);

int cuba_engine_get_state(cuba_engine* e, double* q, double* t, double* Xw);
int cuba_engine_get_chi2(cuba_engine* e, double* per_edge);
int cuba_engine_get_profile(cuba_engine* e, double* seconds);
int cuba_engine_get_launch_count(cuba_engine* e, long long* count);

int cuba_get_transfer_bytes(long long* h2d, long long* d2h);

int cuba_stage_linearize(cuba_engine* e, double* chi2);
int cuba_stage_max_diagonal(cuba_engine* e, double* maxdiag);
int cuba_stage_solve(cuba_engine* e, double lambda, int* pcg_iters, int* ok);
int cuba_stage_update(cuba_engine* e, double lambda, double* chi2_trial, double* scale);
int cuba_stage_commit(cuba_engine* e, int accept);
int cuba_stage_chi2(cuba_engine* e, double* chi2);

int cuba_debug_get_hpl_structure(cuba_engine* e, int32_t* colPtr, int32_t* rowInd, int32_t* edge2Hpl);
int cuba_debug_get_hsc_structure(cuba_engine* e, int32_t* rowPtr, int32_t* colInd);
int cuba_debug_get_system(cuba_engine* e, double* Hpp , double* bp , double* Hll ,
	double* bl , double* Hpl );
int cuba_debug_get_schur(cuba_engine* e, double* Hsc , double* bsc , double* invHll );
int cuba_debug_get_delta(cuba_engine* e, double* xp , double* xl );

#define CUBA_PCG_INFO_LEN 16
#define CUBA_PCG_KERNEL_NONE 0
#define CUBA_PCG_KERNEL_PCG 1
#define CUBA_PCG_KERNEL_PCG2 2
#define CUBA_PCG_KERNEL_PCG3 3
#define CUBA_PCG_KERNEL_PCG4 4
#define CUBA_PCG_KERNEL_PCG5 5
#define CUBA_PCG_KERNEL_PCG5_BIG 6
#define CUBA_PCG_KERNEL_PCG5T 7
#define CUBA_COARSE_KERNEL_NONE 0
#define CUBA_COARSE_KERNEL_INVERT 1
#define CUBA_COARSE_KERNEL_CLUSTER8 2
#define CUBA_COARSE_KERNEL_CLUSTER16 3
#define CUBA_COARSE_KERNEL_DENSE 4
#define CUBA_COARSE_KERNEL_PCG4_CLUSTER 5
int cuba_debug_get_pcg_info(cuba_engine* e, int32_t* info, double* coarse_lambda);
int cuba_debug_get_coarse(cuba_engine* e, int32_t* aggRow, double* AcP, float* AcInv);

int cuba_debug_build_structure_host(const cuba_problem* p, int rank, int world, cuba_sizes* sizes,
	int32_t* hplColPtr , int32_t* hplRowInd , int32_t* edge2Hpl ,
	int32_t* hscRowPtr , int32_t* hscColInd ,
	int32_t* fullRowPtr , int32_t* fullColInd ,
	int32_t* shard );

int cuba_debug_pcg_partition(const cuba_problem* p, int nCtas, int maxAgg, int32_t* info);

int cuba_debug_pcg5_plan(const cuba_problem* p, int world, int numSMs, int maxAgg, int32_t* info);
int cuba_debug_pcg5_plan_apc(const cuba_problem* p, int world, int numSMs, int maxAgg, int aggsPerCta, int32_t* info, uint64_t* hash);
int cuba_debug_dropin_problem(void* dropin, cuba_problem* out);

int cuba_bench_stage(cuba_engine* e, int stage, int reps, int flush_l2, double lambda, double* avg_ms);

#ifdef __cplusplus
}
#endif
#endif
```

Measured before the change: 236.7 million.

## Rewrite dense coarse inverse as in-place tiled Gauss-Jordan with FP64 MMA

Replaces the dense coarse-matrix inversion (blocked Cholesky, then triangular inverse, then W^T W product, with 16-wide tiles and scalar FMA loops) with a single-sweep in-place symmetric inversion. It uses 32x32 packed lower-triangular tiles ping-ponged between two buffers, cp.async staging and FP64 mma.sync m8n8k4 for the tile updates. This removes the separate inverse and product phases and their grid barriers, along with the dense padded M/L/W/Dinv buffers and the memset. It adds dynamic shared memory and a more intricate tile-indexing scheme. A debug entry point is also added to test the inverse on a host-supplied coarse matrix.

```diff
diff --git a/cuda-bundle-adjustment_b200/binding.py b/cuda-bundle-adjustment_b200/binding.py
--- a/cuda-bundle-adjustment_b200/binding.py
+++ b/cuda-bundle-adjustment_b200/binding.py
@@ -54,7 +54,7 @@
     "cuba_engine_optimize", "cuba_engine_get_state", "cuba_engine_get_chi2", "cuba_engine_get_profile",
     "cuba_engine_get_launch_count", "cuba_get_transfer_bytes", "cuba_stage_linearize", "cuba_stage_max_diagonal", "cuba_stage_solve", "cuba_stage_update",
     "cuba_stage_commit", "cuba_stage_chi2", "cuba_debug_get_hpl_structure", "cuba_debug_get_hsc_structure",
-    "cuba_debug_get_system", "cuba_debug_get_schur", "cuba_debug_get_delta", "cuba_debug_get_pcg_info", "cuba_debug_get_coarse", "cuba_debug_build_structure_host", "cuba_debug_pcg_partition", "cuba_debug_pcg5_plan", "cuba_debug_pcg5_plan_apc", "cuba_debug_dropin_problem", "cuba_bench_stage",
+    "cuba_debug_get_system", "cuba_debug_get_schur", "cuba_debug_get_delta", "cuba_debug_get_pcg_info", "cuba_debug_get_coarse", "cuba_debug_coarse_inverse", "cuba_debug_build_structure_host", "cuba_debug_pcg_partition", "cuba_debug_pcg5_plan", "cuba_debug_pcg5_plan_apc", "cuba_debug_dropin_problem", "cuba_bench_stage",
 ]
 
 
@@ -105,6 +105,7 @@
         "cuba_debug_get_delta": [vp, vp, vp],
         "cuba_debug_get_pcg_info": [vp, vp, C.POINTER(d)],
         "cuba_debug_get_coarse": [vp, vp, vp, vp],
+        "cuba_debug_coarse_inverse": [vp, vp, i, vp, vp],
         "cuba_debug_build_structure_host": [C.POINTER(_Problem), i, i, C.POINTER(_Sizes), vp, vp, vp, vp, vp, vp, vp, vp],
         "cuba_debug_pcg_partition": [C.POINTER(_Problem), i, i, vp],
         "cuba_debug_pcg5_plan": [C.POINTER(_Problem), i, i, i, vp],
@@ -373,6 +374,16 @@
         _check(self.L.cuba_debug_get_coarse(self.h, _p(agg), _p(AcP), _p(AcInv)))
         return agg, AcP, AcInv
 
+    def coarse_inverse(self, AcP):
+        AcP = np.ascontiguousarray(AcP, dtype=np.float64)
+        nb = AcP.shape[0]
+        A = int(round(((8 * nb + 1) ** 0.5 - 1) / 2))
+        assert A * (A + 1) // 2 == nb and AcP.shape[1:] == (36,), AcP.shape
+        AcInv = np.zeros((6 * A, 6 * A), np.float32)
+        info = C.c_int(-1)
+        _check(self.L.cuba_debug_coarse_inverse(self.h, _p(AcP), A, _p(AcInv), C.byref(info)))
+        return AcInv, info.value
+
     def bench_stage(self, stage, reps=10, flush_l2=True, lam=1.0):
         ms = C.c_double(0)
         _check(self.L.cuba_bench_stage(self.h, int(stage), int(reps), int(bool(flush_l2)), float(lam), C.byref(ms)))
diff --git a/cuda-bundle-adjustment_b200/csrc/cuba_coarse_dense.cuh b/cuda-bundle-adjustment_b200/csrc/cuba_coarse_dense.cuh
--- a/cuda-bundle-adjustment_b200/csrc/cuba_coarse_dense.cuh
+++ b/cuda-bundle-adjustment_b200/csrc/cuba_coarse_dense.cuh
@@ -5,259 +5,263 @@
 namespace cuba_b200 {
 namespace cdense {
 
-constexpr int NB = 16;
+constexpr int NB = 32;
+constexpr int TT = NB * NB;
 constexpr int WARPS = 8;
-constexpr int TS = NB + 1;
+constexpr int TS = NB + 4;
+constexpr size_t SMEM = ((size_t)(2 * WARPS + 2) * NB * TS + NB) * sizeof(double);
 
 struct Args {
 	const double* AcP;
 	int A;
-	double* M;
-	double* Lm;
-	double* Dinv;
-	double* W;
+	double* T;
 	float* AcInv;
 	int* info;
 	GridBar* bar;
 };
 
-__device__ __forceinline__ double ldcg(const double* p) { return __ldcg(p); }
-
-__device__ __forceinline__ bool chol16(double* sD, double* sLi, int lane)
-{
-	bool ok = true;
-	double rdiag = 0.0;
-	for (int j = 0; j < NB; j++) {
-		const double d = sD[j * TS + j];
-		if (!(d > 0)) { ok = false; break; }
-		const double sq = sqrt(d), rs = 1.0 / sq;
-		__syncwarp();
-		if (lane == j) { sD[j * TS + j] = sq; rdiag = rs; }
-		else if (lane > j && lane < NB) sD[lane * TS + j] = sD[lane * TS + j] * rs;
-		__syncwarp();
-		if (lane > j && lane < NB) {
-			const double lrj = sD[lane * TS + j];
-			for (int c = j + 1; c <= lane; c++) sD[lane * TS + c] -= lrj * sD[c * TS + j];
-		}
-		__syncwarp();
-	}
-	if (!ok) return false;
-	double col[NB];
-#pragma unroll
-	for (int i = 0; i < NB; i++) col[i] = 0.0;
-	const int q = lane;
-#pragma unroll
-	for (int i = 0; i < NB; i++) {
-		const double ri = __shfl_sync(0xffffffffu, rdiag, i);
-		if (q < NB && i >= q) {
-			if (i == q) col[i] = ri;
-			else {
-				double s = 0;
-#pragma unroll
-				for (int k = 0; k < NB; k++) if (k >= q && k < i) s += sD[i * TS + k] * col[k];
-				col[i] = -s * ri;
-			}
-		}
-	}
-	if (q < NB) {
-#pragma unroll
-		for (int i = 0; i < NB; i++) sLi[i * TS + q] = i >= q ? col[i] : 0.0;
-	}
-	__syncwarp();
-	return true;
+__host__ __device__ constexpr size_t tiles(int nt) { return (size_t)nt * (nt + 1) / 2; }
+__device__ __forceinline__ const double* tile(const double* C, int I, int J) { return C + ((size_t)I * (I + 1) / 2 + J) * TT; }
+__device__ __forceinline__ double* tile(double* C, int I, int J) { return C + ((size_t)I * (I + 1) / 2 + J) * TT; }
+
+__device__ __forceinline__ void tri_decode(int t, int& i, int& j)
+{
+	i = (int)((sqrt(8.0 * t + 1.0) - 1.0) * 0.5);
+	while ((i + 1) * (i + 2) / 2 <= t) i++;
+	while (i * (i + 1) / 2 > t) i--;
+	j = t - i * (i + 1) / 2;
+}
+
+__device__ __forceinline__ void stage(double* s, const double* g, int lane)
+{
+#pragma unroll
+	for (int e = lane; e < TT / 2; e += 32) {
+		const int r = e >> 4, c = (e & 15) * 2;
+		cp_async16(s + r * TS + c, g + r * NB + c);
+	}
+	asm volatile("cp.async.commit_group;" ::: "memory");
+}
+
+__device__ __forceinline__ void mma32(double (&D)[4][4][2], const double* sX, int xr, int xc, const double* sY, int yr, int yc, int lane)
+{
+	const int r = lane >> 2, q = lane & 3;
+	const double* xb = sX + r * xr + q * xc;
+	const double* yb = sY + q * yr + r * yc;
+#pragma unroll
+	for (int s = 0; s < NB / 4; s++) {
+		double a[4], b[4];
+#pragma unroll
+		for (int u = 0; u < 4; u++) { a[u] = xb[8 * u * xr + 4 * s * xc]; b[u] = yb[4 * s * yr + 8 * u * yc]; }
+#pragma unroll
+		for (int bi = 0; bi < 4; bi++)
+#pragma unroll
+			for (int bj = 0; bj < 4; bj++) dmma884(D[bi][bj][0], D[bi][bj][1], a[bi], b[bj]);
+	}
+}
+
+__device__ __forceinline__ void frag_store(double* s, const double (&D)[4][4][2], double sgn, int lane)
+{
+	const int r = lane >> 2, c = 2 * (lane & 3);
+#pragma unroll
+	for (int bi = 0; bi < 4; bi++)
+#pragma unroll
+		for (int bj = 0; bj < 4; bj++) *reinterpret_cast<double2*>(s + (8 * bi + r) * TS + 8 * bj + c) = make_double2(sgn * D[bi][bj][0], sgn * D[bi][bj][1]);
+}
+
+__device__ __forceinline__ void tile_out(const double* s, int sr, int sc, double sgn, bool diag, int I, int J, double* dst, bool last,
+                                         float* AcInv, int n, int lane)
+{
+	auto at = [&](int r, int c) { if (diag && r < c) { const int t = r; r = c; c = t; } return sgn * s[r * sr + c * sc]; };
+	if (!last) {
+		for (int e = lane; e < TT / 2; e += 32) {
+			const int r = e >> 4, c = (e & 15) * 2;
+			__stcg(reinterpret_cast<double2*>(dst + r * NB + c), make_double2(at(r, c), at(r, c + 1)));
+		}
+		return;
+	}
+	for (int e = lane; e < TT; e += 32) {
+		const int r = e >> 5, c = e & 31;
+		const int row = NB * I + r, col = NB * J + c;
+		if (row < n && col < n) AcInv[(size_t)row * n + col] = (float)-at(r, c);
+		const int row2 = NB * J + r, col2 = NB * I + c;
+		if (I != J && row2 < n && col2 < n) AcInv[(size_t)row2 * n + col2] = (float)-at(c, r);
+	}
 }
 
 __global__ void __launch_bounds__(WARPS * 32, 1) k_coarse_dense(const Args a)
 {
-	__shared__ double sD[NB * TS], sLi[NB * TS];
-	__shared__ double sP[WARPS][2][NB * TS];
+	extern __shared__ __align__(16) double smem[];
+	double* sN = smem;
+	double* sPv = sN + NB * TS;
+	double* sRow = sPv + NB * TS;
+	double* sW = sRow + NB;
 	__shared__ int s_fail;
 	__shared__ unsigned int s_gen;
 	const int tid = threadIdx.x, lane = tid & 31, wid = tid >> 5;
 	const int G = gridDim.x, cta = blockIdx.x;
-	const int n = 6 * a.A, nt = (n + NB - 1) / NB, np = nt * NB;
-	const int nwarps = G * WARPS, gw = cta * WARPS + wid;
+	const int n = 6 * a.A, nt = (n + NB - 1) / NB;
 	if (tid == 0) { s_gen = ld_acquire_u32(&a.bar->gen); s_fail = 0; }
 	__syncthreads();
 	unsigned int gen = s_gen;
-	const int r = lane >> 1, c0 = (lane & 1) * 8;
 
 	{
-		const int nblkP = a.A * (a.A + 1) / 2;
-		for (long long e = (long long)cta * blockDim.x + tid; e < (long long)nblkP * 36; e += (long long)G * blockDim.x) {
-			const int b = (int)(e / 36), rc = (int)(e - 36LL * b), c = rc / 6, rr = rc - 6 * c;
-			int ib = (int)((sqrt(8.0 * b + 1.0) - 1.0) * 0.5);
-			while ((ib + 1) * (ib + 2) / 2 <= b) ib++;
-			while (ib * (ib + 1) / 2 > b) ib--;
-			const int jb = b - ib * (ib + 1) / 2;
-			const int row = 6 * ib + rr, col = 6 * jb + c;
-			if (row >= col) __stcg(a.M + (size_t)col * np + row, a.AcP[e]);
-		}
-		for (int i = n + cta * blockDim.x + tid; i < np; i += G * blockDim.x) __stcg(a.M + (size_t)i * np + i, 1.0);
+		const long long tot = (long long)tiles(nt) * TT;
+		for (long long e = (long long)cta * blockDim.x + tid; e < tot; e += (long long)G * blockDim.x) {
+			const int t = (int)(e / TT), rc = (int)(e - (long long)t * TT);
+			int I, J;
+			tri_decode(t, I, J);
+			int row = NB * I + (rc >> 5), col = NB * J + (rc & 31);
+			if (row < col) { const int x = row; row = col; col = x; }
+			double v = row == col ? 1.0 : 0.0;
+			if (row < n) {
+				const int ib = row / 6, jb = col / 6;
+				v = a.AcP[((size_t)ib * (ib + 1) / 2 + jb) * 36 + (col - 6 * jb) * 6 + (row - 6 * ib)];
+			}
+			__stcg(a.T + e, v);
+		}
 	}
 	grid_barrier(a.bar, G, gen);
 
-	for (int k = 0; k < nt; k++) {
+	double* sA = sW + (size_t)wid * 2 * NB * TS;
+	double* sB = sA + NB * TS;
+	const int slot = (wid + WARPS - 1) % WARPS;
+	const int m = nt - 1, ntl = m * (m + 1) / 2;
+	for (int K = 0; K < nt; K++) {
+		const double* src = a.T + (size_t)(K & 1) * tiles(nt) * TT;
+		double* dst = a.T + (size_t)((K + 1) & 1) * tiles(nt) * TT;
+		const bool last = K == nt - 1;
+		int t = slot * G + cta;
+		int I = 0, J = 0;
+		auto locate = [&](int tt) {
+			int li, lj;
+			tri_decode(tt, li, lj);
+			I = li + (li >= K); J = lj + (lj >= K);
+		};
+		auto issue = [&]() {
+			stage(sA, I > K ? tile(src, I, K) : tile(src, K, I), lane);
+			stage(sB, J > K ? tile(src, J, K) : tile(src, K, J), lane);
+		};
+		if (t < ntl) { locate(t); issue(); }
 		if (wid == 0) {
-			for (int e = lane; e < NB * NB; e += 32) { const int rr = e % NB, cc = e / NB; sD[rr * TS + cc] = rr >= cc ? ldcg(a.M + (size_t)(k * NB + cc) * np + k * NB + rr) : 0.0; }
-			__syncwarp();
-			const bool ok = chol16(sD, sLi, lane);
-			if (!ok && lane == 0) s_fail = 1;
-			if (ok && cta == 0) {
-				for (int e = lane; e < NB * NB; e += 32) {
-					const int rr = e % NB, cc = e / NB;
-					__stcg(a.Lm + (size_t)(k * NB + cc) * np + k * NB + rr, rr >= cc ? sD[rr * TS + cc] : 0.0);
-					__stcg(a.Dinv + (size_t)k * NB * NB + rr * NB + cc, sLi[rr * TS + cc]);
+			double row[NB];
+			const double* g = tile(src, K, K) + lane * NB;
+#pragma unroll
+			for (int i = 0; i < NB; i += 2) { const double2 v = __ldcg(reinterpret_cast<const double2*>(g + i)); row[i] = v.x; row[i + 1] = v.y; }
+			bool ok = true;
+			double rdiag = 0.0;
+#pragma unroll
+			for (int k = 0; k < NB; k++) {
+				sRow[lane] = row[k];
+				__syncwarp();
+				const double d = sRow[k];
+				if (!(d > 0)) { ok = false; break; }
+				const double lkk = sqrt(d), rk = 1.0 / lkk;
+				const double lik = lane > k ? row[k] * rk : lane == k ? lkk : 0.0;
+				if (lane == k) rdiag = rk;
+				__syncwarp();
+				sRow[lane] = lik;
+				__syncwarp();
+#pragma unroll
+				for (int j = k + 1; j < NB; j++) row[j] = fma(-lik, sRow[j], row[j]);
+				row[k] = lik;
+				__syncwarp();
+			}
+			if (!ok) { if (lane == 0) s_fail = 1; }
+			else {
+#pragma unroll
+				for (int i = 0; i < NB; i += 2) *reinterpret_cast<double2*>(sPv + lane * TS + i) = make_double2(row[i], row[i + 1]);
+				sRow[lane] = rdiag;
+				__syncwarp();
+				double x[NB];
+#pragma unroll
+				for (int i = 0; i < NB; i++) {
+					double sum = i == lane ? 1.0 : 0.0;
+#pragma unroll
+					for (int k = 0; k < i; k++) sum = fma(-sPv[i * TS + k], x[k], sum);
+					x[i] = sum * sRow[i];
 				}
+#pragma unroll
+				for (int i = 0; i < NB; i++) sN[i * TS + lane] = x[i];
+				__syncwarp();
+				if (cta == 0) {
+					double pp[4][4][2];
+#pragma unroll
+					for (int bi = 0; bi < 4; bi++)
+#pragma unroll
+						for (int bj = 0; bj < 4; bj++) pp[bi][bj][0] = pp[bi][bj][1] = 0.0;
+					mma32(pp, sN, 1, TS, sN, TS, 1, lane);
+					frag_store(sPv, pp, 1.0, lane);
+					__syncwarp();
+					tile_out(sPv, TS, 1, -1.0, true, K, K, tile(dst, K, K), last, a.AcInv, n, lane);
+				}
 			}
 		}
 		__syncthreads();
-		if (s_fail) break;
-		const int m = nt - k - 1;
-		const int ntile = m * (m + 1) / 2;
-		double* Pi = sP[wid][0];
-		double* Pj = sP[wid][1];
-		for (int t = gw; t < ntile; t += nwarps) {
-			int li = (int)((sqrt(8.0 * t + 1.0) - 1.0) * 0.5);
-			while ((li + 1) * (li + 2) / 2 <= t) li++;
-			while (li * (li + 1) / 2 > t) li--;
-			const int lj = t - li * (li + 1) / 2;
-			const int i = k + 1 + li, j = k + 1 + lj;
+		if (s_fail) { asm volatile("cp.async.wait_group 0;" ::: "memory"); break; }
+
+		for (bool first = true; t < ntl; t += G * WARPS, first = false) {
+			if (!first) { locate(t); issue(); }
+			const bool trI = I < K, trJ = J < K;
+			double acc[4][4][2];
 			{
-				double arow[NB];
-#pragma unroll
-				for (int mm = 0; mm < NB; mm++) arow[mm] = ldcg(a.M + (size_t)(k * NB + mm) * np + i * NB + r);
-#pragma unroll
-				for (int c = 0; c < 8; c++) {
-					const int cc = c0 + c;
-					double s = 0;
-#pragma unroll
-					for (int mm = 0; mm < NB; mm++) if (mm <= cc) s += arow[mm] * sLi[cc * TS + mm];
-					Pi[r * TS + cc] = s;
-				}
-				if (j != i) {
-#pragma unroll
-					for (int mm = 0; mm < NB; mm++) arow[mm] = ldcg(a.M + (size_t)(k * NB + mm) * np + j * NB + r);
-#pragma unroll
-					for (int c = 0; c < 8; c++) {
-						const int cc = c0 + c;
-						double s = 0;
-#pragma unroll
-						for (int mm = 0; mm < NB; mm++) if (mm <= cc) s += arow[mm] * sLi[cc * TS + mm];
-						Pj[r * TS + cc] = s;
+				const double* g = tile(src, I, J) + (lane >> 2) * NB + 2 * (lane & 3);
+#pragma unroll
+				for (int bi = 0; bi < 4; bi++)
+#pragma unroll
+					for (int bj = 0; bj < 4; bj++) {
+						const double2 v = __ldcg(reinterpret_cast<const double2*>(g + 8 * bi * NB + 8 * bj));
+						acc[bi][bj][0] = v.x; acc[bi][bj][1] = v.y;
 					}
-				}
-			}
-			__syncwarp();
-			const double* Q = j != i ? Pj : Pi;
-#pragma unroll
-			for (int c = 0; c < 8; c++) {
-				const int cc = c0 + c;
-				double s = 0;
-#pragma unroll
-				for (int mm = 0; mm < NB; mm++) s += Pi[r * TS + mm] * Q[cc * TS + mm];
-				double* dst = a.M + (size_t)(j * NB + cc) * np + i * NB + r;
-				__stcg(dst, ldcg(dst) - s);
-				if (j == i) __stcg(a.Lm + (size_t)(k * NB + cc) * np + i * NB + r, Pi[r * TS + cc]);
-			}
-			__syncwarp();
-		}
-		grid_barrier(a.bar, G, gen);
+			}
+			asm volatile("cp.async.wait_group 0;" ::: "memory");
+			__syncwarp();
+			double q[4][4][2];
+#pragma unroll
+			for (int bi = 0; bi < 4; bi++)
+#pragma unroll
+				for (int bj = 0; bj < 4; bj++) q[bi][bj][0] = q[bi][bj][1] = 0.0;
+			mma32(q, sA, trI ? 1 : TS, trI ? TS : 1, sN, 1, TS, lane);
+			__syncwarp();
+			frag_store(sA, q, 1.0, lane);
+			if (I == J) frag_store(sB, q, -1.0, lane);
+			else {
+#pragma unroll
+				for (int bi = 0; bi < 4; bi++)
+#pragma unroll
+					for (int bj = 0; bj < 4; bj++) q[bi][bj][0] = q[bi][bj][1] = 0.0;
+				mma32(q, sB, trJ ? 1 : TS, trJ ? TS : 1, sN, 1, TS, lane);
+				__syncwarp();
+				frag_store(sB, q, -1.0, lane);
+			}
+			__syncwarp();
+			mma32(acc, sA, TS, 1, sB, 1, TS, lane);
+			if (I == J) {
+#pragma unroll
+				for (int bi = 0; bi < 4; bi++)
+#pragma unroll
+					for (int bj = 0; bj < 4; bj++) q[bi][bj][0] = q[bi][bj][1] = 0.0;
+				mma32(q, sA, TS, 1, sN, TS, 1, lane);
+			}
+			__syncwarp();
+			frag_store(sB, acc, 1.0, lane);
+			__syncwarp();
+			tile_out(sB, TS, 1, 1.0, I == J, I, J, tile(dst, I, J), last, a.AcInv, n, lane);
+			__syncwarp();
+			if (I == J) {
+				frag_store(sB, q, 1.0, lane);
+				__syncwarp();
+				if (I > K) tile_out(sB, TS, 1, 1.0, false, I, K, tile(dst, I, K), last, a.AcInv, n, lane);
+				else tile_out(sB, 1, TS, 1.0, false, K, I, tile(dst, K, I), last, a.AcInv, n, lane);
+				__syncwarp();
+			}
+		}
+		if (!last) grid_barrier(a.bar, G, gen);
 	}
 	if (s_fail) {
 		for (long long e = (long long)cta * blockDim.x + tid; e < (long long)n * n; e += (long long)G * blockDim.x) a.AcInv[e] = 0.f;
 		if (cta == 0 && tid == 0) *a.info = 1;
 		return;
 	}
-
-	for (int jt = cta; jt < nt; jt += G) {
-		for (int e = tid; e < NB * NB; e += blockDim.x) { const int rr = e / NB, cc = e % NB; __stcg(a.W + (size_t)(jt * NB + cc) * np + jt * NB + rr, ldcg(a.Dinv + (size_t)jt * NB * NB + e)); }
-		__syncthreads();
-		for (int i = jt + 1; i < nt; i++) {
-			double acc[8];
-#pragma unroll
-			for (int c = 0; c < 8; c++) acc[c] = 0.0;
-			for (int k = jt + wid; k < i; k += WARPS) {
-				double lrow[NB];
-#pragma unroll
-				for (int mm = 0; mm < NB; mm++) lrow[mm] = ldcg(a.Lm + (size_t)(k * NB + mm) * np + i * NB + r);
-#pragma unroll
-				for (int c = 0; c < 8; c++) {
-					const double* wc = a.W + (size_t)(jt * NB + c0 + c) * np + k * NB;
-					double s = 0;
-#pragma unroll
-					for (int mm = 0; mm < NB; mm++) s += lrow[mm] * ldcg(wc + mm);
-					acc[c] += s;
-				}
-			}
-#pragma unroll
-			for (int c = 0; c < 8; c++) sP[wid][1][r * NB + c0 + c] = acc[c];
-			__syncthreads();
-			if (wid == 0) {
-				double* S = sP[0][0];
-#pragma unroll
-				for (int c = 0; c < 8; c++) {
-					double s = 0;
-#pragma unroll
-					for (int w = 0; w < WARPS; w++) s += sP[w][1][r * NB + c0 + c];
-					S[r * TS + c0 + c] = s;
-				}
-				__syncwarp();
-				double lrow[NB];
-#pragma unroll
-				for (int mm = 0; mm < NB; mm++) lrow[mm] = ldcg(a.Dinv + (size_t)i * NB * NB + r * NB + mm);
-#pragma unroll
-				for (int c = 0; c < 8; c++) {
-					double s = 0;
-#pragma unroll
-					for (int mm = 0; mm < NB; mm++) if (mm <= r) s += lrow[mm] * S[mm * TS + c0 + c];
-					__stcg(a.W + (size_t)(jt * NB + c0 + c) * np + i * NB + r, -s);
-				}
-			}
-			__syncthreads();
-		}
-	}
-	grid_barrier(a.bar, G, gen);
-
-	{
-		const int ntile = nt * (nt + 1) / 2;
-		double* Wi = sP[wid][0];
-		double* Wj = sP[wid][1];
-		for (int t = gw; t < ntile; t += nwarps) {
-			int i = (int)((sqrt(8.0 * t + 1.0) - 1.0) * 0.5);
-			while ((i + 1) * (i + 2) / 2 <= t) i++;
-			while (i * (i + 1) / 2 > t) i--;
-			const int j = t - i * (i + 1) / 2;
-			double acc[8];
-#pragma unroll
-			for (int c = 0; c < 8; c++) acc[c] = 0.0;
-			for (int k = i; k < nt; k++) {
-#pragma unroll
-				for (int c = 0; c < 8; c++) {
-					Wi[r * TS + c0 + c] = ldcg(a.W + (size_t)(i * NB + c0 + c) * np + k * NB + r);
-					Wj[r * TS + c0 + c] = ldcg(a.W + (size_t)(j * NB + c0 + c) * np + k * NB + r);
-				}
-				__syncwarp();
-#pragma unroll
-				for (int c = 0; c < 8; c++) {
-					double s = 0;
-#pragma unroll
-					for (int mm = 0; mm < NB; mm++) s += Wi[mm * TS + r] * Wj[mm * TS + c0 + c];
-					acc[c] += s;
-				}
-				__syncwarp();
-			}
-#pragma unroll
-			for (int c = 0; c < 8; c++) {
-				const int row = i * NB + r, col = j * NB + c0 + c;
-				if (row < n && col < n) {
-					const float v = (float)acc[c];
-					a.AcInv[(size_t)row * n + col] = v;
-					a.AcInv[(size_t)col * n + row] = v;
-				}
-			}
-		}
-	}
 	if (cta == 0 && tid == 0) *a.info = 0;
 }
 
diff --git a/cuda-bundle-adjustment_b200/csrc/cuba_engine.cu b/cuda-bundle-adjustment_b200/csrc/cuba_engine.cu
--- a/cuda-bundle-adjustment_b200/csrc/cuba_engine.cu
+++ b/cuda-bundle-adjustment_b200/csrc/cuba_engine.cu
@@ -185,6 +185,7 @@
 	virtual int dbg_pcg_timing(long long* out, int maxCtas) = 0;
 	virtual int dbg_pcg_info(int32_t* info, double* coarseLambda) = 0;
 	virtual int dbg_coarse(int32_t* rowAgg, double* AcP, float* AcInv) = 0;
+	virtual int dbg_coarse_inverse(const double* AcP, int A, float* AcInv, int* info) = 0;
 };
 
 template <typename T>
@@ -1361,7 +1362,7 @@
 	DBuf<T> p5Linv, p5R0, p5Zhat, p5RcRow, p5Rc0;
 	DBuf<float> p5AcInv;
 	DBuf<double> p5AcP, p5Lp, p5Wp, p5Ld;
-	DBuf<double> cdM, cdL, cdW, cdDinv;
+	DBuf<double> cdT;
 	bool p5Dense = false;
 	DBuf<unsigned long long> p5Boards;
 	void* p5PeerBase[PCG5_MAXWORLD] = { nullptr };
@@ -1583,8 +1584,7 @@
 		CUDA_TRY(fHat.alloc(36 * (size_t)S.nfull));
 		CUDA_TRY(p5AcP.alloc(nblkPz * 36)); CUDA_TRY(p5AcInv.alloc((size_t)nc * nc)); CUDA_TRY(p5Lp.alloc(nblkPz * 36)); CUDA_TRY(p5Wp.alloc(nblkPz * 36)); CUDA_TRY(p5Ld.alloc((size_t)A * 36));
 		if (p5Dense) {
-			const size_t ntd = ((size_t)nc + cdense::NB - 1) / cdense::NB, npd = ntd * cdense::NB;
-			CUDA_TRY(cdM.alloc(npd * npd)); CUDA_TRY(cdL.alloc(npd * npd)); CUDA_TRY(cdW.alloc(npd * npd)); CUDA_TRY(cdDinv.alloc(ntd * cdense::NB * cdense::NB));
+			CUDA_TRY(cdT.alloc(2 * cdense::tiles((nc + cdense::NB - 1) / cdense::NB) * cdense::TT));
 			CUDA_TRY(gridBar.alloc(1));
 		}
 		const size_t wW = 4 * 6 * nP, pW = 4 * (size_t)PCG5_REPL * G * p5t::pcg5t_np(plan.apc), rW = 4 * (size_t)PCG5_REPL * W * NR, cW = 4 * (size_t)PCG5_REPL * nc;
@@ -1611,21 +1611,24 @@
 		return CUBA_OK;
 	}
 
+	int launch_coarse_dense(const double* AcP, int A, double* tiles, float* AcInv, int* info, GridBar* bar)
+	{
+		CUDA_TRY(cudaFuncSetAttribute(cdense::k_coarse_dense, cudaFuncAttributeMaxDynamicSharedMemorySize, (int)cdense::SMEM));
+		cdense::Args da;
+		da.AcP = AcP; da.A = A; da.T = tiles; da.AcInv = AcInv; da.info = info; da.bar = bar;
+		void* dargs[] = { (void*)&da };
+		CUDA_TRY(cudaLaunchCooperativeKernel((void*)cdense::k_coarse_dense, dim3(numSMs), dim3(cdense::WARPS * 32), dargs, cdense::SMEM, stream));
+		launches++;
+		return CUBA_OK;
+	}
+
 	int launch_coarse_setup(int A, int cluster, size_t invSmem, const int* cbPtr, const int* cbList, double* AcP, float* AcInv, double* Lp, double* Ld, double* Wp, bool dense = false)
 	{
 		const int nblkP = A * (A + 1) / 2;
 		int* infoP = p5InfoSlot();
 		KLAUNCH(k_coarse_project<T>, 36LL * S.nfull, fVal.p, cRowOf.p, fColInd.p, S.nfull, cZx.p, cU.p);
 		KLAUNCH(k_coarse_assemble, (long long)nblkP * 36, cbPtr, cbList, cU.p, nblkP, AcP);
-		if (dense) {
-			CUDA_TRY(cudaMemsetAsync(cdM.p, 0, sizeof(double) * cdM.n, stream));
-			cdense::Args da;
-			da.AcP = AcP; da.A = A; da.M = cdM; da.Lm = cdL; da.Dinv = cdDinv; da.W = cdW; da.AcInv = AcInv; da.info = infoP; da.bar = gridBar;
-			void* dargs[] = { (void*)&da };
-			CUDA_TRY(cudaLaunchCooperativeKernel((void*)cdense::k_coarse_dense, dim3(numSMs), dim3(cdense::WARPS * 32), dargs, 0, stream));
-			launches++;
-			return CUBA_OK;
-		}
+		if (dense) return launch_coarse_dense(AcP, A, cdT, AcInv, infoP, gridBar);
 		if (cluster) {
 			cudaLaunchConfig_t lc = {};
 			lc.gridDim = dim3(cluster); lc.blockDim = dim3(1024); lc.dynamicSmemBytes = invSmem; lc.stream = stream;
@@ -2106,6 +2109,25 @@
 		if (oAcInv) CUDA_TRY(cudaMemcpy(oAcInv, p5AcInv.p, sizeof(float) * (size_t)nc * nc, cudaMemcpyDeviceToHost));
 		return CUBA_OK;
 	}
+	int dbg_coarse_inverse(const double* hAcP, int A, float* hAcInv, int* hInfo) override
+	{
+		if (A < 1 || !hAcP || !hAcInv || !hInfo) return fail(CUBA_ERR_INVALID, "debug_coarse_inverse: A < 1 or a NULL pointer");
+		const size_t nc = 6 * (size_t)A, nblkP = (size_t)A * (A + 1) / 2;
+		DBuf<double> dAcP, dT;
+		DBuf<float> dInv;
+		DBuf<int> dInfo;
+		DBuf<GridBar> dBar;
+		CUDA_TRY(dAcP.alloc(36 * nblkP)); CUDA_TRY(dInv.alloc(nc * nc)); CUDA_TRY(dInfo.alloc(1)); CUDA_TRY(dBar.alloc(1));
+		CUDA_TRY(dT.alloc(2 * cdense::tiles((int)((nc + cdense::NB - 1) / cdense::NB)) * cdense::TT));
+		CUDA_TRY(cudaMemcpyAsync(dAcP.p, hAcP, sizeof(double) * 36 * nblkP, cudaMemcpyHostToDevice, stream));
+		CUDA_TRY(cudaMemsetAsync(dBar.p, 0, sizeof(GridBar), stream));
+		CUDA_TRY(cudaMemsetAsync(dInfo.p, 0xff, sizeof(int), stream));
+		int rc = launch_coarse_dense(dAcP, A, dT, dInv, dInfo, dBar); if (rc) return rc;
+		CUDA_TRY(cudaMemcpyAsync(hAcInv, dInv.p, sizeof(float) * nc * nc, cudaMemcpyDeviceToHost, stream));
+		CUDA_TRY(cudaMemcpyAsync(hInfo, dInfo.p, sizeof(int), cudaMemcpyDeviceToHost, stream));
+		CUDA_TRY(cudaStreamSynchronize(stream));
+		return CUBA_OK;
+	}
 
 	int bench_stage(int stage, int reps, int flush, double lambda, double* ms) override
 	{
@@ -2275,6 +2297,7 @@
 int cuba_debug_get_delta(cuba_engine* e, double* xp, double* xl) { ENGINE_OR_FAIL(e); return e->impl->dbg_delta(xp, xl); }
 int cuba_debug_get_pcg_info(cuba_engine* e, int32_t* info, double* coarse_lambda) { ENGINE_OR_FAIL(e); return e->impl->dbg_pcg_info(info, coarse_lambda); }
 int cuba_debug_get_coarse(cuba_engine* e, int32_t* aggRow, double* AcP, float* AcInv) { ENGINE_OR_FAIL(e); return e->impl->dbg_coarse(aggRow, AcP, AcInv); }
+int cuba_debug_coarse_inverse(cuba_engine* e, const double* AcP, int A, float* AcInv, int* info) { ENGINE_OR_FAIL(e); return e->impl->dbg_coarse_inverse(AcP, A, AcInv, info); }
 int cuba_debug_build_structure_host(const cuba_problem* p, int rank, int world, cuba_sizes* sizes,
 	int32_t* hplColPtr, int32_t* hplRowInd, int32_t* edge2Hpl, int32_t* hscRowPtr, int32_t* hscColInd,
 	int32_t* fullRowPtr, int32_t* fullColInd, int32_t* shard)
diff --git a/cuda-bundle-adjustment_b200/csrc/cuba_math.cuh b/cuda-bundle-adjustment_b200/csrc/cuba_math.cuh
--- a/cuda-bundle-adjustment_b200/csrc/cuba_math.cuh
+++ b/cuda-bundle-adjustment_b200/csrc/cuba_math.cuh
@@ -212,4 +212,9 @@
 	for (int i = 0; i < 4; i++) q[i] = invn * r[i];
 }
 
-}
+__device__ __forceinline__ void dmma884(double& c0, double& c1, double a, double b)
+{
+	asm volatile("mma.sync.aligned.m8n8k4.row.col.f64.f64.f64.f64 {%0, %1}, {%2}, {%3}, {%0, %1};" : "+d"(c0), "+d"(c1) : "d"(a), "d"(b));
+}
+
+}
diff --git a/cuda-bundle-adjustment_b200/csrc/cuba_schur5.cuh b/cuda-bundle-adjustment_b200/csrc/cuba_schur5.cuh
--- a/cuda-bundle-adjustment_b200/csrc/cuba_schur5.cuh
+++ b/cuda-bundle-adjustment_b200/csrc/cuba_schur5.cuh
@@ -16,11 +16,6 @@
 	double L[TL * 6];
 	int lm[TL];
 };
-
-__device__ __forceinline__ void dmma884(double& c0, double& c1, double a, double b)
-{
-	asm volatile("mma.sync.aligned.m8n8k4.row.col.f64.f64.f64.f64 {%0, %1}, {%2}, {%3}, {%0, %1};" : "+d"(c0), "+d"(c1) : "d"(a), "d"(b));
-}
 
 __device__ __forceinline__ void chol3(const double B[6], double L[6])
 {
diff --git a/include/cuba_b200.h b/include/cuba_b200.h
--- a/include/cuba_b200.h
+++ b/include/cuba_b200.h
@@ -138,6 +138,7 @@
 #define CUBA_COARSE_KERNEL_PCG4_CLUSTER 5
 int cuba_debug_get_pcg_info(cuba_engine* e, int32_t* info, double* coarse_lambda);
 int cuba_debug_get_coarse(cuba_engine* e, int32_t* aggRow, double* AcP, float* AcInv);
+int cuba_debug_coarse_inverse(cuba_engine* e, const double* AcP, int A, float* AcInv, int* info);
 
 int cuba_debug_build_structure_host(const cuba_problem* p, int rank, int world, cuba_sizes* sizes,
 	int32_t* hplColPtr , int32_t* hplRowInd , int32_t* edge2Hpl ,
```

New measurement: 246.3 million (median of 6 runs). 4.0% higher.
